# simonmeister/UnFlow

Measured on AMD Instinct MI355X. Metric: image-pairs/s (fwd+bwd) FlowNetC 384x512, higher is better.
Workload: dtype f32; 1 GPU; FlowNetC unsupervised step: bidirectional fwd + census/2nd-order loss pyramid + bwd + L2/Adam, 4 pairs/GPU, 384x512, 441-ch correlation (BASELINE configs[1]); global_batch=4, height=384, width=512, parallelism=dp1, hipgraph=True

## Files before the change

### include/unflow_hip.h

```cpp
#ifndef UNFLOW_HIP_H_
#define UNFLOW_HIP_H_

#include <stddef.h>

#ifdef __cplusplus
extern "C" {
#endif

typedef void* unflow_stream_t;
typedef struct unflow_planes unflow_planes;

#define UNFLOW_OK 0
#define UNFLOW_ERR_NULL (-1)
#define UNFLOW_ERR_EMPTY_OUTPUT (-2)
#define UNFLOW_ERR_EVEN_KERNEL (-3)
#define UNFLOW_ERR_NOT_DIVISIBLE (-4)
#define UNFLOW_ERR_SHAPE (-5)
#define UNFLOW_ERR_UNSUPPORTED (-7)
#define UNFLOW_ERR_LAUNCH (-8)
#define UNFLOW_ERR_WORKSPACE (-9)

const char* unflow_status_string(int status);
int unflow_version(void);

// ... 68 lines not shown
                             size_t workspace_bytes, unflow_stream_t stream);

int unflow_conv2d_transpose_fwd(const float* x, int ldx, const float* w, const float* bias, float* y, int ldy,
                                int B, int H, int W, int Cin, int Cout, int leaky, void* workspace,
                                size_t workspace_bytes, unflow_stream_t stream);
int unflow_conv2d_transpose_bwd_data(const float* dz, int lddz, const float* w, float* dx, int lddx, int B, int H,
                                     int W, int Cin, int Cout, int accumulate, const float* act_src, int ld_act,
                                     int act_lo, int act_hi, void* workspace, size_t workspace_bytes,
                                     unflow_stream_t stream);
int unflow_conv2d_transpose_bwd_filter(const float* x, int ldx, const float* dz, int lddz, float* dw, float* dbias,
                                       int B, int H, int W, int Cin, int Cout, void* workspace,
                                       size_t workspace_bytes, unflow_stream_t stream);

size_t unflow_colsum_batched_workspace_bytes(int n, const int* C);
int unflow_colsum_batched(int n, const float* const* x, const int* ld, const long* npix, const int* C,
                          float* const* out, void* workspace, size_t workspace_bytes, unflow_stream_t stream);

size_t unflow_conv_workspace_bytes(int B, int H, int W, int Cin, int Cout, int k, int stride);

int unflow_leaky_bwd_inplace(float* dy, int lddy, const float* y, int ldy, long npix, int C, unflow_stream_t stream);


int unflow_rgb_to_gray255(const float* im, int ld_im, float* gray, long npix, unflow_stream_t stream);

int unflow_warp_gray_fwd(const float* im, int ld_im, const float* flow, float flow_scale, float* out_gray,
                         int pair_shift, int N, int H, int W, unflow_stream_t stream);
int unflow_warp_gray_bwd(const float* d_gray, const float* im, int ld_im, const float* flow, float flow_scale,
                         float* d_flow, int accumulate, int pair_shift, int N, int H, int W,
                         unflow_stream_t stream);

int unflow_ternary_fwd(const float* gray1, const float* gray2w, const float* mask, int n_mask, float* dist_out,
                       float* loss_acc, float weight, float normalizer, int max_distance, int N, int H, int W,
                       unflow_stream_t stream);
int unflow_ternary_bwd(const float* gray1, const float* gray2w, const float* mask, int n_mask,
                       const float* dist, float* d_gray2w, float weight, float normalizer, int max_distance,
                       int N, int H, int W, unflow_stream_t stream);

int unflow_gray_pair(const float* im, int ld_im, const float* flow, float flow_scale, float* gray1, float* gray2w,
                     int pair_shift, int N, int H, int W, unflow_stream_t stream);
int unflow_ternary_warp_bwd(const float* gray1, const float* gray2w, const float* dist, const float* im, int ld_im,
                            const float* flow, float flow_scale, float* d_flow, int accumulate, int pair_shift,
                            int max_distance, int N, int H, int W, unflow_stream_t stream);

int unflow_second_order_fwd_bwd(const float* flow, float flow_scale, float* loss_acc, float* d_flow,
                                int accumulate, float weight, float normalizer, int N, int H, int W,
                                unflow_stream_t stream);

int unflow_mask_terms(const float* flow, const float* warped_other, const float* fwarp, const float* base_mask,
                      int n_base, float flow_scale, int occlusion_mode, float* mask_out, float* loss_acc, float* d_flow,
                      float* d_warped, int accumulate, float fb_weight, float occ_weight, float sym_weight,
                      int batch_per_direction, int pair_shift, int N, int H, int W, unflow_stream_t stream);

#define UNFLOW_MAX_PYR_LEVELS 7
typedef struct unflow_pyr_level {
  const float* im;
  const float* flow;
  float* gray1;
  float* gray2w;
  const float* mask;
  float* dist;
  float* d_flow;
  int H, W, n_mask, max_distance;
  float flow_scale, ternary_scale, smooth_scale;
} unflow_pyr_level;
int unflow_sizeof_pyr_level(void);
int unflow_loss_pyramid_default(const unflow_pyr_level* levels, int n_levels, int N, int pair_shift, float* loss_acc,
                                int with_grad, unflow_stream_t stream);

int unflow_photometric_fwd_bwd(const float* im, int ld_im, const float* flow, float flow_scale, const float* mask,
                               int n_mask, float* loss_acc, float* d_flow, int accumulate, float weight, float normalizer,
                               int pair_shift, int N, int H, int W, unflow_stream_t stream);

int unflow_charbonnier_loss(const float* x, const float* mask, int mask_channels, float truncate, float alpha, float beta,
                            float epsilon, float* loss_acc, float weight, long npix, int C, unflow_stream_t stream);
int unflow_length_sq(const float* x, float* out, long npix, int C, unflow_stream_t stream);

int unflow_smooth_1st_fwd_bwd(const float* flow, float flow_scale, float* loss_acc, float* d_flow, int accumulate,
                              float weight, float normalizer, int N, int H, int W, unflow_stream_t stream);

int unflow_gradient_loss_fwd(const float* im1, int ld_im1, const float* im2_warped, const float* mask, int n_mask,
                             float* gdiff, float* loss_acc, float weight, float normalizer, int N, int H, int W,
                             unflow_stream_t stream);
int unflow_gradient_loss_bwd(const float* gdiff, float* d_im2_warped, int N, int H, int W, unflow_stream_t stream);


int unflow_prepare_images(const float* im_u8range, float* net_in4, float* out01, const float* mean3, long npix,
                          unflow_stream_t stream);

int unflow_prepare_image_pair(const float* im1, const float* im2, long npix_each, float* net_in4, float* out01,
                              const float* mean3, const unflow_planes* net_pl, unflow_stream_t stream);

int unflow_scale(const float* x, float s, float* y, long n, unflow_stream_t stream);
int unflow_mul_inplace(float* y, const float* x, long n, unflow_stream_t stream);
int unflow_add_inplace(float* y, const float* x, long n, unflow_stream_t stream);
int unflow_zero(void* p, size_t bytes, unflow_stream_t stream);
int unflow_copy(void* dst, const void* src, size_t bytes, unflow_stream_t stream);


int unflow_stn_affine_fwd(const float* U, int n_u, int ld_u, const float* theta, int n_theta, float* out, int ld_out,
                          int B, int H, int W, int C, int out_h, int out_w, unflow_stream_t stream);

int unflow_photometric_augment(const float* im, int ld_in, float* out, int ld_out, const float* contrast,
                               const float* brightness, const float* colour3, const float* gamma, const float* noise,
                               int n_par, const float* mean3, int N, int H, int W, unflow_stream_t stream);

int unflow_supervised_geo_augment(const float* im1, const float* im2, const float* flow_gt, const float* mask_gt,
                                  const float* mats, const float* contrast, const float* brightness, const float* colour3,
                                  const float* gamma, const float* noise, int n_par, const float* mean3, float* im01, float* x0,
                                  int ld_out, float* flow_out, float* mask_out, int mode, int B, int H, int W,
                                  unflow_stream_t stream);

int unflow_stack_input(const float* net_in4, const float* prev_flow2, float* out, int ld_out, int pair_shift, int N,
                       int H, int W, int h, int w, float flow_scale, unflow_stream_t stream);

int unflow_stack_input_bwd(const float* d_out, int ld_out, const float* net_in4, const float* prev_flow2,
                           float* d_prev_flow2, int pair_shift, int N, int H, int W, int h, int w, float flow_scale,
                           unflow_stream_t stream);

typedef struct unflow_planes {
  void* base;
  long plane_stride;
  int ld;
  int n_planes;
  float scale;
} unflow_planes;

int unflow_correlation_nhwc_fwd_pl(const float* in0, const float* in1, int ld_in, const unflow_planes* in0_pl,
                                   const unflow_planes* in1_pl, int pair_shift, float* out, int ld_out, int B, int C,
                                   int H, int W, int kernel_size, int max_displacement, int pad, int stride_1,
                                   int stride_2, unflow_stream_t stream);

int unflow_correlation_nhwc_bwd_pl(const float* dout, int ld_dout, const float* in0, const float* in1, int ld_in,
                                   const unflow_planes* in0_pl, const unflow_planes* in1_pl, int pair_shift, float* grad0,
                                   float* grad1, int ld_grad, int accumulate_g1_into_g0, int B, int C, int H, int W,
                                   int kernel_size, int max_displacement, int pad, int stride_1, int stride_2,
                                   unflow_stream_t stream);

int unflow_planes_from_f32(const float* x, int ldx, long npix, int C, int C_fill, const unflow_planes* out,
                           unflow_stream_t stream);

size_t unflow_weight_planes_elems(int taps, int R, int Cc, int transposed);
int unflow_weight_planes_batched(int n, const float* const* w, const int* taps, const int* R, const int* Cc,
                                 void* const* direct, void* const* transposed, int n_planes, unflow_stream_t stream);

int unflow_adam_planes_batched(int n, float* const* w, const int* taps, const int* R, const int* Cc, void* const* direct,
                               void* const* transposed, const int* regularized, int n_planes, float* P, const float* G, float* M,
                               float* V, float grad_scale, float l2_scale, float lr_t, float beta1, float beta2, float eps,
                               float* loss_acc, unflow_stream_t stream);

size_t unflow_conv_pl_workspace_bytes(int B, int H, int W, int Cin, int Cout, int k, int stride, int n_planes);

size_t unflow_flow_wgrad_batched_workspace_bytes(int n, const int* kind, const int* B, const int* H, const int* W, const int* Cin);
int unflow_flow_wgrad_batched(int n, const int* kind, const float* const* x, const int* ldx, const float* const* dz,
                              const int* lddz, float* const* dw, const int* B, const int* H, const int* W, const int* Cin,
                              void* workspace, size_t workspace_bytes, unflow_stream_t stream);

int unflow_debug_work_order(int mt, int nt, int ncls, int nsplit, int order, int xcd, int* out, int out_blocks);

int unflow_comm_available(void);
int unflow_comm_unique_id(void* id128);
int unflow_comm_init(const void* id128, int nranks, int rank, void** comm);
int unflow_comm_info(void* comm, int* nranks, int* rank);
int unflow_allreduce_sum_f32(float* buf, long n, void* comm, unflow_stream_t stream);
int unflow_comm_destroy(void* comm);

int unflow_debug_streamk_plan(int G, int mtp, int nt, int nchunk, int ncls, const int* ntaps, int ngroups, int* range_pos, int npos,
                              const int* pos, int* decoded);
int unflow_debug_streamk_timeouts(void);

int unflow_conv2d_fwd_pl(const float* x, int ldx, const unflow_planes* x_pl, const float* w, const unflow_planes* w_pl,
                         const float* bias, float* y, int ldy, const unflow_planes* y_pl, int B, int H, int W, int Cin,
                         int Cout, int k, int stride, int leaky, void* workspace, size_t workspace_bytes,
                         unflow_stream_t stream);
int unflow_conv2d_bwd_data_pl(const float* dz, int lddz, const unflow_planes* dz_pl, const float* w,
                              const unflow_planes* w_pl, float* dx, int lddx, const unflow_planes* dx_pl, int pl_lo,
                              int pl_hi, int B, int H, int W, int Cin, int Cout, int k, int stride, int accumulate,
                              const float* act_src, int ld_act, const unflow_planes* act_pl, int act_lo, int act_hi,
                              void* workspace, size_t workspace_bytes, unflow_stream_t stream);
int unflow_conv2d_bwd_filter_pl(const float* x, int ldx, const unflow_planes* x_pl, const float* dz, int lddz,
                                const unflow_planes* dz_pl, float* dw, int B, int H, int W, int Cin, int Cout, int k,
                                int stride, void* workspace, size_t workspace_bytes, unflow_stream_t stream);
int unflow_conv2d_transpose_fwd_pl(const float* x, int ldx, const unflow_planes* x_pl, const float* w,
                                   const unflow_planes* w_pl, const float* bias, float* y, int ldy,
                                   const unflow_planes* y_pl, int B, int H, int W, int Cin, int Cout, int leaky,
                                   void* workspace, size_t workspace_bytes, unflow_stream_t stream);
int unflow_conv2d_transpose_bwd_data_pl(const float* dz, int lddz, const unflow_planes* dz_pl, const float* w,
                                        const unflow_planes* w_pl, float* dx, int lddx, const unflow_planes* dx_pl,
                                        int pl_lo, int pl_hi, int B, int H, int W, int Cin, int Cout, int accumulate,
                                        const float* act_src, int ld_act, const unflow_planes* act_pl, int act_lo,
                                        int act_hi, void* workspace, size_t workspace_bytes, unflow_stream_t stream);
int unflow_conv2d_transpose_bwd_filter_pl(const float* x, int ldx, const unflow_planes* x_pl, const float* dz, int lddz,
                                          const unflow_planes* dz_pl, float* dw, int B, int H, int W, int Cin, int Cout,
                                          void* workspace, size_t workspace_bytes, unflow_stream_t stream);

int unflow_resize_bilinear_tf1(const float* in, float* out, int B, int H, int W, int C, int out_h, int out_w,
                               float scale, unflow_stream_t stream);

int unflow_supervised_flow_loss(const float* flow, int h, int w, const float* flow_gt, const float* mask_gt, float flow_scale,
                                float weight, float* loss_acc, float* d_flow, int accumulate, int B, int H, int W,
                                unflow_stream_t stream);

int unflow_stack_input_pair(const float* first4, const float* second4, const float* prev_flow2, float* out, int ld_out, int N,
                            int H, int W, int h, int w, float flow_scale, unflow_stream_t stream);
int unflow_stack_input_pair_bwd(const float* d_out, int ld_out, const float* first4, const float* second4,
                                const float* prev_flow2, float* d_prev_flow2, int N, int H, int W, int h, int w,
                                float flow_scale, unflow_stream_t stream);

int unflow_adam_step(float* p, const float* grad, float* m, float* v, long n, long n_regularized, float grad_scale,
                     float l2_scale, float lr_t, float beta1, float beta2, float eps, unflow_stream_t stream);

int unflow_adam_step_regloss(float* p, const float* grad, float* m, float* v, long n, long n_regularized,
                             float grad_scale, float l2_scale, float lr_t, float beta1, float beta2, float eps,
                             float* loss_acc, unflow_stream_t stream);

int unflow_l2_loss(const float* p, long n, float scale, float* loss_acc, unflow_stream_t stream);

int unflow_flow_error_sums(const float* f1, const float* f2, const float* mask ,
                           float* out2, long npix, unflow_stream_t stream);



int unflow_inference_input(const void* frames, const int* desc, int B, int Hmax, int Wmax, int H, int W, float* net_in4,
                           const float* mean3, const unflow_planes* net_pl, unflow_stream_t stream);

int unflow_inference_input_frames(const void* frames, const int* desc, int F, int Hmax, int Wmax, int H, int W, float* net_in4,
                                  const float* mean3, const unflow_planes* net_pl, unflow_stream_t stream);

typedef struct {
  void* base;
  long pixels;
  int bytes;
  int stride;
} unflow_carry_buf;
#define UNFLOW_CARRY_MAX 16

int unflow_sequence_carry(const unflow_carry_buf* bufs, int n_bufs, const int* src_row, int max_row, unflow_stream_t stream);

int unflow_sequence_mirror(const unflow_carry_buf* bufs, int n_bufs, int src0, int dst0, int n, int max_row,
                           unflow_stream_t stream);

int unflow_sequence_track(const float* flow_fw, const unsigned char* occ_fw, const int* tab, int B, int Hmax, int Wmax,
                          const int* anchors, int Ncap, float* disp, unsigned char* alive, float* out_disp,
                          unsigned char* out_alive, unflow_stream_t stream);

int unflow_inference_output_blocks(int Hmax, int Wmax);
int unflow_inference_output(const float* flow, int fh, int fw, float flow_scale, int H, int W, const int* desc, int B, int Hmax,
                            int Wmax, float* out_flow, unsigned short* out_u16, const float* gt_flow, const float* gt_mask,
                            double* partial, unsigned* ticket, double* sums, int* counts, unflow_stream_t stream);

int unflow_inference_occlusion(const float* flow_fw, const float* flow_bw, const int* desc, int B, int Hmax, int Wmax,
                               const float* gt_mask, unsigned char* occ_fw, unsigned char* occ_bw, int* counts,
                               unflow_stream_t stream);



int unflow_flow_to_color(const float* flow, const float* mask, const float* max_flow, int B, int H, int W, float* out_f32,
                         unsigned char* out_u8, unsigned* max_bits, unflow_stream_t stream);

int unflow_flow_error_image(const float* flow_1, const float* flow_2, const float* mask_occ, const float* mask_noc, int log_colors,
                            int B, int H, int W, float* out_f32, unsigned char* out_u8, unflow_stream_t stream);

#define UNFLOW_VISUAL_IMAGES 5
int unflow_inference_visual(const void* frames, const int* desc, int B, int Hmax, int Wmax, int H, int W, const float* flow,
                            const float* gt_flow, const float* gt_mask, float* shown, unsigned* max_bits, unsigned char* out_u8,
                            float* out_f32, unflow_stream_t stream);

int unflow_sequence_visual(const void* frames, const int* tab, int B, int Hmax, int Wmax, int H, int W, const float* flow_fw,
                           const float* flow_bw, const unsigned char* occ_fw, float* shown, unsigned* max_bits,
                           unsigned char* out_u8, float* out_f32, unflow_stream_t stream);

size_t unflow_sequence_interpolate_workspace_bytes(int n, int B, int Hmax, int Wmax);
int unflow_sequence_interpolate(const void* frames, const int* tab, int B, int Hmax, int Wmax, int n, const float* flow_fw,
                                const float* flow_bw, const unsigned char* occ_fw, const unsigned char* occ_bw, void* prev,
                                void* workspace, unsigned char* out_mid, int* out_holes, unflow_stream_t stream);



int unflow_png_unfilter_rows(void);

int unflow_png_unfilter(const unsigned char* raw, long raw_bytes, unsigned char* decoded, long decoded_bytes, const long* desc,
                        int n, unflow_stream_t stream);

int unflow_png_to_batch(const unsigned char* decoded, long decoded_bytes, const long* desc, int n, int H, int W,
                        const float* mean3, float stddev, float* out, unflow_stream_t stream);

int unflow_png_to_window(const unsigned char* decoded, long decoded_bytes, const long* desc, int n, int Hs, int Ws,
                         const float* mean3, float stddev, float* out, unflow_stream_t stream);

int unflow_png_to_flow_gt(const unsigned char* decoded, long decoded_bytes, const long* desc, int n, int Hs, int Ws, float* flow,
                          float* mask, unflow_stream_t stream);

int unflow_flo_to_flow_gt(const unsigned char* raw, long raw_bytes, const long* desc, int n, int Hs, int Ws, float* flow,
                          float* mask, unflow_stream_t stream);

int unflow_sintel_gt(const unsigned char* raw, long raw_bytes, const unsigned char* decoded, long decoded_bytes, const long* desc,
                     int n, int Hs, int Ws, float* flow, float* mask, unflow_stream_t stream);


#define UNFLOW_PNG_U8 0
#define UNFLOW_PNG_U8X255 1
#define UNFLOW_PNG_U16BE 2
typedef struct {
  const void* base;
  long image_stride;
  long row_stride;
  int images, H, W;
  int channels;
  int kind;
} unflow_png_surface;
#define UNFLOW_PNG_SURFACES_MAX 16
#define UNFLOW_PNG_FILTER_FIELDS 8
#define UNFLOW_PNG_FILTER_MAX_ROW_BYTES 32512

int unflow_png_filter(const unflow_png_surface* surfaces, int n_surfaces, const long* desc, int n, int max_h, int max_row_bytes,
                      unsigned char* out, long out_bytes, unflow_stream_t stream);

int unflow_stream_create(unflow_stream_t* stream);

#define UNFLOW_DEFLATE_FIELDS 8
#define UNFLOW_DEFLATE_META 4
#define UNFLOW_DEFLATE_CHUNK_MAX 65535
#define UNFLOW_DEFLATE_CHUNK_DEFAULT 16384
int unflow_deflate(const unsigned char* in, long in_bytes, const long* desc, int n, int max_chunks, int chunk_bytes,
                   unsigned char* scratch, long scratch_bytes, int* meta, long meta_chunks, unsigned char* out, long out_bytes,
                   long* sizes, unflow_stream_t stream);
long unflow_deflate_segment_bound(int chunk_bytes);
long unflow_deflate_stream_bound(long bytes, int chunk_bytes);
long unflow_deflate_slot_bytes(int chunk_bytes);

#ifdef __cplusplus
}
#endif
#endif
```

### unflow_amd/core/engine.py

```python
import math
import os
from collections import OrderedDict

import numpy as np
import torch

from .. import _lib
from .._lib import check, ptr, stream, cf, cl
from . import layers as L

FLOW_SCALE = 5.0
CHANNEL_MEAN = [104.920005, 110.1753, 114.785955]
LAYER_WEIGHTS = [12.7, 4.35, 3.9, 3.4, 1.1]
LAYER_PATCH_DISTANCES = [3, 2, 2, 1, 1]
LAYER_WEIGHTS_FULL_RES = [12.7, 5.5, 5.0, 4.35, 3.9, 3.4, 1.1]
LAYER_PATCH_DISTANCES_FULL_RES = [3, 3] + LAYER_PATCH_DISTANCES
L2_SCALE = 0.0004
LOSSES = ['occ', 'sym', 'fb', 'grad', 'ternary', 'photo', 'smooth_1st', 'smooth_2nd']

DEFAULT_PARAMS = dict(flownet='C', pyramid_loss=True, border_mask=True, ternary_weight=1.0, smooth_2nd_weight=3.0)


def pad4(c):
    return (c + 3) // 4 * 4
# ... 302 lines not shown
        assert cuts == sorted(cuts) and (not cuts or cuts[-1] < len(self.bwd))
        self.part_bounds = [0] + cuts + [len(self.bwd)]

    def part_weight_range(self, part):
        ls = [op.l for op, _, _, _ in self.bwd[self.part_bounds[part]:self.part_bounds[part + 1]] if op.kind == 'layer']
        return self.eng.weight_range(ls)

    def alloc(self):
        e = self.eng
        H, W, dev = e.H, e.W, e.dev
        npl = e.n_planes
        self.A, self.Gd = {}, {}
        for name, (div, lay, width) in self.bufs.items():
            is_flow = name.startswith('flow')
            self.A[name] = L.PT.alloc((self.rows[name], H // div, W // div, width), dev, 0 if is_flow else npl)
        self.need_in_grad = (not self.is_c) and self.index > 0 and e.train_all
        if self.need_in_grad and self.full_res:
            raise NotImplementedError("train_all through a full_res refinement stage")
        if self.trainable:
            for name, (div, lay, width) in self.bufs.items():
                if name == 'x0s' and not self.need_in_grad:
                    continue
                is_flow = name.startswith('flow')
                self.Gd[name] = L.PT.alloc((self.rows[name], H // div, W // div, width), dev, 0 if is_flow else npl,
                                           scale=e.grad_plane_scale)
        self.planes_only = set()
        if npl:
            self.planes_only = {n for n in ('c1', 'c4', 'c5', 'c6') + (() if self.is_c else ('c3',)) if n in self.A}
        self.act = ActView(self)
        self.act.update({k: v.t for k, v in self.A.items()})
        self.grad = {k: v.t for k, v in self.Gd.items()}
        if self.full_res:
            self.act['x0s'] = self.act['cat0'][..., :pad4(self.in_ch)]

    def pt(self, spec, grad=False):
        b, lo, hi = spec
        if b == 'x0':
            return self.eng.X0
        src = (self.Gd if grad else self.A)[b]
        return src if (lo == 0 and hi == src.t.shape[-1]) else src.sl(lo, hi)

    def forward(self, prev_flow2=None):
        e = self.eng
        B, N = e.B, e.N
        if not self.is_c:
            x0s = self.act['x0s']
            pf = prev_flow2
            ph, pw = (0, 0) if pf is None else (pf.shape[1], pf.shape[2])
            if self.pairs is None:
                check(_lib.lib().unflow_stack_input(ptr(e.x0), ptr(pf), ptr(x0s), x0s.stride(2), B, N, e.H, e.W, ph, pw,
                                                    cf(4 * FLOW_SCALE), e.stream()), "stack_input")
            else:
                for a, b, o in self.pairs:
                    flow = None if pf is None else pf[o:o + B]
                    check(_lib.lib().unflow_stack_input_pair(ptr(e.x0[a:]), ptr(e.x0[b:]), ptr(flow), ptr(x0s[o:o + B]),
                                                             x0s.stride(2), B, e.H, e.W, ph, pw, cf(4 * FLOW_SCALE), e.stream()),
                          "stack_input_pair")
            inp = self.A[self.bin]
            if inp.pl is not None:
                w_in = pad4(self.in_ch)
                L.planes_from_f32(x0s, inp.pl[..., :round8(w_in)], C=w_in)
        for op in self.ops:
            if op.kind == 'corr':
                c3, out = self.pt(op.src), self.pt(op.dst)
                C = op.src[2] - op.src[1]
                h8, w8 = e.H // 8, e.W // 8
                pl = self._corr_planes(c3, refresh=True)
                if self.pairs is None:
                    c3pl = _lib.planes_of(pl)
                    check(_lib.lib().unflow_correlation_nhwc_fwd_pl(ptr(c3.t), ptr(c3.t), c3.t.stride(2), c3pl, c3pl, B,
                                                                    ptr(out.t), out.t.stride(2), N, C, h8, w8, 1, 20, 20, 1, 2,
                                                                    e.stream()), "correlation")
                else:
                    for a, b, o in self.pairs:
                        p0, p1 = (None, None) if pl is None else (_lib.planes_of(pl[:, a:a + B]), _lib.planes_of(pl[:, b:b + B]))
                        check(_lib.lib().unflow_correlation_nhwc_fwd_pl(ptr(c3.t[a:a + B]), ptr(c3.t[b:b + B]), c3.t.stride(2), p0, p1,
                                                                        0, ptr(out.t[o:o + B]), out.t.stride(2), B, C, h8, w8, 1, 20,
                                                                        20, 1, 2, e.stream()), "correlation")
                if out.pl is not None:
                    L.planes_from_f32(out.t, out.pl)
                continue
            l = op.l
            if self.pairs is not None and l.short == 'conv_redir':
                runs = [(a, o, B) for a, _, o in self.pairs]
            else:
                runs = [(op.r0, op.d0, op.n)]
            for r0, d0, n in runs:
                x, y = _row_range(self.pt(op.src), r0, n), _row_range(self.pt(op.dst), d0, n)
                if l.cout_p != l.cout:
                    y = L.PT(y.t.as_strided(y.t.shape[:3] + (l.cout_p,), y.t.stride(), y.t.storage_offset()),
                             None if y.pl is None else y.pl)
                po = op.dst[0] in self.planes_only
                if l.kind == 'conv':
                    L.conv_fwd(x, l.w, l.wpl_t, l.b, y, l.stride, l.act, planes_only=po)
                else:
                    L.deconv_fwd(x, l.w, l.wpl_d, l.b, y, l.act, planes_only=po)
            if self.seq_bidir and l.short == 'conv2' and self.is_c:
                self.sequence_mirror()

    def mirror_list(self):
        lo, n = self.bufs['cat2'][1]['conv2']
        return _carry_bufs(self.A['cat2'].t, self.A['cat2'].pl, lo, pad4(n))

    def sequence_mirror(self):
        B = self.eng.B
        bufs = self.mirror_list()
        arr = (_lib.CarryBuf * len(bufs))(*bufs)
        check(_lib.lib().unflow_sequence_mirror(arr, len(bufs), self.row0['cat2'] + 1, 0, B, self.rows['cat2'] - 1,
                                                self.eng.stream()), "sequence_mirror")

    def _corr_planes(self, c3, refresh=False):
        e = self.eng
        if e.n_planes == 3:
            return c3.pl
        if e.n_planes != 1:
            return None
        if getattr(self, '_c3_b3', None) is None:
            n, h, w, c = c3.t.shape
            self._c3_b3 = torch.zeros(3, n, h, w, (c + 7) // 8 * 8, dtype=torch.int16, device=c3.t.device)
        if refresh:
            L.planes_from_f32(c3.t, self._c3_b3)
        return self._c3_b3

    def _leaky_bwd_rows(self, g, a, r0, r1, clo, chi):
        gt, at = g.t[r0:r1, ..., clo:chi], a.t[r0:r1, ..., clo:chi]
        L.leaky_bwd_inplace(gt, at)
        if g.pl is not None:
            pl = g.pl[:, r0:r1, ..., clo:min(g.pl.shape[-1], clo + round8(chi - clo))]
            check(_lib.lib().unflow_planes_from_f32(ptr(gt), gt.stride(2), cl(gt.shape[0] * gt.shape[1] * gt.shape[2]),
                                                    chi - clo, min(round8(chi - clo), pl.shape[-1]), _lib.planes_of(pl, g.scale),
                                                    self.eng.stream()), "planes_from_f32")

    def backward(self, part=None, before_join=None):
        e = self.eng
        lo, hi = (0, len(self.bwd)) if part is None else (self.part_bounds[part], self.part_bounds[part + 1])
        B, N = e.B, e.N
        side = e.wgrad_stream
        main = torch.cuda.current_stream(e.dev)
        pending = []
        counter = [100 * (part or 0)]

        def flush():
            if not pending:
                return
            side.wait_stream(main)
            with torch.cuda.stream(side):
                for fn, a in pending:
                    with L.ws_slot(3 + (counter[0] if e.wgrad_unique_ws else 0)):
                        fn(*a)
                    counter[0] += 1
            pending.clear()

        flow_jobs = []
        n_flow = sum(1 for op, _, _, _ in self.bwd[lo:hi] if op.kind == 'layer' and op.l.cout <= 2)

        for k, (op, first, act_lo, act_hi) in enumerate(self.bwd[lo:hi], lo):
            if op.kind == 'corr':
                c3, g3, gout = self.pt(op.src), self.pt(op.src, True), self.pt(op.dst, True)
                C = op.src[2] - op.src[1]
                h8, w8 = e.H // 8, e.W // 8
                assert first
                pl = self._corr_planes(c3)
                if self.pairs is None:
                    c3pl = _lib.planes_of(pl)
                    check(_lib.lib().unflow_correlation_nhwc_bwd_pl(ptr(gout.t), gout.t.stride(2), ptr(c3.t), ptr(c3.t),
                                                                    c3.t.stride(2), c3pl, c3pl, B, ptr(g3.t), ptr(None),
                                                                    g3.t.stride(2), 1, N, C, h8, w8, 1, 20, 20, 1, 2, e.stream()),
                          "correlation_grad")
                else:
                    (a, b, o), = self.pairs
                    p0, p1 = (None, None) if pl is None else (_lib.planes_of(pl[:, a:a + B]), _lib.planes_of(pl[:, b:b + B]))
                    check(_lib.lib().unflow_correlation_nhwc_bwd_pl(ptr(gout.t[o:o + B]), gout.t.stride(2), ptr(c3.t[a:a + B]),
                                                                    ptr(c3.t[b:b + B]), c3.t.stride(2), p0, p1, 0, ptr(g3.t[a:a + B]),
                                                                    ptr(g3.t[b:b + B]), g3.t.stride(2), 0, B, C, h8, w8, 1, 20, 20, 1, 2,
                                                                    e.stream()), "correlation_grad")
                for r0, r1, clo, chi in self.bwd_post_act.get(k, ()):
                    self._leaky_bwd_rows(g3, c3, r0, r1, clo, chi)
                continue
            l = op.l
            x, dz = _rows(self.pt(op.src), op.n), _rows(self.pt(op.dst, True), op.n)
            if l.cout_p != l.cout:
                dz = L.PT(dz.t.as_strided(dz.t.shape[:3] + (l.cout_p,), dz.t.stride(), dz.t.storage_offset()), dz.pl, dz.scale)
            if e._bias_plan is None:
                e._bias_jobs.append((dz.t, l))
            xv = op.src[0] not in self.planes_only
            wg = (L.conv_bwd_filter, (x, dz, l.dw, l.stride, xv)) if l.kind == 'conv' else (L.deconv_bwd_filter, (x, dz, l.dw, xv))
            if l.cout <= 2:
                flow_jobs.append((l.kind, x, dz, l.dw))
                wg = (L.flow_wgrad_batched, (flow_jobs,)) if len(flow_jobs) == n_flow else None
            if wg is None:
                pass
            elif side is None or (e.wgrad_inline_tiny and l.cout <= 2):
                wg[0](*wg[1])
            else:
                pending.append(wg)
                if len(pending) >= e.wgrad_group:
                    flush()
            sb = op.src[0]
            is_input = sb == 'x0' or (sb == self.bin and op.src[1] == 0 and op.src[2] == pad4(self.in_ch)
                                      and op.l.name.endswith('conv1'))
            if sb not in self.Gd or (is_input and not self.need_in_grad):
                continue
            dx = _rows(self.pt(op.src, True), op.n)
            accumulate = (not first) or sb.startswith('flow')
            if k in self.bwd_zero_rows:
                r0, r1 = self.bwd_zero_rows[k]
                gz = self.Gd[sb].t[r0:r1]
                check(_lib.lib().unflow_zero(ptr(gz), _lib.csz(gz.numel() * 4), e.stream()), "zero")
            act_src = _rows(self.pt(op.src), op.n) if act_hi > act_lo else None
            apl = sb in self.planes_only
            if l.kind == 'conv':
                L.conv_bwd_data(dz, l.w, l.wpl_d, dx, l.stride, accumulate, act_src, act_lo, act_hi, act_planes=apl)
            else:
                L.deconv_bwd_data(dz, l.w, l.wpl_t, dx, accumulate, act_src, act_lo, act_hi, act_planes=apl)
        if side is not None:
            flush()
        if before_join is not None:
            before_join()
        if side is not None:
            main.wait_stream(side)


class FlowNetEngine:

    def __init__(self, batch, height, width, params=None, device=None, seed=0, layout_only=False, supervised=False,
                 inference=False, bidirectional=False, sequence=False):
        assert height % 64 == 0 and width % 64 == 0, "FlowNet needs H, W divisible by 64"
        if bidirectional and supervised:
            raise ValueError("FlowNetEngine: bidirectional is for the inference engine; the supervised engine is one-direction")
        if bidirectional and not inference:
            raise ValueError("FlowNetEngine: bidirectional needs inference=True (the training engine is bidirectional already)")
        if supervised and inference:
            raise ValueError("FlowNetEngine: supervised and inference are exclusive")
        if not isinstance(sequence, bool) and sequence != 'bidirectional':
            raise ValueError("FlowNetEngine: sequence is False, True or 'bidirectional', got %r" % (sequence,))
        if sequence and (bidirectional or supervised or not inference):
            raise ValueError("FlowNetEngine: sequence needs inference=True without supervised or bidirectional=True (both "
                             "directions of a clip: sequence='bidirectional')")
        self.supervised = bool(supervised)
        self.inference = bool(inference)
        self.seq_bidir = sequence == 'bidirectional'
        self.bidirectional = bool(bidirectional) or self.seq_bidir
        self.sequence = bool(sequence)
        self.one_dir = self.supervised or (self.inference and not self.bidirectional)
        self.params = dict(DEFAULT_PARAMS) if params is None else dict(params)
        if self.params.get('mask_occlusion', '') not in ('', 'fb', 'disocc'):
            raise ValueError("mask_occlusion must be one of 'fb', 'disocc', ''")
        spec = self.params.get('flownet', 'C')
        if not spec or any(ch not in 'CScs' for ch in spec) or any(ch in 'Cc' for ch in spec[1:]):
            raise ValueError("flownet spec: 'C'/'c' or 'S'/'s' first, then 'S'/'s' refinement nets (flownet.py:20-28)")
        self.train_all = bool(self.params.get('train_all')) and len(spec) > 1
        self.full_res = bool(self.params.get('full_res'))
        if self.supervised and self.full_res and self.train_all:
            raise ValueError("supervised full_res with train_all: the reference subtracts the earlier networks' quarter-size "
                             "flow2 * 20 from the full-size ground truth (supervised.py:50-60), a shape error")
        if sequence and self.full_res:
            raise ValueError("FlowNetEngine: sequence with full_res is not built (DESIGN 7.5)")
        self.spec = spec
        self.B, self.H, self.W = batch, height, width
        self.N = 2 * batch
        self.F = batch + 1
        self.dev = torch.device('cuda:0') if device is None else torch.device(device)
        self.math = conv_math_mode()
        self.wgrad_group = int(os.environ.get('UNFLOW_WGRAD_GROUP', '6'))
        self.wgrad_stream = None
        self.planes_external = False
        self.wgrad_unique_ws = False
        self.wgrad_inline_tiny = False
        self.n_planes = {'bf16x3': 3, 'f16': 1}.get(self.math, 0)
        self.fused_adam = os.environ.get('UNFLOW_FUSED_ADAM', '0') == '1'
        self.grad_plane_scale = 4096.0 if self.math == 'f16' else 0.0
        if layout_only:
            self.n_planes = 0
        self.fused_adam = self.fused_adam and self.n_planes > 0
        import contextlib
        with (torch.cuda.device(self.dev) if self.dev.type == 'cuda' else contextlib.nullcontext()):
            self.stages = [_Stage(self, k, i, self.full_res and i == len(spec) - 1) for i, k in enumerate(spec)]
            for st in self.stages[:-1]:
                st.trainable = self.train_all
            if self.inference:
                for st in self.stages:
                    st.trainable = False
            self.layers = [l for st in self.stages for l in st.layers]
            self.by_name = self.stages[-1].by_name
            self._alloc_params()
            if not layout_only:
                self._alloc_activations()
                if self.wgrad_group > 0 and self.dev.type == 'cuda' and not self.inference:
                    self.wgrad_stream = torch.cuda.Stream(self.dev)
                self._build_masks()
        self.step_count = 0
        self._bias_jobs, self._bias_plan = [], None
        self.defer_l2 = False
        self.fused_pyramid = True
        self._pyr_cache = None
        self._wplanes_version = None
        if seed is not None and not layout_only:
            self.init_params(seed)

    def stream(self):
        return stream(self.dev)

    def _alloc_params(self):
        nw = sum(int(torch.Size(l.wshape()).numel()) for l in self.layers)
        nb = sum(l.cout_p for l in self.layers)
        self.n_weights, self.n_params = nw, nw + nb
        z = lambda: torch.zeros(self.n_params, dtype=torch.float32, device=self.dev)
        self.P = z()
        self.G, self.M, self.V = (None, None, None) if self.inference else (z(), z(), z())
        view = lambda flat, lo, hi, shape=None: None if flat is None else (flat[lo:hi] if shape is None else flat[lo:hi].view(shape))
        off = 0
        for l in self.layers:
            n = int(torch.Size(l.wshape()).numel())
            l.w = self.P[off:off + n].view(l.wshape())
            l.dw = view(self.G, off, off + n, l.wshape())
            l.mw, l.vw = view(self.M, off, off + n, l.wshape()), view(self.V, off, off + n, l.wshape())
            off += n
        for l in self.layers:
            l.b = self.P[off:off + l.cout_p]
            l.db = view(self.G, off, off + l.cout_p)
            l.mb, l.vb = view(self.M, off, off + l.cout_p), view(self.V, off, off + l.cout_p)
            off += l.cout_p
        self._wp_table = None
        if self.n_planes:
            P = self.n_planes
            users = [l for l in self.layers if l.uses_planes()]
            tot = 0
            for l in users:
                d, t = self._wp_layouts(l)
                taps, R, Cc = l.wplane_view()
                tot += P * (d * taps * R * round8(Cc) + t * taps * Cc * round8(R))
            self.WP = torch.zeros(tot, dtype=torch.int16, device=self.dev)
            off = 0
            for l in users:
                d, t = self._wp_layouts(l)
                taps, R, Cc = l.wplane_view()
                if d:
                    n = P * taps * R * round8(Cc)
                    l.wpl_d = self.WP[off:off + n].view(P, taps, R, round8(Cc))
                    off += n
                if t:
                    n = P * taps * Cc * round8(R)
                    l.wpl_t = self.WP[off:off + n].view(P, taps, Cc, round8(R))
                    off += n
            self._wp_users = users
            self._wp_table = self._wp_table_of(users)
            self._wp_range_tables = {}
        self._adam_tables = {}

    def _wp_layouts(self, l):
# ... 828 lines not shown
```

### unflow_amd/core/layers.py

```python
import torch

from .. import _lib
from .._lib import check, ptr, stream, csz
from ..ops import workspace


def nhwc(t):
    assert t.dim() == 4 and t.dtype == torch.float32 and t.is_cuda, "NHWC float32 CUDA tensor expected"
    B, H, W, C = t.shape
    ld = t.stride(2)
    assert t.stride(3) == 1 and t.stride(1) == W * ld and t.stride(0) == H * W * ld, \
        "tensor must be a channel-slice view of a contiguous NHWC buffer"
    return ptr(t), ld, B, H, W, C


def out_hw(H, W, stride):
    return -(-H // stride), -(-W // stride)


_WS_SLOT = [1]


class ws_slot:

# ... 77 lines not shown

def conv2d_transpose_bwd_filter(x, dz, dw, dbias):
    xp, ldx, B, H, W, Cin = nhwc(x)
    dzp, lddz, _, Ho, Wo, Cout = nhwc(dz)
    assert tuple(dw.shape) == (4, 4, Cout, Cin)
    wsp, wsn = _ws(x.device, B, Ho, Wo, Cin, Cout, 4, 2)
    check(_lib.lib().unflow_conv2d_transpose_bwd_filter(xp, ldx, dzp, lddz, ptr(dw), ptr(dbias), B, H, W, Cin, Cout,
                                                        wsp, wsn, stream()), "conv2d_transpose_bwd_filter")
    return dw, dbias


def leaky_bwd_inplace(dy, y):
    dp, ldd, B, H, W, C = nhwc(dy)
    yp, ldy = nhwc(y)[:2]
    check(_lib.lib().unflow_leaky_bwd_inplace(dp, ldd, yp, ldy, _lib.cl(B * H * W), C, stream()), "leaky_bwd")
    return dy


def round8(c):
    return (c + 7) // 8 * 8


class PT:
    __slots__ = ('t', 'pl', 'scale')

    def __init__(self, t, pl=None, scale=0.0):
        self.t, self.pl, self.scale = t, pl, scale

    def sl(self, lo, hi):
        if self.pl is None:
            return PT(self.t[..., lo:hi])
        return PT(self.t[..., lo:hi], self.pl[..., lo:min(self.pl.shape[-1], lo + round8(hi - lo))], self.scale)

    def planes(self):
        return _lib.planes_of(self.pl, self.scale)

    @staticmethod
    def alloc(shape, device, n_planes, scale=0.0):
        import torch as _t
        t = _t.zeros(*shape, dtype=_t.float32, device=device)
        pad = 32
        cp = (shape[-1] + pad - 1) // pad * pad if shape[-1] > 8 else round8(shape[-1])
        pl = _t.zeros(n_planes, *shape[:-1], cp, dtype=_t.int16, device=device) if n_planes else None
        return PT(t, pl, scale if n_planes == 1 else 0.0)


def _pt(x):
    return x if isinstance(x, PT) else PT(x)


def _ws_pl(device, B, H, W, Cin, Cout, k, stride, npl):
    n = _lib.lib().unflow_conv_pl_workspace_bytes(B, H, W, Cin, Cout, k, stride, npl)
    t = workspace(n, device, slot=_WS_SLOT[0])
    return ptr(t), csz(t.numel() * 4)


def _npl(*pts):
    for q in pts:
        if q.pl is not None:
            return q.pl.shape[0]
    return 0


def planes_from_f32(x, out_pl, C=None):
    xp, ldx, B, H, W, Cx = nhwc(x)
    C = Cx if C is None else C
    fill = min(round8(C), out_pl.shape[-1])
    check(_lib.lib().unflow_planes_from_f32(xp, ldx, _lib.cl(B * H * W), C, fill, _lib.planes_of(out_pl), stream()),
          "planes_from_f32")


def conv_fwd(x, w, w_pl, bias, y, stride, leaky, planes_only=False):
    x, y = _pt(x), _pt(y)
    xp, ldx, B, H, W, Cin = nhwc(x.t)
    yp, ldy, _, Ho, Wo, Cout = nhwc(y.t)
    if planes_only:
        assert y.pl is not None
        yp = ptr(None)
    k = w.shape[0]
    assert tuple(w.shape) == (k, k, Cin, Cout) and w.is_contiguous() and (Ho, Wo) == out_hw(H, W, stride)
    wsp, wsn = _ws_pl(x.t.device, B, H, W, Cin, Cout, k, stride, _npl(x, y))
    check(_lib.lib().unflow_conv2d_fwd_pl(xp, ldx, x.planes(), ptr(w), _lib.planes_of(w_pl), ptr(bias), yp, ldy,
                                          y.planes(), B, H, W, Cin, Cout, k, stride, int(bool(leaky)), wsp, wsn,
                                          stream()), "conv2d_fwd_pl")


def _act_args(act_src, act_planes):
    if act_src is None:
        return ptr(None), 0, None
    a = _pt(act_src)
    if act_planes:
        assert a.pl is not None
        return ptr(None), 0, a.planes()
    ap, lda = nhwc(a.t)[:2]
    return ap, lda, None


def conv_bwd_data(dz, w, w_pl, dx, stride, accumulate=False, act_src=None, act_lo=0, act_hi=0, act_planes=False):
    dz, dx = _pt(dz), _pt(dx)
    dzp, lddz, B, Ho, Wo, Cout = nhwc(dz.t)
    dxp, lddx, _, H, W, Cin = nhwc(dx.t)
    k = w.shape[0]
    assert tuple(w.shape) == (k, k, Cin, Cout)
    ap, lda, apl = _act_args(act_src, act_planes)
    wsp, wsn = _ws_pl(dz.t.device, B, H, W, Cin, Cout, k, stride, _npl(dz, dx))
    check(_lib.lib().unflow_conv2d_bwd_data_pl(dzp, lddz, dz.planes(), ptr(w), _lib.planes_of(w_pl), dxp, lddx,
                                               dx.planes(), act_lo, act_hi, B, H, W, Cin, Cout, k, stride,
                                               int(bool(accumulate)), ap, lda, apl, act_lo, act_hi, wsp, wsn, stream()),
          "conv2d_bwd_data_pl")


def conv_bwd_filter(x, dz, dw, stride, x_fp32=True):
    x, dz = _pt(x), _pt(dz)
    xp, ldx, B, H, W, Cin = nhwc(x.t)
    if not x_fp32:
        assert x.pl is not None
        xp = ptr(None)
    dzp, lddz, _, Ho, Wo, Cout = nhwc(dz.t)
    k = dw.shape[0]
    assert tuple(dw.shape) == (k, k, Cin, Cout) and dw.is_contiguous()
    wsp, wsn = _ws_pl(x.t.device, B, H, W, Cin, Cout, k, stride, _npl(x, dz))
    check(_lib.lib().unflow_conv2d_bwd_filter_pl(xp, ldx, x.planes(), dzp, lddz, dz.planes(), ptr(dw), B, H,
                                                 W, Cin, Cout, k, stride, wsp, wsn, stream()), "conv2d_bwd_filter_pl")


def deconv_fwd(x, w, w_pl, bias, y, leaky, planes_only=False):
    x, y = _pt(x), _pt(y)
    xp, ldx, B, H, W, Cin = nhwc(x.t)
    yp, ldy, _, Ho, Wo, Cout = nhwc(y.t)
    if planes_only:
        assert y.pl is not None
        yp = ptr(None)
    assert tuple(w.shape) == (4, 4, Cout, Cin) and (Ho, Wo) == (2 * H, 2 * W)
    wsp, wsn = _ws_pl(x.t.device, B, 2 * H, 2 * W, Cin, Cout, 4, 2, _npl(x, y))
    check(_lib.lib().unflow_conv2d_transpose_fwd_pl(xp, ldx, x.planes(), ptr(w), _lib.planes_of(w_pl), ptr(bias), yp,
                                                    ldy, y.planes(), B, H, W, Cin, Cout, int(bool(leaky)), wsp, wsn,
                                                    stream()), "conv2d_transpose_fwd_pl")


def deconv_bwd_data(dz, w, w_pl, dx, accumulate=False, act_src=None, act_lo=0, act_hi=0, act_planes=False):
    dz, dx = _pt(dz), _pt(dx)
    dzp, lddz, B, Ho, Wo, Cout = nhwc(dz.t)
    dxp, lddx, _, H, W, Cin = nhwc(dx.t)
    assert tuple(w.shape) == (4, 4, Cout, Cin) and (Ho, Wo) == (2 * H, 2 * W)
    ap, lda, apl = _act_args(act_src, act_planes)
    wsp, wsn = _ws_pl(dz.t.device, B, Ho, Wo, Cin, Cout, 4, 2, _npl(dz, dx))
    check(_lib.lib().unflow_conv2d_transpose_bwd_data_pl(dzp, lddz, dz.planes(), ptr(w), _lib.planes_of(w_pl), dxp,
                                                         lddx, dx.planes(), act_lo, act_hi, B, H, W, Cin, Cout,
                                                         int(bool(accumulate)), ap, lda, apl, act_lo, act_hi, wsp, wsn,
                                                         stream()),
          "conv2d_transpose_bwd_data_pl")


def deconv_bwd_filter(x, dz, dw, x_fp32=True):
    x, dz = _pt(x), _pt(dz)
    xp, ldx, B, H, W, Cin = nhwc(x.t)
    if not x_fp32:
        assert x.pl is not None
        xp = ptr(None)
    dzp, lddz, _, Ho, Wo, Cout = nhwc(dz.t)
    assert tuple(dw.shape) == (4, 4, Cout, Cin)
    wsp, wsn = _ws_pl(x.t.device, B, Ho, Wo, Cin, Cout, 4, 2, _npl(x, dz))
    check(_lib.lib().unflow_conv2d_transpose_bwd_filter_pl(xp, ldx, x.planes(), dzp, lddz, dz.planes(),
                                                           ptr(dw), B, H, W, Cin, Cout, wsp, wsn, stream()),
          "conv2d_transpose_bwd_filter_pl")


def flow_wgrad_batched(jobs):
    import ctypes
    n = len(jobs)
    if n == 0:
        return
    xs = [_pt(j[1]).t for j in jobs]
    dzs = [_pt(j[2]).t for j in jobs]
    kinds = (ctypes.c_int * n)(*[0 if j[0] == 'conv' else 1 for j in jobs])
    dims = [nhwc(x) for x in xs]
    Bs = (ctypes.c_int * n)(*[d[2] for d in dims])
    Hs = (ctypes.c_int * n)(*[d[3] for d in dims])
    Ws = (ctypes.c_int * n)(*[d[4] for d in dims])
    Cs = (ctypes.c_int * n)(*[d[5] for d in dims])
    lib = _lib.lib()
    lib.unflow_flow_wgrad_batched_workspace_bytes.restype = ctypes.c_size_t
    need = lib.unflow_flow_wgrad_batched_workspace_bytes(n, kinds, Bs, Hs, Ws, Cs)
    if need == 0 or n > 16:
        for kind, x, dz, dw in jobs:
            if kind == 'conv':
                conv_bwd_filter(x, dz, dw, 1)
            else:
                deconv_bwd_filter(x, dz, dw)
        return
    for (kind, x, dz, dw), xt, dzt in zip(jobs, xs, dzs):
        assert dw.is_contiguous() and dzt.shape[-1] == 2
        assert tuple(dw.shape) == ((3, 3, xt.shape[-1], 2) if kind == 'conv' else (4, 4, 2, 2))
    ws = workspace(need, xs[0].device, slot=_WS_SLOT[0])
    check(lib.unflow_flow_wgrad_batched(n, kinds, (ctypes.c_void_p * n)(*[x.data_ptr() for x in xs]),
                                        (ctypes.c_int * n)(*[x.stride(2) for x in xs]),
                                        (ctypes.c_void_p * n)(*[d.data_ptr() for d in dzs]),
                                        (ctypes.c_int * n)(*[d.stride(2) for d in dzs]),
                                        (ctypes.c_void_p * n)(*[j[3].data_ptr() for j in jobs]), Bs, Hs, Ws, Cs, ptr(ws),
                                        csz(ws.numel() * 4), stream()), "flow_wgrad_batched")
```

### unflow_amd/csrc/conv_igemm.hip

```cpp
#include "igemm_shared.h"
#include "options.h"

namespace {
using namespace igemm;

constexpr int LDK = BK + 4;

struct GatherParams : GatherGeom {
  const float* src;
  const float* w;
  const float* bias;
  float* dst;
  float* partial;
  const float* act_src;
  int lds, ldd, ld_act, act_lo, act_hi;
  int nsplit;
  int leaky, accumulate;
  unsigned cs_magic;
  PlaneOut pl;
};

__device__ __forceinline__ float4 ldg4(const float* p) { return *reinterpret_cast<const float4*>(p); }

typedef __bf16 bf16x8 __attribute__((ext_vector_type(8)));
// ... 1246 lines not shown
    bool ok[2][2];
#pragma unroll
    for (int a = 0; a < 2; a++)
#pragma unroll
      for (int c = 0; c < 2; c++) {
        const int iy = ((oy + 1 - ky0) >> 1) - a, ix = ((ox + 1 - kx0) >> 1) - c;
        ok[a][c] = (unsigned)iy < (unsigned)H && (unsigned)ix < (unsigned)W;
        const float* xp = x + ((size_t)(b * H + min(max(iy, 0), H - 1)) * W + min(max(ix, 0), W - 1)) * ldx;
#pragma unroll
        for (int ci = 0; ci < CI; ci++) xv[a][c][ci] = xp[ci];
      }
    float acc[CO];
#pragma unroll
    for (int c = 0; c < CO; c++) acc[c] = bias ? bias[c] : 0.f;
#pragma unroll
    for (int a = 0; a < 2; a++)
#pragma unroll
      for (int c = 0; c < 2; c++) {
        const float* wp = w + ((ky0 + 2 * a) * 4 + kx0 + 2 * c) * CO * CI;
#pragma unroll
        for (int co = 0; co < CO; co++)
#pragma unroll
          for (int ci = 0; ci < CI; ci++) acc[co] += (ok[a][c] ? xv[a][c][ci] : 0.f) * wp[co * CI + ci];
      }
#pragma unroll
    for (int c = 0; c < CO; c++) {
      y[(size_t)e * ldy + c] = acc[c];
      store_planes(po, (size_t)e, c, acc[c]);
    }
  }
}

template <int CI, int CO>
__global__ void tiny_deconv_dgrad_kernel(const float* __restrict__ dz, int lddz, const float* __restrict__ w,
                                         float* __restrict__ dx, int lddx, int accumulate, int B, int H, int W) {
  const int OH = 2 * H, OW = 2 * W;
  const unsigned n = (unsigned)B * (unsigned)H * (unsigned)W;
  for (unsigned e = blockIdx.x * blockDim.x + threadIdx.x; e < n; e += gridDim.x * blockDim.x) {
    const Pix pp = decode_pix(e, (unsigned)W, (unsigned)H);
    const int ix = pp.x, iy = pp.y, b = pp.n;
    float g[16][CO];
    bool ok[16];
#pragma unroll
    for (int ky = 0; ky < 4; ky++)
#pragma unroll
      for (int kx = 0; kx < 4; kx++) {
        const int oy = 2 * iy + ky - 1, ox = 2 * ix + kx - 1;
        ok[ky * 4 + kx] = (unsigned)oy < (unsigned)OH && (unsigned)ox < (unsigned)OW;
        const float* gp = dz + ((size_t)(b * OH + min(max(oy, 0), OH - 1)) * OW + min(max(ox, 0), OW - 1)) * lddz;
#pragma unroll
        for (int co = 0; co < CO; co++) g[ky * 4 + kx][co] = gp[co];
      }
    float acc[CI];
#pragma unroll
    for (int c = 0; c < CI; c++) acc[c] = 0.f;
#pragma unroll
    for (int t = 0; t < 16; t++) {
      const float* wp = w + t * CO * CI;
#pragma unroll
      for (int co = 0; co < CO; co++)
#pragma unroll
        for (int ci = 0; ci < CI; ci++) acc[ci] += (ok[t] ? g[t][co] : 0.f) * wp[co * CI + ci];
    }
#pragma unroll
    for (int c = 0; c < CI; c++) {
      float* d = dx + (size_t)e * lddx + c;
      *d = accumulate ? *d + acc[c] : acc[c];
    }
  }
}

template <int CI, int CO>
__device__ __forceinline__ void tiny_deconv_wgrad_body(const float* __restrict__ x, int ldx, const float* __restrict__ dz, int lddz,
                                                       float* __restrict__ partial, int B, int H, int W, int bx, int nblocks,
                                                       float (*red)[16 * CO * CI]) {
  constexpr int NV = 16 * CO * CI;
  const int OH = 2 * H, OW = 2 * W;
  const long n = (long)B * H * W;
  float acc[16][CO][CI];
#pragma unroll
  for (int t = 0; t < 16; t++)
#pragma unroll
    for (int a = 0; a < CO; a++)
#pragma unroll
      for (int c = 0; c < CI; c++) acc[t][a][c] = 0.f;
  for (long e = bx * (long)blockDim.x + threadIdx.x; e < n; e += (long)nblocks * blockDim.x) {
    const int ix = (int)(e % W), iy = (int)((e / W) % H);
    const long b = e / ((long)W * H);
    float xv[CI];
#pragma unroll
    for (int c = 0; c < CI; c++) xv[c] = x[e * ldx + c];
#pragma unroll
    for (int ky = 0; ky < 4; ky++) {
      const int oy = 2 * iy + ky - 1;
#pragma unroll
      for (int kx = 0; kx < 4; kx++) {
        const int ox = 2 * ix + kx - 1;
        if ((unsigned)oy < (unsigned)OH && (unsigned)ox < (unsigned)OW) {
          const float* gp = dz + ((b * OH + oy) * OW + ox) * lddz;
#pragma unroll
          for (int co = 0; co < CO; co++)
#pragma unroll
            for (int ci = 0; ci < CI; ci++) acc[ky * 4 + kx][co][ci] += gp[co] * xv[ci];
        }
      }
    }
  }
  const int lane = threadIdx.x & 63, wid = threadIdx.x >> 6;
  static_assert(NV == 64, "the transpose-reduce below maps value index == lane");
  float v32[32], v16[16], v8[8], v4[4], v2[2];
  {
    const float* f = &acc[0][0][0];
    const bool hi = lane & 32;
#pragma unroll
    for (int i = 0; i < 32; i++) v32[i] = (hi ? f[32 + i] : f[i]) + __shfl_xor(hi ? f[i] : f[32 + i], 32);
  }
  {
    const bool hi = lane & 16;
#pragma unroll
    for (int i = 0; i < 16; i++) v16[i] = (hi ? v32[16 + i] : v32[i]) + __shfl_xor(hi ? v32[i] : v32[16 + i], 16);
  }
  {
    const bool hi = lane & 8;
#pragma unroll
    for (int i = 0; i < 8; i++) v8[i] = (hi ? v16[8 + i] : v16[i]) + __shfl_xor(hi ? v16[i] : v16[8 + i], 8);
  }
  {
    const bool hi = lane & 4;
#pragma unroll
    for (int i = 0; i < 4; i++) v4[i] = (hi ? v8[4 + i] : v8[i]) + __shfl_xor(hi ? v8[i] : v8[4 + i], 4);
  }
  {
    const bool hi = lane & 2;
#pragma unroll
    for (int i = 0; i < 2; i++) v2[i] = (hi ? v4[2 + i] : v4[i]) + __shfl_xor(hi ? v4[i] : v4[2 + i], 2);
  }
  {
    const bool hi = lane & 1;
    red[wid][lane] = (hi ? v2[1] : v2[0]) + __shfl_xor(hi ? v2[0] : v2[1], 1);
  }
  __syncthreads();
  if (threadIdx.x < NV)
    partial[(size_t)bx * NV + threadIdx.x] =
        (red[0][threadIdx.x] + red[1][threadIdx.x]) + (red[2][threadIdx.x] + red[3][threadIdx.x]);
}
template <int CI, int CO>
__global__ __launch_bounds__(256) void tiny_deconv_wgrad_kernel(const float* __restrict__ x, int ldx,
                                                                const float* __restrict__ dz, int lddz,
                                                                float* __restrict__ partial, int B, int H, int W) {
  __shared__ float red[4][16 * CO * CI];
  tiny_deconv_wgrad_body<CI, CO>(x, ldx, dz, lddz, partial, B, H, W, blockIdx.x, gridDim.x, red);
}

constexpr int MAX_FLOW_WGRAD = 16;
struct FlowWgradDesc {
  SkinnyWgradParams p;
  float* out;
  int kind;
  int spw, colblocks, chunks, block0, wsz, rblock0;
};
struct FlowWgradBatch {
  FlowWgradDesc d[MAX_FLOW_WGRAD];
  int n;
};
__global__ __launch_bounds__(256) void flow_wgrad_batched_kernel(const FlowWgradBatch b) {
  __shared__ float red[72 * 64];
  int di = 0;
  while (di + 1 < b.n && (int)blockIdx.x >= b.d[di + 1].block0) di++;
  const FlowWgradDesc& d = b.d[di];
  const int lb = blockIdx.x - d.block0;
  if (d.kind == 2) {
    tiny_deconv_wgrad_body<2, 2>(d.p.x, d.p.ldx, d.p.dz, d.p.lddz, d.p.partial, d.p.B, d.p.H, d.p.W, lb, d.chunks,
                                 reinterpret_cast<float(*)[64]>(red));
    return;
  }
  const int bx = lb % d.colblocks, by = lb / d.colblocks;
  if (d.kind == 0) head3_wgrad_strip_body<8>(d.p, d.spw, bx, by, red);
  else head3_wgrad_strip_body<4>(d.p, d.spw, bx, by, red);
}
__global__ __launch_bounds__(256) void flow_wgrad_sum_kernel(const FlowWgradBatch b) {
  int di = 0;
  while (di + 1 < b.n && (int)blockIdx.x >= b.d[di + 1].rblock0) di++;
  const FlowWgradDesc& d = b.d[di];
  const int e = (blockIdx.x - d.rblock0) * 16 + (threadIdx.x >> 4), q = threadIdx.x & 15;
  const bool ok = e < d.wsz;
  float v = 0.f;
  if (ok) {
#pragma unroll 16
    for (int k = q; k < d.chunks; k += 16) v += d.p.partial[(size_t)k * d.wsz + e];
  }
#pragma unroll
  for (int off = 1; off < 16; off <<= 1) v += __shfl_down(v, off, 64);
  if (ok && q == 0) d.out[e] = v;
}

constexpr int MAX_COLSUM = 32;
constexpr int COLSUM_MAX_CHUNKS = 256;
struct ColsumBatch {
  const float* x[MAX_COLSUM];
  float* out[MAX_COLSUM];
  long npix[MAX_COLSUM];
  int ld[MAX_COLSUM], C[MAX_COLSUM], chunks[MAX_COLSUM];
  int block0[MAX_COLSUM + 1];
  long part0[MAX_COLSUM];
  int n;
};

__global__ __launch_bounds__(256) void colsum_batched_kernel(const ColsumBatch d, float* __restrict__ partial) {
  __shared__ float red[16][64];
  int di = 0;
  while (di + 1 < d.n && (int)blockIdx.x >= d.block0[di + 1]) di++;
  const int lb = blockIdx.x - d.block0[di];
  const int C = d.C[di], ld = d.ld[di];
  const int ctiles = (C + 63) / 64;
  const int ct = lb % ctiles, chunk = lb / ctiles;
  const long per = (d.npix[di] + d.chunks[di] - 1) / d.chunks[di];
  const long r0 = chunk * per, r1 = min(d.npix[di], r0 + per);
  const float* x = d.x[di];
  const bool vec = (C % 4 == 0) && (ld % 4 == 0) && ((reinterpret_cast<size_t>(x) & 15) == 0);
  if (vec) {
    const int cq = threadIdx.x & 15, rl = threadIdx.x >> 4;
    const int col = ct * 64 + cq * 4;
    float4 s0 = make_float4(0, 0, 0, 0), s1 = s0;
    if (col < C) {
      long r = r0 + rl;
      for (; r + 16 < r1; r += 32) {
        const float4 a = *reinterpret_cast<const float4*>(x + r * ld + col);
        const float4 b = *reinterpret_cast<const float4*>(x + (r + 16) * ld + col);
        s0.x += a.x; s0.y += a.y; s0.z += a.z; s0.w += a.w;
        s1.x += b.x; s1.y += b.y; s1.z += b.z; s1.w += b.w;
      }
      if (r < r1) {
        const float4 a = *reinterpret_cast<const float4*>(x + r * ld + col);
        s0.x += a.x; s0.y += a.y; s0.z += a.z; s0.w += a.w;
      }
    }
    red[rl][cq * 4] = s0.x + s1.x; red[rl][cq * 4 + 1] = s0.y + s1.y;
    red[rl][cq * 4 + 2] = s0.z + s1.z; red[rl][cq * 4 + 3] = s0.w + s1.w;
  } else {
    const int cl = threadIdx.x & 63, rl = threadIdx.x >> 6;
    const int col = ct * 64 + cl;
    float s0 = 0.f;
    if (col < C)
      for (long r = r0 + rl; r < r1; r += 4) s0 += x[r * ld + col];
    red[rl][cl] = s0;
    for (int k = 4 + rl; k < 16; k += 4) red[k][cl] = 0.f;
  }
  __syncthreads();
  if (threadIdx.x < 64) {
    const int col = ct * 64 + threadIdx.x;
    if (col < C) {
      float v = 0.f;
#pragma unroll
      for (int k = 0; k < 16; k++) v += red[k][threadIdx.x];
      partial[d.part0[di] + (size_t)chunk * C + col] = v;
    }
  }
}

__global__ __launch_bounds__(256) void colsum_batched_final_kernel(const ColsumBatch d, const float* __restrict__ partial) {
  __shared__ float red[4][64];
  const int di = blockIdx.y;
  const int C = d.C[di];
  const int col = blockIdx.x * 64 + (threadIdx.x & 63), rl = threadIdx.x >> 6;
  if (blockIdx.x * 64 >= C) return;
  float v = 0.f;
  if (col < C)
    for (int k = rl; k < d.chunks[di]; k += 4) v += partial[d.part0[di] + (size_t)k * C + col];
  red[rl][threadIdx.x & 63] = v;
  __syncthreads();
  if (rl == 0 && col < C)
    d.out[di][col] = (red[0][threadIdx.x] + red[1][threadIdx.x]) + (red[2][threadIdx.x] + red[3][threadIdx.x]);
}

__global__ void leaky_bwd_inplace_kernel(float* __restrict__ dy, int lddy, const float* __restrict__ y, int ldy,
                                         long npix, int C) {
  const long n = npix * C;
  for (long e = blockIdx.x * (long)blockDim.x + threadIdx.x; e < n; e += (long)gridDim.x * blockDim.x) {
    const long px = e / C;
    const int c = (int)(e - px * C);
    dy[px * lddy + c] *= leaky_grad_from_out(y[px * ldy + c]);
  }
}


struct GatherPlan {
  int cfg;
  int nsplit;
};

inline bool conv_math_bf16x3() { return !unflow::options().conv_math_fp32; }

inline bool wgrad_math_bf16x3() { return conv_math_bf16x3() && !unflow::options().wgrad_math_fp32; }

inline GatherPlan plan_gather(const GatherParams& p) {
  GatherPlan pl;
  const long M = (long)p.B * p.Hg * p.Wg;
  if (p.N <= 32) pl.cfg = 2;
  else if (p.N <= 64) pl.cfg = 1;
  else pl.cfg = 0;
  int maxtaps = 0;
  for (int c = 0; c < p.ncls; c++) maxtaps = max(maxtaps, p.cls[c].nty * p.cls[c].ntx);
  const int KT = (maxtaps * p.Cs + BK - 1) / BK;
  const int min_kt = max(1, unflow::options().gather_min_kt);
  const int max_by_k = min(16, KT / min_kt > 0 ? KT / min_kt : 1);
  if (pl.cfg == 0) {
    const long b128 = ((M + 127) / 128) * ((p.N + 127) / 128) * p.ncls;
    if (b128 * max_by_k < 384) pl.cfg = 2;
  }
  const int bm = pl.cfg == 2 ? 64 : 128, bn = pl.cfg == 0 ? 128 : 64;
  const int slots = 256 * (pl.cfg == 0 ? 3 : pl.cfg == 1 ? 4 : 6);
  const long blocks = ((M + bm - 1) / bm) * ((p.N + bn - 1) / bn) * p.ncls;
  pl.nsplit = fill_one_round(blocks, slots, max_by_k);
  return pl;
}

inline size_t gather_partial_bytes(const GatherParams& p, int nsplit) {
  return nsplit > 1 ? (size_t)nsplit * p.B * p.Hd * p.Wd * p.N * sizeof(float) : 0;
}

inline int wgrad_cfg(const WgradParams& p) { return p.Cb <= 64 ? 1 : 0; }

inline int plan_wgrad(const WgradParams& p) {
  const int Mp = p.KH * p.KW * p.Ca;
  const int cfg = wgrad_cfg(p);
  const int bn = cfg == 1 ? 64 : 128;
  const long blocks = (long)cdiv(Mp, 128) * cdiv(p.Cb, bn);
  const long S = (long)p.B * p.Hg * p.Wg;
  const int KT = (int)((S + BK - 1) / BK);
  const int min_kt = max(1, unflow::options().wgrad_min_kt);
  const int max_by_k = min(256, KT / min_kt > 0 ? KT / min_kt : 1);
  const bool b3 = wgrad_math_bf16x3();
  const int slots = 256 * (b3 ? (cfg == 1 ? 4 : 3) : cfg == 1 ? 5 : 4);
  return fill_one_round(blocks, slots, max_by_k);
}

inline size_t wgrad_partial_bytes(const WgradParams& p, int nsplit) {
  const size_t n = (size_t)p.KH * p.KW * p.Ca * p.Cb;
  return nsplit > 1 ? (size_t)nsplit * n * sizeof(float) + reduce_scratch_bytes(n, nsplit) : 0;
}

inline int skinny_wgrad_chunks(long npix, int Cin) {
  const long colblocks = (Cin / 4 + 63) / 64;
  long c = (4096 + colblocks - 1) / colblocks;
  c = min(c, max((long)1, npix / 8));
  return (int)min(c, (long)1024);
// ... 248 lines not shown
    else if (Cout == 1) skinny_conv_dgrad_kernel<1><<<stream_grid(total), 256, 0, st>>>(p);
    else if (Cout == 4) skinny_conv_dgrad_kernel<4><<<stream_grid(total), 256, 0, st>>>(p);
    else return UNFLOW_ERR_UNSUPPORTED;
    return launch_status();
  }
  if (Cout % 4 != 0 || lddz % 4 != 0) return UNFLOW_ERR_UNSUPPORTED;
  if (k == 1 && stride == 1 && Cout == PW_CO && lddx % 4 == 0 && (!act_src || ld_act % 4 == 0) &&
      (reinterpret_cast<uintptr_t>(dx) & 15) == 0 && (reinterpret_cast<uintptr_t>(act_src) & 15) == 0 &&
      (reinterpret_cast<uintptr_t>(w) & 15) == 0) {
    SkinnyBwdParams sp{dz, lddz, w, dx, lddx, act_src, ld_act, act_lo, act_hi, accumulate, B, H, W, Cin, 1, 0, 0, po};
    const long jobs = (((long)B * H * W + PW_S - 1) / PW_S) * cdiv(Cin / 4, 64);
    pointwise32_dgrad_kernel<<<(int)((jobs + 3) / 4), 256, 0, st>>>(sp);
    return launch_status();
  }
  GatherParams p{};
  const int bc = build_conv_dgrad(p, B, H, W, Cin, Cout, k, stride);
  if (bc != UNFLOW_OK) return bc;
  p.src = dz; p.w = w; p.bias = nullptr; p.dst = dx; p.act_src = act_src;
  p.lds = lddz; p.ldd = lddx; p.ld_act = ld_act; p.act_lo = act_lo; p.act_hi = act_hi;
  p.leaky = 0; p.accumulate = accumulate;
  p.pl = po;
  return run_gather<true>(p, workspace, workspace_bytes, st);
}

UNFLOW_API int unflow_conv2d_bwd_filter(const float* x, int ldx, const float* dz, int lddz, float* dw, float* dbias,
                                        int B, int H, int W, int Cin, int Cout, int k, int stride, void* workspace,
                                        size_t workspace_bytes, unflow_stream_t stream) {
  if (!x || !dz || !dw) return UNFLOW_ERR_NULL;
  if (B <= 0 || H <= 0 || W <= 0 || Cin <= 0 || Cout <= 0 || k <= 0 || stride <= 0) return UNFLOW_ERR_SHAPE;
  if (Cin % 4 != 0 || ldx % 4 != 0 || ldx < Cin || lddz < Cout) return UNFLOW_ERR_UNSUPPORTED;
  int pt, pl, Ho, Wo;
  same_pads(H, k, stride, &pt, &Ho);
  same_pads(W, k, stride, &pl, &Wo);
  hipStream_t st = as_stream(stream);
  size_t used = 0;
  if (Cout <= 4) {
    if (stride != 1 || k != 3 || Cout != 2) return UNFLOW_ERR_UNSUPPORTED;
    const long npix = (long)B * H * W;
    const size_t wsz = (size_t)9 * Cin * Cout;
    const int S = head_strip(B, H, W, k, Cout);
    const bool strip = S != 0;
    int spw = 1;
    const int chunks = strip ? head_wgrad_blocks(B, H, W, Cin, S, &spw) : skinny_wgrad_chunks(npix, Cin);
    used = (size_t)chunks * wsz * sizeof(float) + reduce_scratch_bytes(wsz, chunks);
    if (!workspace || workspace_bytes < used) return UNFLOW_ERR_WORKSPACE;
    SkinnyWgradParams p{x, ldx, dz, lddz, reinterpret_cast<float*>(workspace), B, H, W, Cin, pt, pl};
    dim3 grid(cdiv(Cin / 4, 64), chunks);
    if (S == 8) head3_wgrad_strip_kernel<8><<<grid, 256, 0, st>>>(p, spw);
    else if (S == 4) head3_wgrad_strip_kernel<4><<<grid, 256, 0, st>>>(p, spw);
    else skinny_conv_wgrad3_kernel<2><<<grid, 64, 0, st>>>(p);
    const int rc = reduce_partials(p.partial, p.partial + (size_t)chunks * wsz, dw, wsz, chunks, st);
    if (rc != UNFLOW_OK) return rc;
  } else {
    if (Cout % 4 != 0 || lddz % 4 != 0) return UNFLOW_ERR_UNSUPPORTED;
    WgradParams p{};
    build_conv_wgrad(p, B, H, W, Cin, Cout, k, stride);
    p.src = x; p.dst = dz; p.out = dw; p.lds = ldx; p.ldd = lddz;
    const int code = run_wgrad(p, workspace, workspace_bytes, &used, st);
    if (code != UNFLOW_OK) return code;
  }
  if (dbias) return run_colsum(dz, lddz, (long)B * Ho * Wo, Cout, dbias, workspace, workspace_bytes, used, st);
  return launch_status();
}

UNFLOW_API int unflow_conv2d_transpose_fwd(const float* x, int ldx, const float* w, const float* bias, float* y,
                                           int ldy, int B, int H, int W, int Cin, int Cout, int leaky, void* workspace,
                                           size_t workspace_bytes, unflow_stream_t stream) {
  return unflow_conv2d_transpose_fwd_po(x, ldx, w, bias, y, ldy, B, H, W, Cin, Cout, leaky, igemm::PlaneOut{}, workspace,
                                        workspace_bytes, stream);
}

int unflow_conv2d_transpose_fwd_po(const float* x, int ldx, const float* w, const float* bias, float* y, int ldy, int B, int H,
                                   int W, int Cin, int Cout, int leaky, const igemm::PlaneOut& po, void* workspace,
                                   size_t workspace_bytes, unflow_stream_t stream) {
  if (!x || !w || !y) return UNFLOW_ERR_NULL;
  if (B <= 0 || H <= 0 || W <= 0 || Cin <= 0 || Cout <= 0) return UNFLOW_ERR_SHAPE;
  hipStream_t st = as_stream(stream);
  if (Cin == 2 && Cout == 2) {
    if (leaky) return UNFLOW_ERR_UNSUPPORTED;
    tiny_deconv_fwd_kernel<2, 2><<<stream_grid((long)B * 4 * H * W), 256, 0, st>>>(x, ldx, w, bias, y, ldy, B, H, W, po);
    return launch_status();
  }
  if (Cin % 4 != 0 || ldx % 4 != 0 || ldx < Cin || ldy < Cout) return UNFLOW_ERR_UNSUPPORTED;
  GatherParams p{};
  build_deconv_fwd(p, B, H, W, Cin, Cout);
  p.src = x; p.w = w; p.bias = bias; p.dst = y; p.act_src = nullptr;
  p.lds = ldx; p.ldd = ldy; p.leaky = leaky; p.accumulate = 0;
  p.pl = po;
  return run_gather<true>(p, workspace, workspace_bytes, st);
}

UNFLOW_API int unflow_conv2d_transpose_bwd_data(const float* dz, int lddz, const float* w, float* dx, int lddx, int B,
                                                int H, int W, int Cin, int Cout, int accumulate, const float* act_src,
                                                int ld_act, int act_lo, int act_hi, void* workspace,
                                                size_t workspace_bytes, unflow_stream_t stream) {
  return unflow_conv2d_transpose_bwd_data_po(dz, lddz, w, dx, lddx, B, H, W, Cin, Cout, accumulate, act_src, ld_act, act_lo,
                                             act_hi, igemm::PlaneOut{}, workspace, workspace_bytes, stream);
}

int unflow_conv2d_transpose_bwd_data_po(const float* dz, int lddz, const float* w, float* dx, int lddx, int B, int H, int W,
                                        int Cin, int Cout, int accumulate, const float* act_src, int ld_act, int act_lo,
                                        int act_hi, const igemm::PlaneOut& po, void* workspace, size_t workspace_bytes,
                                        unflow_stream_t stream) {
  if (!dz || !w || !dx) return UNFLOW_ERR_NULL;
  if (B <= 0 || H <= 0 || W <= 0 || Cin <= 0 || Cout <= 0) return UNFLOW_ERR_SHAPE;
  hipStream_t st = as_stream(stream);
  if (Cin == 2 && Cout == 2) {
    if (act_src) return UNFLOW_ERR_UNSUPPORTED;
    tiny_deconv_dgrad_kernel<2, 2><<<stream_grid((long)B * H * W), 256, 0, st>>>(dz, lddz, w, dx, lddx, accumulate, B, H, W);
    return launch_status();
  }
  if (Cout % 4 != 0 || Cin % 4 != 0 || lddz % 4 != 0 || lddz < Cout || lddx < Cin) return UNFLOW_ERR_UNSUPPORTED;
  GatherParams p{};
  build_deconv_dgrad(p, B, H, W, Cin, Cout);
  p.src = dz; p.w = w; p.bias = nullptr; p.dst = dx; p.act_src = act_src;
  p.lds = lddz; p.ldd = lddx; p.ld_act = ld_act; p.act_lo = act_lo; p.act_hi = act_hi;
  p.leaky = 0; p.accumulate = accumulate;
  p.pl = po;
  return run_gather<false>(p, workspace, workspace_bytes, st);
}

UNFLOW_API int unflow_conv2d_transpose_bwd_filter(const float* x, int ldx, const float* dz, int lddz, float* dw,
                                                  float* dbias, int B, int H, int W, int Cin, int Cout, void* workspace,
                                                  size_t workspace_bytes, unflow_stream_t stream) {
  if (!x || !dz || !dw) return UNFLOW_ERR_NULL;
  if (B <= 0 || H <= 0 || W <= 0 || Cin <= 0 || Cout <= 0) return UNFLOW_ERR_SHAPE;
  hipStream_t st = as_stream(stream);
  size_t used = 0;
  if (Cin == 2 && Cout == 2) {
    const int blocks = (int)min((long)32, ((long)B * H * W + 255) / 256);
    if (!workspace || workspace_bytes < (size_t)blocks * 64 * sizeof(float)) return UNFLOW_ERR_WORKSPACE;
    float* part = reinterpret_cast<float*>(workspace);
    tiny_deconv_wgrad_kernel<2, 2><<<blocks, 256, 0, st>>>(x, ldx, dz, lddz, part, B, H, W);
    sum_partials_kernel<<<1, 64, 0, st>>>(part, dw, 64, blocks, 128);
    used = (size_t)blocks * 64 * sizeof(float);
  } else {
    if (Cout % 4 != 0 || Cin % 4 != 0 || lddz % 4 != 0 || ldx % 4 != 0) return UNFLOW_ERR_UNSUPPORTED;
    WgradParams p{};
    build_deconv_wgrad(p, B, H, W, Cin, Cout);
    p.src = dz; p.dst = x; p.out = dw; p.lds = lddz; p.ldd = ldx;
    const int code = run_wgrad(p, workspace, workspace_bytes, &used, st);
    if (code != UNFLOW_OK) return code;
  }
  if (dbias) return run_colsum(dz, lddz, (long)B * 4 * H * W, Cout, dbias, workspace, workspace_bytes, used, st);
  return launch_status();
}

static bool flow_wgrad_plan(FlowWgradDesc& d, int kind_in, int B, int H, int W, int Cin) {
  if (kind_in == 1) {
    d.kind = 2; d.colblocks = 1; d.spw = 0; d.wsz = 64;
    d.chunks = (int)min((long)32, ((long)B * H * W + 255) / 256);
    return true;
  }
  const int S = head_strip(B, H, W, 3, 2);
  if (S != 8 && S != 4) return false;
  d.kind = S == 8 ? 0 : 1;
  d.colblocks = cdiv(Cin / 4, 64);
  d.wsz = 9 * Cin * 2;
  const long nstrips = (long)B * H * (W / S);
  const long blocks = min((long)256, max((long)1, nstrips / 16));
  const long spw = (nstrips + blocks * 4 - 1) / (blocks * 4);
  d.spw = (int)spw;
  d.chunks = (int)((nstrips + spw * 4 - 1) / (spw * 4));
  return true;
}

UNFLOW_API size_t unflow_flow_wgrad_batched_workspace_bytes(int n, const int* kind, const int* B, const int* H, const int* W,
                                                            const int* Cin) {
  size_t need = 0;
  for (int i = 0; i < n; i++) {
    FlowWgradDesc d{};
    if (!flow_wgrad_plan(d, kind[i], B[i], H[i], W[i], Cin[i])) return 0;
    need += ((size_t)d.chunks * d.wsz * sizeof(float) + 255) & ~(size_t)255;
  }
  return need;
}

UNFLOW_API int unflow_flow_wgrad_batched(int n, const int* kind, const float* const* x, const int* ldx, const float* const* dz,
                                         const int* lddz, float* const* dw, const int* B, const int* H, const int* W, const int* Cin,
                                         void* workspace, size_t workspace_bytes, unflow_stream_t stream) {
  if (!kind || !x || !ldx || !dz || !lddz || !dw || !B || !H || !W || !Cin) return UNFLOW_ERR_NULL;
  if (n <= 0) return UNFLOW_OK;
  if (n > MAX_FLOW_WGRAD) return UNFLOW_ERR_UNSUPPORTED;
  FlowWgradBatch b{};
  b.n = n;
  size_t off = 0;
  int blocks = 0, rblocks = 0;
  for (int i = 0; i < n; i++) {
    FlowWgradDesc& d = b.d[i];
    if (!x[i] || !dz[i] || !dw[i]) return UNFLOW_ERR_NULL;
    if (B[i] <= 0 || H[i] <= 0 || W[i] <= 0 || Cin[i] <= 0) return UNFLOW_ERR_SHAPE;
    if (kind[i] == 0 && (Cin[i] % 4 != 0 || ldx[i] % 4 != 0 || ldx[i] < Cin[i] || lddz[i] < 2)) return UNFLOW_ERR_UNSUPPORTED;
    if (kind[i] == 1 && Cin[i] != 2) return UNFLOW_ERR_UNSUPPORTED;
    if (!flow_wgrad_plan(d, kind[i], B[i], H[i], W[i], Cin[i])) return UNFLOW_ERR_UNSUPPORTED;
    int pt, pl, ho, wo;
    same_pads(H[i], 3, 1, &pt, &ho);
    same_pads(W[i], 3, 1, &pl, &wo);
    const size_t bytes = ((size_t)d.chunks * d.wsz * sizeof(float) + 255) & ~(size_t)255;
    if (!workspace || off + bytes > workspace_bytes) return UNFLOW_ERR_WORKSPACE;
    d.p = SkinnyWgradParams{x[i], ldx[i], dz[i], lddz[i], reinterpret_cast<float*>(reinterpret_cast<char*>(workspace) + off),
                            B[i], H[i], W[i], Cin[i], pt, pl};
    off += bytes;
    d.out = dw[i];
    d.block0 = blocks;
    blocks += d.chunks * d.colblocks;
    d.rblock0 = rblocks;
    rblocks += cdiv(d.wsz, 16);
  }
  hipStream_t st = as_stream(stream);
  flow_wgrad_batched_kernel<<<blocks, 256, 0, st>>>(b);
  flow_wgrad_sum_kernel<<<rblocks, 256, 0, st>>>(b);
  return launch_status();
}

UNFLOW_API int unflow_leaky_bwd_inplace(float* dy, int lddy, const float* y, int ldy, long npix, int C,
                                        unflow_stream_t stream) {
  if (!dy || !y) return UNFLOW_ERR_NULL;
  if (npix <= 0 || C <= 0) return UNFLOW_OK;
  leaky_bwd_inplace_kernel<<<stream_grid(npix * C), 256, 0, as_stream(stream)>>>(dy, lddy, y, ldy, npix, C);
  return launch_status();
}

UNFLOW_API size_t unflow_colsum_batched_workspace_bytes(int n, const int* C) {
  size_t t = 0;
  for (int i = 0; i < n; i++) t += (size_t)COLSUM_MAX_CHUNKS * C[i];
  return t * sizeof(float) + 256;
}

UNFLOW_API int unflow_colsum_batched(int n, const float* const* x, const int* ld, const long* npix, const int* C,
                                     float* const* out, void* workspace, size_t workspace_bytes,
                                     unflow_stream_t stream) {
  if (!x || !ld || !npix || !C || !out || !workspace) return UNFLOW_ERR_NULL;
  if (n <= 0) return UNFLOW_OK;
  if (n > MAX_COLSUM) return UNFLOW_ERR_UNSUPPORTED;
  if (workspace_bytes < unflow_colsum_batched_workspace_bytes(n, C)) return UNFLOW_ERR_WORKSPACE;
  ColsumBatch d{};
  d.n = n;
  int blocks = 0;
  long poff = 0;
  for (int i = 0; i < n; i++) {
    if (!x[i] || !out[i] || C[i] <= 0 || npix[i] <= 0 || ld[i] < C[i]) return UNFLOW_ERR_SHAPE;
    d.x[i] = x[i]; d.out[i] = out[i]; d.npix[i] = npix[i]; d.ld[i] = ld[i]; d.C[i] = C[i];
    d.chunks[i] = (int)min((long)COLSUM_MAX_CHUNKS, max((long)1, npix[i] / 512));
    d.block0[i] = blocks;
    blocks += ((C[i] + 63) / 64) * d.chunks[i];
    d.part0[i] = poff;
    poff += (long)d.chunks[i] * C[i];
  }
  d.block0[n] = blocks;
  hipStream_t st = as_stream(stream);
  float* part = reinterpret_cast<float*>(workspace);
  colsum_batched_kernel<<<blocks, 256, 0, st>>>(d, part);
  int maxc = 0;
  for (int i = 0; i < n; i++) maxc = max(maxc, C[i]);
  colsum_batched_final_kernel<<<dim3((maxc + 63) / 64, n), 256, 0, st>>>(d, part);
  return launch_status();
}
```

### unflow_amd/csrc/conv_planes.hip

```cpp
#include "igemm_shared.h"
#include "planes_shared.h"
#include "halo_kernel.h"

namespace {
using namespace igemm;

template <int BM, int BN, int WM, int WN, int NPL, bool F16>
__global__ __launch_bounds__(256, (NPL == 3 && BM == 128 && BN == 128) ? 3 : 1) void igemm_pl_gather_kernel(const PlGatherParams p) {
  constexpr int TM = WM / 32, TN = WN / 32;
  constexpr int WAVES_N = BN / WN;
  static_assert((BM / WM) * WAVES_N == 4, "4 waves");
  static_assert(BM % 64 == 0 && BN % 64 == 0, "row passes of 64");
  constexpr int A_PLANE = BM * LDH, B_PLANE = BN * LDH;
  constexpr int AR = BM / 64, NB = BN / 64;
  constexpr int NT = NPL == 3 ? 6 : 1;

  extern __shared__ __attribute__((aligned(16))) unsigned short smem16[];
  const int tid = threadIdx.x, lane = tid & 63, wid = tid >> 6;
  unsigned short* Ah = smem16;
  unsigned short* Bh = Ah + NPL * A_PLANE;
  int* pix = reinterpret_cast<int*>(reinterpret_cast<char*>(smem16) + pl_gather_main_bytes(BM, BN, WN, NPL));

  const int wm = wid / WAVES_N, wn = wid % WAVES_N;
  int mtile, ntile, cls_id, split;
// ... 295 lines not shown
    for (int i = 0; i < AR; i++) {
      const int y = (a_yx[i] >> 16) + dy, x = (a_yx[i] & 0xffff) + dx;
      const bool inb = (unsigned)y < (unsigned)p.Hs && (unsigned)x < (unsigned)p.Ws;
      const int voff = inb ? a_lin[i] + a_tile : OOB_MARK;
#pragma unroll
      for (int pl = 0; pl < NPL; pl++) ra[i][pl] = buf_ld16(src_rs[pl], voff);
    }
    {
      const int voff = b_row + w_tile;
#pragma unroll
      for (int pl = 0; pl < NPL; pl++) rb[pl] = buf_ld16(w_rs[pl], voff);
    }
    q_cg += adv_c;
    q_tap += adv_t;
    const bool wrap = q_cg >= Cg;
    q_cg -= wrap ? Cg : 0;
    q_tap += wrap ? 1 : 0;
    ld_left--;
  };
  auto swz = [](int row, int g) { return row * LDP + 8 * (g ^ ((row >> 2) & 3)); };
  auto store_tile = [&](int buf) {
    unsigned short* Ah = Abase + buf * A_TILE;
    unsigned short* Bh = Bbase + buf * B_TILE;
#pragma unroll
    for (int i = 0; i < AR; i++)
#pragma unroll
      for (int pl = 0; pl < NPL; pl++)
        *reinterpret_cast<u32x4*>(Ah + pl * A_PLANE + swz((tid >> 2) + 64 * i, kq)) = ra[i][pl];
#pragma unroll
    for (int pl = 0; pl < NPL; pl++) *reinterpret_cast<u32x4*>(Bh + pl * B_PLANE + swz(b_r, kq)) = rb[pl];
  };

  f32x16 acc[TM][TN];
#pragma unroll
  for (int i = 0; i < TM; i++)
#pragma unroll
    for (int j = 0; j < TN; j++)
#pragma unroll
      for (int r = 0; r < 16; r++) acc[i][j][r] = 0.f;

  const int l31 = lane & 31, lh = lane >> 5;
  const int gsw = lh ^ ((l31 >> 2) & 3);
  const int a_rd = (wm * WM + l31) * LDP, b_rd = (wn * WN + l31) * LDP;
  s16x8 av[2][TM][NPL], bv[2][TN][NPL];
  auto read_frags = [&](int buf) {
    const unsigned short* Ah = Abase + buf * A_TILE + a_rd;
    const unsigned short* Bh = Bbase + buf * B_TILE + b_rd;
#pragma unroll
    for (int slab = 0; slab < 2; slab++)
#pragma unroll
      for (int pl = 0; pl < NPL; pl++) {
#pragma unroll
        for (int j = 0; j < TN; j++)
          bv[slab][j][pl] = *reinterpret_cast<const s16x8*>(Bh + pl * B_PLANE + j * 32 * LDP + 8 * (gsw ^ (2 * slab)));
#pragma unroll
        for (int i = 0; i < TM; i++)
          av[slab][i][pl] = *reinterpret_cast<const s16x8*>(Ah + pl * A_PLANE + i * 32 * LDP + 8 * (gsw ^ (2 * slab)));
      }
  };
  auto slot_end = [&]() {
    __builtin_amdgcn_sched_barrier(0);
    __builtin_amdgcn_s_barrier();
    __builtin_amdgcn_sched_barrier(0);
  };

  if (T > 0) {
    load_tile();
    asm volatile("s_waitcnt vmcnt(0)" ::: "memory");
    store_tile(0);
    load_tile();
    asm volatile("s_waitcnt lgkmcnt(0)" ::: "memory");
    slot_end();
    if (inst == 1) slot_end();
#pragma unroll 1
    for (int t = 0; t < T; t++) {
      read_frags(t & 1);
      __builtin_amdgcn_sched_barrier(0);
      asm volatile("s_waitcnt vmcnt(0)" ::: "memory");
      store_tile((t + 1) & 1);
      __builtin_amdgcn_sched_barrier(0);
      load_tile();
      __builtin_amdgcn_sched_barrier(0);
      asm volatile("s_waitcnt lgkmcnt(0)" ::: "memory");
      slot_end();
      __builtin_amdgcn_s_setprio(1);
#pragma unroll
      for (int slab = 0; slab < 2; slab++)
#pragma unroll
        for (int tt = 0; tt < NT; tt++)
#pragma unroll
          for (int i = 0; i < TM; i++)
#pragma unroll
            for (int j = 0; j < TN; j++) mfma_terms<NPL, F16>(av[slab][i], bv[slab][j], acc[i][j], tt);
      __builtin_amdgcn_s_setprio(0);
      slot_end();
    }
    if (inst == 0) slot_end();
    asm volatile("s_waitcnt vmcnt(0)" ::: "memory");
  }
  __syncthreads();
  if (!tile_ok) return;
  pl_gather_epilogue<WM, WN>(p, acc, pix, smem16 + inst * 2 * A_TILE, wm, wn, wid, lane, n0, split);
}


__global__ void pl_splitk_reduce_epilogue_kernel(const PlGatherParams p, int vec) {
  const size_t npix = (size_t)p.B * p.Hd * p.Wd;
  const size_t total = npix * p.N;
  if (vec) {
    const unsigned nq = (unsigned)(p.N >> 2);
    const size_t totq = total >> 2;
    for (size_t q = blockIdx.x * (size_t)blockDim.x + threadIdx.x; q < totq; q += (size_t)gridDim.x * blockDim.x) {
      const size_t px = q / nq;
      const int n = (int)(q - px * nq) * 4;
      const float4* src = reinterpret_cast<const float4*>(p.partial) + q;
      float4 v = make_float4(0.f, 0.f, 0.f, 0.f);
#pragma unroll 4
      for (int s = 0; s < p.nsplit; s++) {
        const f32x4_nt t = __builtin_nontemporal_load(reinterpret_cast<const f32x4_nt*>(src) + (size_t)s * totq);
        v.x += t.x; v.y += t.y; v.z += t.z; v.w += t.w;
      }
      epi_store4(p, px, n, v);
    }
    return;
  }
  for (size_t e = blockIdx.x * (size_t)blockDim.x + threadIdx.x; e < total; e += (size_t)gridDim.x * blockDim.x) {
    const size_t px = e / p.N;
    const int n = (int)(e - px * p.N);
    float v = 0.f;
    for (int s = 0; s < p.nsplit; s++) v += p.partial[(size_t)s * total + e];
    v *= p.src_inv;
    if (p.bias) v += p.bias[n];
    if (p.leaky) v = leaky_relu(v);
    float* d = p.dst + px * p.ldd + n;
    if (p.accumulate) v += *d;
    if (n >= p.act_lo && n < p.act_hi) {
      if (p.act_src) v *= leaky_grad_from_out(p.act_src[px * p.ld_act + n]);
      else if (p.act_pl) v *= leaky_grad_from_bits(p.act_pl[px * p.ld_act + n]);
    }
    if (p.dst) *d = v;
    store_planes(p.pl, px, n, v);
  }
}


struct PlWgradParams : WgradGeom {
  const unsigned short* src;
  long src_ps;
  const unsigned short* dst;
  long dst_ps;
  float* out;
  float* partial;
  int lds, ldd;
  int Ca_out;
  float out_scale;
  int nsplit;
  int gpx;
  unsigned cag_magic;
  int mt, nt, xcd;
};

template <int ROWS>
__device__ __forceinline__ int tr_swz(int k, int granule) {
  const int pair = granule >> 1;
  const int sw = ROWS == 128 ? ((k & 3) << 1) : (((k >> 1) & 1) << 1);
  return k * ROWS + (((pair ^ sw) << 1) | (granule & 1)) * 8;
}

template <int BM, int BN, int WM, int WN, int NPL, bool F16>
__global__ __launch_bounds__(256, (NPL == 3 && BM == 128 && BN == 128) ? 3 : 1) void igemm_pl_wgrad_kernel(const PlWgradParams p) {
  constexpr int TM = WM / 32, TN = WN / 32;
  constexpr int WAVES_N = BN / WN;
  static_assert((BM / WM) * WAVES_N == 4, "4 waves");
  static_assert((BM == 128 || BM == 64) && (BN == 128 || BN == 64), "swizzle forms");
  constexpr int A_PLANE = BK * BM, B_PLANE = BK * BN;
  constexpr int AJ = BM / 8, BJ = BN / 8;
  constexpr int AKS = 256 / AJ, BKS = 256 / BJ;
  constexpr int AR = BK / AKS, BR = BK / BKS;
  constexpr int NT = NPL == 3 ? 6 : 1;

  extern __shared__ __attribute__((aligned(16))) unsigned short smem16[];
  unsigned short* Ah = smem16;
  unsigned short* Bh = Ah + NPL * A_PLANE;

  const int tid = threadIdx.x, lane = tid & 63, wid = tid >> 6;
  const int wm = wid / WAVES_N, wn = wid % WAVES_N;
  const int taps = p.KH * p.KW;
  const int Cag = p.Ca >> 3;
  const int Mg = taps * Cag;
  int v = xcd_remap(blockIdx.x, gridDim.x, p.xcd);
  const int mtile = v % p.mt; v /= p.mt;
  const int ntile = v % p.nt;
  const int split = v / p.nt;
  const int m0 = mtile * BM, n0 = ntile * BN;
  const int S = p.B * p.Hg * p.Wg;
  const int KT = (S + BK - 1) / BK;
  const int kt_per = (KT + p.nsplit - 1) / p.nsplit;
  const int kt0 = split * kt_per, kt1 = min(KT, kt0 + kt_per);

  __amdgpu_buffer_rsrc_t src_rs[NPL], dst_rs[NPL];
#pragma unroll
  for (int pl = 0; pl < NPL; pl++) {
    src_rs[pl] = make_rsrc(p.src + pl * p.src_ps, (((size_t)p.B * p.Hs * p.Ws - 1) * (size_t)p.lds + (size_t)(p.gpx ? p.lds : p.Ca)) * 2);
    dst_rs[pl] = make_rsrc(p.dst + pl * p.dst_ps, (((size_t)S - 1) * (size_t)p.ldd + (size_t)((p.Cb + 7) & ~7)) * 2);
  }

  const int aj = tid % AJ, ak = tid / AJ;
  const int mg = (m0 >> 3) + aj;
  const bool m_ok = mg < Mg;
  const unsigned tap = p.cag_magic ? fast_div((unsigned)mg, p.cag_magic) : (unsigned)mg;
  const int ag = mg - (int)tap * Cag;
  const int ky = (int)tap / p.KW, kx = (int)tap - ky * p.KW;
  const int dy = p.dy0 + ky, dx = p.dx0 + kx + p.gpx * ag;
  const int lds2 = p.lds * 2;
  const int a_lane_off = (dy * p.Ws + (p.dx0 + kx)) * lds2 + ag * 16;
  const int bj = tid % BJ, bk = tid / BJ;
  const int nbq = (n0 >> 3) + bj;
  const bool b_ok = nbq * 8 < p.Cb;
  const int b_lane_off = nbq * 16;
  const int ldd2 = p.ldd * 2;
  const unsigned magW = (unsigned)((0x100000000ull + p.Wg - 1) / p.Wg), magH = (unsigned)((0x100000000ull + p.Hg - 1) / p.Hg);

  u32x4 ra[AR][NPL], rb[BR][NPL];
  auto piece_a = [&](int i, int kt) {
    const unsigned sidx = (unsigned)(kt * BK + ak + AKS * i);
    const unsigned q = fast_div(sidx, magW);
    const int xg = (int)(sidx - q * (unsigned)p.Wg);
    const unsigned bb = fast_div(q, magH);
    const int yg = (int)(q - bb * (unsigned)p.Hg);
    const int yb = yg * p.sm, xb = xg * p.sm;
    const bool ok = m_ok && (int)bb < p.B && (unsigned)(yb + dy) < (unsigned)p.Hs && (unsigned)(xb + dx) < (unsigned)p.Ws;
    const int voff = ok ? (((int)bb * p.Hs + yb) * p.Ws + xb) * lds2 + a_lane_off : OOB_MARK;
#pragma unroll
    for (int pl = 0; pl < NPL; pl++) ra[i][pl] = buf_ld16(src_rs[pl], voff);
  };
  auto piece_b = [&](int i, int kt) {
    const int sidx = kt * BK + bk + BKS * i;
    const int voff = (b_ok && sidx < S) ? sidx * ldd2 + b_lane_off : OOB_MARK;
#pragma unroll
    for (int pl = 0; pl < NPL; pl++) rb[i][pl] = buf_ld16(dst_rs[pl], voff);
  };
  constexpr int NPIECE = AR + BR;
  auto piece = [&](int step, int kt) {
    if (step < AR) piece_a(step, kt);
    else if (step < AR + BR) piece_b(step - AR, kt);
  };
  auto store_tile = [&]() {
#pragma unroll
    for (int i = 0; i < AR; i++)
#pragma unroll
      for (int pl = 0; pl < NPL; pl++)
        *reinterpret_cast<u32x4*>(Ah + pl * A_PLANE + tr_swz<BM>(ak + AKS * i, aj)) = ra[i][pl];
#pragma unroll
    for (int i = 0; i < BR; i++)
#pragma unroll
      for (int pl = 0; pl < NPL; pl++)
        *reinterpret_cast<u32x4*>(Bh + pl * B_PLANE + tr_swz<BN>(bk + BKS * i, bj)) = rb[i][pl];
  };

  f32x16 acc[TM][TN];
#pragma unroll
  for (int i = 0; i < TM; i++)
#pragma unroll
    for (int j = 0; j < TN; j++)
#pragma unroll
      for (int r = 0; r < 16; r++) acc[i][j][r] = 0.f;

  const int i16 = lane & 15, grp = lane >> 4, lh = grp >> 1;
  const int krow = 8 * lh + (i16 >> 2);
  int a_rd[TM], b_rd[TN];
#pragma unroll
  for (int i = 0; i < TM; i++) {
    const int c = wm * WM + i * 32 + 16 * (grp & 1) + 4 * (i16 & 3);
    a_rd[i] = tr_swz<BM>(krow, c >> 3) + (c & 7);
  }
#pragma unroll
  for (int j = 0; j < TN; j++) {
    const int c = wn * WN + j * 32 + 16 * (grp & 1) + 4 * (i16 & 3);
    b_rd[j] = tr_swz<BN>(krow, c >> 3) + (c & 7);
  }
#pragma unroll
  for (int st = 0; st < NPIECE; st++) piece(st, kt0);
  store_tile();
  __syncthreads();
  constexpr int NGROUP = 2 * NT;
  constexpr int PPG = (NPIECE + NGROUP - 1) / NGROUP;
  const int l31 = lane & 31;
  for (int kt = kt0; kt < kt1; kt++) {
    const int ktn = kt + 1 < kt1 ? kt + 1 : KT + 1;
    s16x8 av[TM][NPL], bv[TN][NPL];
    auto read_slab = [&](int slab) {
#pragma unroll
      for (int pl = 0; pl < NPL; pl++) {
#pragma unroll
        for (int i = 0; i < TM; i++) {
          const unsigned short* b0 = Ah + pl * A_PLANE + a_rd[i] + (16 * slab) * BM;
          const s16x4 lo = __builtin_amdgcn_ds_read_tr16_b64_v4i16((s16x4 __attribute__((address_space(3)))*)(b0));
          const s16x4 hi = __builtin_amdgcn_ds_read_tr16_b64_v4i16((s16x4 __attribute__((address_space(3)))*)(b0 + 4 * BM));
          av[i][pl] = __builtin_shufflevector(lo, hi, 0, 1, 2, 3, 4, 5, 6, 7);
        }
#pragma unroll
        for (int j = 0; j < TN; j++) {
          const unsigned short* b0 = Bh + pl * B_PLANE + b_rd[j] + (16 * slab) * BN;
          const s16x4 lo = __builtin_amdgcn_ds_read_tr16_b64_v4i16((s16x4 __attribute__((address_space(3)))*)(b0));
          const s16x4 hi = __builtin_amdgcn_ds_read_tr16_b64_v4i16((s16x4 __attribute__((address_space(3)))*)(b0 + 4 * BN));
          bv[j][pl] = __builtin_shufflevector(lo, hi, 0, 1, 2, 3, 4, 5, 6, 7);
        }
      }
    };
#pragma unroll
    for (int slab = 0; slab < 2; slab++) {
      read_slab(slab);
#pragma unroll
      for (int t = 0; t < NT; t++) {
#pragma unroll
        for (int i = 0; i < TM; i++)
#pragma unroll
          for (int j = 0; j < TN; j++) mfma_terms<NPL, F16>(av[i], bv[j], acc[i][j], t);
#pragma unroll
        for (int q2 = 0; q2 < PPG; q2++) piece((slab * NT + t) * PPG + q2, ktn);
        __builtin_amdgcn_sched_barrier(0);
      }
    }
    __syncthreads();
    store_tile();
    __syncthreads();
  }

  float* o = p.nsplit > 1 ? p.partial + (size_t)split * taps * p.Ca_out * p.Cb : p.out;
  const int lh5 = lane >> 5;
#pragma unroll
  for (int i = 0; i < TM; i++)
#pragma unroll
    for (int r = 0; r < 16; r++) {
      const int m = m0 + wm * WM + i * 32 + (r & 3) + 8 * (r >> 2) + 4 * lh5;
      const int mgr = m >> 3;
      if (mgr >= Mg) continue;
      const unsigned tp = p.cag_magic ? fast_div((unsigned)mgr, p.cag_magic) : (unsigned)mgr;
      const int a = (mgr - (int)tp * Cag) * 8 + (m & 7);
      if (a >= p.Ca_out) continue;
      float* orow = o + ((size_t)tp * p.Ca_out + a) * p.Cb;
#pragma unroll
      for (int j = 0; j < TN; j++) {
        const int n = n0 + wn * WN + j * 32 + l31;
        if (n < p.Cb) orow[n] = acc[i][j][r] * p.out_scale;
      }
    }
}

template <int BN, int WN, bool F16 = false>
__global__ __launch_bounds__(256, 3) void igemm_pl_wgrad_dma_kernel(const PlWgradParams p) {
  constexpr int BM = 128, WM = 64, NPL = 3, KS = 16;
  constexpr int GPS = F16 ? 3 : 1;
  constexpr int TM = WM / 32, TN = WN / 32;
  constexpr int WAVES_N = BN / WN;
  static_assert((BM / WM) * WAVES_N == 4, "4 waves");
  static_assert(BN == 128 || BN == 64, "swizzle forms");
  constexpr int A_PLANE = KS * BM, B_PLANE = KS * BN;
  constexpr int STAGE = NPL * (A_PLANE + B_PLANE);
  constexpr int B_RPI = 512 / BN;
  constexpr int B_NI = KS / B_RPI;
  constexpr int B_SLOTS = BN / 8;

  extern __shared__ __attribute__((aligned(16))) unsigned short smem16[];

  const int lane = threadIdx.x & 63;
  const int wid = __builtin_amdgcn_readfirstlane(threadIdx.x >> 6);
  const int wm = wid / WAVES_N, wn = wid % WAVES_N;
  const int taps = p.KH * p.KW;
  const int Cag = p.Ca >> 3;
  const int Mg = taps * Cag;
  int v = xcd_remap(blockIdx.x, gridDim.x, p.xcd);
  const int mtile = v % p.mt; v /= p.mt;
  const int ntile = v % p.nt;
  const int split = v / p.nt;
  const int m0 = mtile * BM, n0 = ntile * BN;
  const int S = p.B * p.Hg * p.Wg;
  const int KT = ((S + KS - 1) / KS + GPS - 1) / GPS;
  const int kt_per = F16 ? (KT + p.nsplit - 1) / p.nsplit
                         : (((KT + 1) / 2 + p.nsplit - 1) / p.nsplit) * 2;
  const int kt0 = split * kt_per, kt1 = min(KT, kt0 + kt_per);

  u32x4 src_rs[NPL], dst_rs[NPL];
#pragma unroll
  for (int pl = 0; pl < NPL; pl++) {
    src_rs[pl] = raw_rsrc(p.src + (F16 ? 0 : pl * p.src_ps), (((size_t)p.B * p.Hs * p.Ws - 1) * (size_t)p.lds + (size_t)(p.gpx ? p.lds : p.Ca)) * 2);
    dst_rs[pl] = raw_rsrc(p.dst + (F16 ? 0 : pl * p.dst_ps), (((size_t)S - 1) * (size_t)p.ldd + (size_t)((p.Cb + 7) & ~7)) * 2);
  }

  const int a_k = 4 * wid + (lane >> 4);
  const int a_slot = lane & 15;
  const int a_g = ((((a_slot >> 1) ^ ((a_k & 3) << 1)) << 1) | (a_slot & 1));
  const int mg = (m0 >> 3) + a_g;
  const bool m_ok = mg < Mg;
  const unsigned tap = p.cag_magic ? fast_div((unsigned)mg, p.cag_magic) : (unsigned)mg;
  const int ag = mg - (int)tap * Cag;
  const int ky = (int)tap / p.KW, kx = (int)tap - ky * p.KW;
  const int dy = p.dy0 + ky, dx = p.dx0 + kx + p.gpx * ag;
  const int lds2 = p.lds * 2;
  const int a_lane_off = (dy * p.Ws + (p.dx0 + kx)) * lds2 + ag * 16;
  const int b_k = B_RPI * wid + lane / B_SLOTS;
  const int b_slot = lane % B_SLOTS;
  const int b_sw = BN == 128 ? ((b_k & 3) << 1) : (((b_k >> 1) & 1) << 1);
  const int b_g = ((((b_slot >> 1) ^ b_sw) << 1) | (b_slot & 1));
  const int nbq = (n0 >> 3) + b_g;
  const bool b_ok = nbq * 8 < p.Cb;
  const int b_lane_off = nbq * 16;
  const int ldd2 = p.ldd * 2;
  const unsigned magW = (unsigned)((0x100000000ull + p.Wg - 1) / p.Wg), magH = (unsigned)((0x100000000ull + p.Hg - 1) / p.Hg);

  const unsigned lds0 = lds_addr(smem16);
  auto a_voff = [&](int kt) {
    const unsigned sidx = (unsigned)(kt * KS + a_k);
    const unsigned q = fast_div(sidx, magW);
    const int xg = (int)(sidx - q * (unsigned)p.Wg);
    const unsigned bb = fast_div(q, magH);
    const int yg = (int)(q - bb * (unsigned)p.Hg);
    const int yb = yg * p.sm, xb = xg * p.sm;
    const bool ok = m_ok && (int)bb < p.B && (unsigned)(yb + dy) < (unsigned)p.Hs && (unsigned)(xb + dx) < (unsigned)p.Ws;
    return ok ? (((int)bb * p.Hs + yb) * p.Ws + xb) * lds2 + a_lane_off : OOB_MARK;
  };
  auto b_voff = [&](int kt) {
    const int sidx = kt * KS + b_k;
    return (b_ok && sidx < S) ? sidx * ldd2 + b_lane_off : OOB_MARK;
  };
  auto issue = [&](int kt, int buf) {
    const unsigned st = lds0 + (unsigned)(buf * STAGE * 2);
    const unsigned d = st + (unsigned)(4 * wid * BM * 2);
    if constexpr (F16) {
#pragma unroll
      for (int g = 0; g < 3; g++) dma1(a_voff(3 * kt + g), src_rs[0], d + g * A_PLANE * 2);
    } else {
      dma3(a_voff(kt), src_rs[0], src_rs[1], src_rs[2], d, d + A_PLANE * 2, d + 2 * A_PLANE * 2);
    }
    if (wid < B_NI) {
      const unsigned e = st + (unsigned)((NPL * A_PLANE + B_RPI * wid * BN) * 2);
      if constexpr (F16) {
#pragma unroll
        for (int g = 0; g < 3; g++) dma1(b_voff(3 * kt + g), dst_rs[0], e + g * B_PLANE * 2);
      } else {
        dma3(b_voff(kt), dst_rs[0], dst_rs[1], dst_rs[2], e, e + B_PLANE * 2, e + 2 * B_PLANE * 2);
      }
    }
  };

  f32x16 acc[TM][TN];
#pragma unroll
  for (int i = 0; i < TM; i++)
#pragma unroll
    for (int j = 0; j < TN; j++)
#pragma unroll
      for (int r = 0; r < 16; r++) acc[i][j][r] = 0.f;

  const int i16 = lane & 15, grp16 = lane >> 4, lh = grp16 >> 1;
  const int krow = 8 * lh + (i16 >> 2);
  int a_rd[TM], b_rd[TN];
#pragma unroll
  for (int i = 0; i < TM; i++) {
    const int c = wm * WM + i * 32 + 16 * (grp16 & 1) + 4 * (i16 & 3);
    a_rd[i] = tr_swz<BM>(krow, c >> 3) + (c & 7);
  }
#pragma unroll
  for (int j = 0; j < TN; j++) {
    const int c = wn * WN + j * 32 + 16 * (grp16 & 1) + 4 * (i16 & 3);
    b_rd[j] = NPL * A_PLANE + tr_swz<BN>(krow, c >> 3) + (c & 7);
  }
  if (kt0 < kt1) issue(kt0, 0);
  asm volatile("s_waitcnt vmcnt(0)" ::: "memory");
  __builtin_amdgcn_s_barrier();
  __builtin_amdgcn_sched_barrier(0);
  PHASE_DECL;
  for (int kt = kt0; kt < kt1; kt++) {
    PHASE_STAMP(6);
    const int cur = (kt - kt0) & 1;
    const unsigned short* st = smem16 + cur * STAGE;
    s16x8 av[TM][NPL], bv[TN][NPL];
    auto read_a = [&](int pl) {
#pragma unroll
      for (int i = 0; i < TM; i++) {
        const unsigned short* b0 = st + pl * A_PLANE + a_rd[i];
        const s16x4 lo = __builtin_amdgcn_ds_read_tr16_b64_v4i16((s16x4 __attribute__((address_space(3)))*)(b0));
        const s16x4 hi = __builtin_amdgcn_ds_read_tr16_b64_v4i16((s16x4 __attribute__((address_space(3)))*)(b0 + 4 * BM));
        av[i][pl] = __builtin_shufflevector(lo, hi, 0, 1, 2, 3, 4, 5, 6, 7);
      }
    };
    auto read_b = [&](int pl) {
#pragma unroll
      for (int j = 0; j < TN; j++) {
        const unsigned short* b0 = st + pl * B_PLANE + b_rd[j];
        const s16x4 lo = __builtin_amdgcn_ds_read_tr16_b64_v4i16((s16x4 __attribute__((address_space(3)))*)(b0));
        const s16x4 hi = __builtin_amdgcn_ds_read_tr16_b64_v4i16((s16x4 __attribute__((address_space(3)))*)(b0 + 4 * BN));
        bv[j][pl] = __builtin_shufflevector(lo, hi, 0, 1, 2, 3, 4, 5, 6, 7);
      }
    };
    read_a(2); read_b(0); read_a(0); read_b(2); read_a(1); read_b(1);
    __builtin_amdgcn_sched_barrier(0);
    PHASE_STAMP(4);
    const int ktn = kt + 1 < kt1 ? kt + 1 : KT + 1;
    const unsigned stn = lds0 + (unsigned)((cur ^ 1) * STAGE * 2);
    const unsigned da = stn + (unsigned)(4 * wid * BM * 2);
    const unsigned db = stn + (unsigned)((NPL * A_PLANE + B_RPI * wid * BN) * 2);
    auto group = [&](int t) {
#pragma unroll
      for (int i = 0; i < TM; i++)
#pragma unroll
        for (int j = 0; j < TN; j++) mfma_terms<NPL, F16>(av[i], bv[j], acc[i][j], t);
    };
    if constexpr (F16) {
      const int voa0 = a_voff(3 * ktn), voa1 = a_voff(3 * ktn + 1), voa2 = a_voff(3 * ktn + 2);
      const int vob0 = b_voff(3 * ktn), vob1 = b_voff(3 * ktn + 1), vob2 = b_voff(3 * ktn + 2);
      dma1(voa0, src_rs[0], da);
      dma1(voa1, src_rs[0], da + A_PLANE * 2);
      __builtin_amdgcn_sched_barrier(0);
      PHASE_STAMP(0);
      group(0);
      __builtin_amdgcn_sched_barrier(0);
      dma1(voa2, src_rs[0], da + 2 * A_PLANE * 2);
      if (wid < B_NI) dma1(vob0, dst_rs[0], db);
      __builtin_amdgcn_sched_barrier(0);
      group(1);
      __builtin_amdgcn_sched_barrier(0);
      if (wid < B_NI) {
        dma1(vob1, dst_rs[0], db + B_PLANE * 2);
        dma1(vob2, dst_rs[0], db + 2 * B_PLANE * 2);
      }
      __builtin_amdgcn_sched_barrier(0);
      group(2);
    } else {
      const int voa = a_voff(ktn);
      const int vob = b_voff(ktn);
      dma1(voa, src_rs[0], da);
      dma1(voa, src_rs[1], da + A_PLANE * 2);
      __builtin_amdgcn_sched_barrier(0);
      PHASE_STAMP(0);
      group(0);
      __builtin_amdgcn_sched_barrier(0);
      dma1(voa, src_rs[2], da + 2 * A_PLANE * 2);
      if (wid < B_NI) dma1(vob, dst_rs[0], db);
      __builtin_amdgcn_sched_barrier(0);
      group(1);
      __builtin_amdgcn_sched_barrier(0);
      if (wid < B_NI) {
        dma1(vob, dst_rs[1], db + B_PLANE * 2);
        dma1(vob, dst_rs[2], db + 2 * B_PLANE * 2);
      }
      __builtin_amdgcn_sched_barrier(0);
      group(2);
      group(3);
      group(4);
      group(5);
    }
    __builtin_amdgcn_sched_barrier(0);
    PHASE_STAMP(1);
    asm volatile("s_waitcnt vmcnt(0) lgkmcnt(0)" ::: "memory");
    PHASE_STAMP(2);
    __builtin_amdgcn_s_barrier();
    __builtin_amdgcn_sched_barrier(0);
    PHASE_STAMP(3);
  }
  PHASE_FLUSH;

  float* o = p.nsplit > 1 ? p.partial + (size_t)split * taps * p.Ca_out * p.Cb : p.out;
  const int lh5 = lane >> 5, l31 = lane & 31;
#pragma unroll
  for (int i = 0; i < TM; i++)
#pragma unroll
    for (int r = 0; r < 16; r++) {
      const int m = m0 + wm * WM + i * 32 + (r & 3) + 8 * (r >> 2) + 4 * lh5;
      const int mgr = m >> 3;
      if (mgr >= Mg) continue;
      const unsigned tp = p.cag_magic ? fast_div((unsigned)mgr, p.cag_magic) : (unsigned)mgr;
      const int a = (mgr - (int)tp * Cag) * 8 + (m & 7);
      if (a >= p.Ca_out) continue;
      float* orow = o + ((size_t)tp * p.Ca_out + a) * p.Cb;
#pragma unroll
      for (int j = 0; j < TN; j++) {
        const int n = n0 + wn * WN + j * 32 + l31;
        if (n < p.Cb) orow[n] = acc[i][j][r] * p.out_scale;
      }
    }
}

template <int BN, bool F16 = false>
__global__ __launch_bounds__(512, 1) void igemm_pl_wgrad_pp_kernel(const PlWgradParams p, int grp_mode) {
  constexpr int BM = 256, WM = BN == 256 ? 128 : 64, WN = 64, NPL = 3, NT = F16 ? 3 : 6, KS = 16;
  constexpr int GPS = F16 ? 3 : 1;
  constexpr int TM = WM / 32, TN = WN / 32;
  constexpr int A_HALF = KS * 128;
  constexpr int A_PLANE = 2 * A_HALF, B_PLANE = KS * BN;
  constexpr int STAGE = NPL * (A_PLANE + B_PLANE);
  constexpr int NSTAGE = 3;
  extern __shared__ __attribute__((aligned(16))) unsigned short smem16[];

  const int lane = threadIdx.x & 63;
  const int wid = __builtin_amdgcn_readfirstlane((int)(threadIdx.x >> 6));
  const int grp = grp_mode == 0 ? (wid >> 2) : (wid & 1);
  const int idx = grp_mode == 0 ? (wid & 3) : (wid >> 1);
  const int wmq = BN == 256 ? 2 * grp : idx, wn = BN == 256 ? idx : grp;
  const int taps = p.KH * p.KW;
  const int Cag = p.Ca >> 3;
  const int Mg = taps * Cag;
  int v = xcd_remap(blockIdx.x, gridDim.x, p.xcd);
  const int mtile = v % p.mt; v /= p.mt;
  const int ntile = v % p.nt;
  const int split = v / p.nt;
  const int m0 = mtile * BM, n0 = ntile * BN;
  const int S = p.B * p.Hg * p.Wg;
  const int KT = ((S + KS - 1) / KS + GPS - 1) / GPS;
  const int kt_per = F16 ? (KT + p.nsplit - 1) / p.nsplit : (((KT + 1) / 2 + p.nsplit - 1) / p.nsplit) * 2;
  const int kt0 = split * kt_per, kt1 = min(KT, kt0 + kt_per);
  const int n = max(kt1 - kt0, 0);

  u32x4 src_rs[NPL], dst_rs[NPL];
#pragma unroll
  for (int pl = 0; pl < NPL; pl++) {
    src_rs[pl] = raw_rsrc(p.src + (F16 ? 0 : pl * p.src_ps), (((size_t)p.B * p.Hs * p.Ws - 1) * (size_t)p.lds + (size_t)(p.gpx ? p.lds : p.Ca)) * 2);
    dst_rs[pl] = raw_rsrc(p.dst + (F16 ? 0 : pl * p.dst_ps), (((size_t)S - 1) * (size_t)p.ldd + (size_t)((p.Cb + 7) & ~7)) * 2);
  }
  const int dh = wid >> 2, dq = wid & 3;
  const int a_k = 4 * dq + (lane >> 4);
  const int a_slot = lane & 15;
  const int a_g = ((((a_slot >> 1) ^ ((a_k & 3) << 1)) << 1) | (a_slot & 1));
  const int mg = (m0 >> 3) + 16 * dh + a_g;
  const bool m_ok = mg < Mg;
  const unsigned tap = p.cag_magic ? fast_div((unsigned)mg, p.cag_magic) : (unsigned)mg;
  const int ag = mg - (int)tap * Cag;
  const int ky = (int)tap / p.KW, kx = (int)tap - ky * p.KW;
  const int dy = p.dy0 + ky, dx = p.dx0 + kx + p.gpx * ag;
  const int lds2 = p.lds * 2;
  const int a_lane_off = (dy * p.Ws + (p.dx0 + kx)) * lds2 + ag * 16;
  const int b_k = 4 * dq + (lane >> 4);
  const int b_slot = lane & 15;
  const int b_g = ((((b_slot >> 1) ^ ((b_k & 3) << 1)) << 1) | (b_slot & 1));
  const int nbq = (n0 >> 3) + (BN == 256 ? 16 * dh : 0) + b_g;
  const bool b_ok = nbq * 8 < p.Cb;
  const int b_lane_off = nbq * 16;
  const int ldd2 = p.ldd * 2;
  const unsigned magW = (unsigned)((0x100000000ull + p.Wg - 1) / p.Wg), magH = (unsigned)((0x100000000ull + p.Hg - 1) / p.Hg);
  const unsigned lds0 = lds_addr(smem16);
  auto a_voff = [&](int kt) {
    const unsigned sidx = (unsigned)(kt * KS + a_k);
    const unsigned q = fast_div(sidx, magW);
    const int xg = (int)(sidx - q * (unsigned)p.Wg);
    const unsigned bb = fast_div(q, magH);
    const int yg = (int)(q - bb * (unsigned)p.Hg);
    const int yb = yg * p.sm, xb = xg * p.sm;
    const bool ok = m_ok && (int)bb < p.B && (unsigned)(yb + dy) < (unsigned)p.Hs && (unsigned)(xb + dx) < (unsigned)p.Ws;
    return ok ? (((int)bb * p.Hs + yb) * p.Ws + xb) * lds2 + a_lane_off : OOB_MARK;
  };
  auto b_voff = [&](int kt) {
    const int sidx = kt * KS + b_k;
    return (b_ok && sidx < S) ? sidx * ldd2 + b_lane_off : OOB_MARK;
  };
  auto load_a = [&](int kt, unsigned da) {
    if constexpr (F16) {
#pragma unroll
      for (int g = 0; g < 3; g++) dma1(a_voff(3 * kt + g), src_rs[0], da + g * A_PLANE * 2);
    } else {
      dma3(a_voff(kt), src_rs[0], src_rs[1], src_rs[2], da, da + A_PLANE * 2, da + 2 * A_PLANE * 2);
    }
  };
  auto load_b = [&](int kt, unsigned db) {
    if constexpr (F16) {
#pragma unroll
      for (int g = 0; g < 3; g++) dma1(b_voff(3 * kt + g), dst_rs[0], db + g * B_PLANE * 2);
    } else {
      dma3(b_voff(kt), dst_rs[0], dst_rs[1], dst_rs[2], db, db + B_PLANE * 2, db + 2 * B_PLANE * 2);
    }
  };
  auto issue = [&](int x) {
    const int kt = x < n ? kt0 + x : KT + 1;
    const unsigned st = lds0 + (unsigned)((x % NSTAGE) * STAGE * 2);
    const unsigned da = st + (unsigned)((dh * A_HALF + 4 * dq * 128) * 2);
    load_a(kt, da);
    if (BN == 256 || wid < 4) {
      const unsigned db = st + (unsigned)((NPL * A_PLANE + (BN == 256 ? dh * A_HALF : 0) + 4 * dq * 128) * 2);
      load_b(kt, db);
    }
  };
  auto wait_older = [&]() {
    if (BN == 256 || wid < 4) asm volatile("s_waitcnt vmcnt(6)" ::: "memory");
    else asm volatile("s_waitcnt vmcnt(3)" ::: "memory");
  };

  f32x16 acc[TM][TN];
#pragma unroll
  for (int i = 0; i < TM; i++)
#pragma unroll
    for (int j = 0; j < TN; j++)
#pragma unroll
      for (int r = 0; r < 16; r++) acc[i][j][r] = 0.f;

  const int i16 = lane & 15, grp16 = lane >> 4, lh = grp16 >> 1;
  const int krow = 8 * lh + (i16 >> 2);
  int a_rd[TM], b_rd[TN];
#pragma unroll
  for (int i = 0; i < TM; i++) {
    const int c = (BN == 256 ? 0 : (wmq & 1) * 64) + i * 32 + 16 * (grp16 & 1) + 4 * (i16 & 3);
    a_rd[i] = (wmq >> 1) * A_HALF + tr_swz<128>(krow, c >> 3) + (c & 7);
  }
#pragma unroll
  for (int j = 0; j < TN; j++) {
    const int c = (BN == 256 ? (wn & 1) : wn) * WN + j * 32 + 16 * (grp16 & 1) + 4 * (i16 & 3);
    b_rd[j] = NPL * A_PLANE + (BN == 256 ? (wn >> 1) * A_HALF : 0) + tr_swz<128>(krow, c >> 3) + (c & 7);
  }

  constexpr int HALVES = TM / 2;
  s16x8 av[2][NPL], bv[TN][NPL];
  auto read_frags = [&](int x, int half) {
    const unsigned short* st = smem16 + (x % NSTAGE) * STAGE;
    auto read_a = [&](int pl) {
#pragma unroll
      for (int i = 0; i < 2; i++) {
        const unsigned short* b0 = st + pl * A_PLANE + a_rd[2 * half + i];
        const s16x4 lo = __builtin_amdgcn_ds_read_tr16_b64_v4i16((s16x4 __attribute__((address_space(3)))*)(b0));
        const s16x4 hi = __builtin_amdgcn_ds_read_tr16_b64_v4i16((s16x4 __attribute__((address_space(3)))*)(b0 + 4 * 128));
        av[i][pl] = __builtin_shufflevector(lo, hi, 0, 1, 2, 3, 4, 5, 6, 7);
      }
    };
    auto read_b = [&](int pl) {
#pragma unroll
      for (int j = 0; j < TN; j++) {
        const unsigned short* b0 = st + pl * B_PLANE + b_rd[j];
        const s16x4 lo = __builtin_amdgcn_ds_read_tr16_b64_v4i16((s16x4 __attribute__((address_space(3)))*)(b0));
        const s16x4 hi = __builtin_amdgcn_ds_read_tr16_b64_v4i16((s16x4 __attribute__((address_space(3)))*)(b0 + 4 * 128));
        bv[j][pl] = __builtin_shufflevector(lo, hi, 0, 1, 2, 3, 4, 5, 6, 7);
      }
    };
    if (half == 0) { read_a(2); read_b(0); read_a(0); read_b(2); read_a(1); read_b(1); }
    else { read_a(2); read_a(0); read_a(1); }
    __builtin_amdgcn_sched_barrier(0);
  };
  auto issue_part = [&](int x, int part) {
    const int kt = x < n ? kt0 + x : KT + 1;
    const unsigned st = lds0 + (unsigned)((x % NSTAGE) * STAGE * 2);
    if (part == 0 || HALVES == 1) {
      const unsigned da = st + (unsigned)((dh * A_HALF + 4 * dq * 128) * 2);
      load_a(kt, da);
    }
    if ((part == HALVES - 1) && (BN == 256 || wid < 4)) {
      const unsigned db = st + (unsigned)((NPL * A_PLANE + (BN == 256 ? dh * A_HALF : 0) + 4 * dq * 128) * 2);
      load_b(kt, db);
    }
    __builtin_amdgcn_sched_barrier(0);
  };
  auto multiply = [&](int half) {
    __builtin_amdgcn_s_setprio(1);
#pragma unroll
    for (int t = 0; t < NT; t++)
#pragma unroll
      for (int i = 0; i < 2; i++)
#pragma unroll
        for (int j = 0; j < TN; j++) {
          if (half == 0) mfma_terms<NPL, F16>(av[i], bv[j], acc[i][j], t);
          else mfma_terms<NPL, F16>(av[i], bv[j], acc[(TM > 2 ? 2 : 0) + i][j], t);
        }
    __builtin_amdgcn_s_setprio(0);
    __builtin_amdgcn_sched_barrier(0);
  };

  if (n > 0) {
    issue(0);
    issue(1);
    wait_older();
    __builtin_amdgcn_s_barrier();
    __builtin_amdgcn_sched_barrier(0);
    auto slot_end = [&]() {
      __builtin_amdgcn_sched_barrier(0);
      __builtin_amdgcn_s_barrier();
      __builtin_amdgcn_sched_barrier(0);
    };
    if (grp == 1) slot_end();
    PHASE_DECL;
#pragma unroll 1
    for (int x = 0; x < n; x++) {
      PHASE_STAMP(6);
      read_frags(x, 0);
      issue_part(x + 2, 0);
      if (HALVES == 1) {
        asm volatile("s_waitcnt lgkmcnt(0)" ::: "memory");
        wait_older();
      }
      PHASE_STAMP(0);
      slot_end();
      PHASE_STAMP(1);
      multiply(0);
      PHASE_STAMP(2);
      slot_end();
      PHASE_STAMP(3);
      if (HALVES == 2) {
        read_frags(x, 1);
        issue_part(x + 2, 1);
        asm volatile("s_waitcnt lgkmcnt(0)" ::: "memory");
        wait_older();
        slot_end();
        PHASE_STAMP(4);
        multiply(1);
        slot_end();
      }
    }
    PHASE_FLUSH;
    if (grp == 0) slot_end();
    asm volatile("s_waitcnt vmcnt(0)" ::: "memory");
  }

  float* o = p.nsplit > 1 ? p.partial + (size_t)split * taps * p.Ca_out * p.Cb : p.out;
  const int lh5 = lane >> 5, l31 = lane & 31;
#pragma unroll
  for (int i = 0; i < TM; i++)
#pragma unroll
    for (int r = 0; r < 16; r++) {
      const int m = m0 + wmq * 64 + i * 32 + (r & 3) + 8 * (r >> 2) + 4 * lh5;
      const int mgr = m >> 3;
      if (mgr >= Mg) continue;
      const unsigned tp = p.cag_magic ? fast_div((unsigned)mgr, p.cag_magic) : (unsigned)mgr;
      const int a = (mgr - (int)tp * Cag) * 8 + (m & 7);
      if (a >= p.Ca_out) continue;
      float* orow = o + ((size_t)tp * p.Ca_out + a) * p.Cb;
#pragma unroll
      for (int j = 0; j < TN; j++) {
        const int nn = n0 + wn * WN + j * 32 + l31;
        if (nn < p.Cb) orow[nn] = acc[i][j][r] * p.out_scale;
      }
    }
}

__global__ void planes_from_f32_kernel(const float* __restrict__ x, int ldx, long npix, int C, int Cp, PlaneOut o) {
  const int nq = Cp >> 2;
  const long total = npix * nq;
  for (long e = blockIdx.x * (long)blockDim.x + threadIdx.x; e < total; e += (long)gridDim.x * blockDim.x) {
    const long px = e / nq;
    const int n = (int)(e - px * nq) * 4;
    float4 v = make_float4(0.f, 0.f, 0.f, 0.f);
    const float* s = x + px * ldx + n;
    if (n < C) v.x = s[0];
    if (n + 1 < C) v.y = s[1];
    if (n + 2 < C) v.z = s[2];
    if (n + 3 < C) v.w = s[3];
    store_planes4(o, (size_t)px, n, v);
  }
}

struct WPlaneDesc {
  const float* w;
  unsigned short* direct;
  unsigned short* transposed;
  int taps, R, Cc;
  int tiles_r, tiles_c;
  int block0;
};
constexpr int MAX_WDESC = 64;
struct WPlaneBatch {
  WPlaneDesc d[MAX_WDESC];
  int n, n_planes;
};

__device__ __forceinline__ void put_planes8(unsigned short* base, long ps, int n_planes, size_t idx, const float (&v)[8]) {
  if (n_planes == 1) {
    u32x4 o;
#pragma unroll
    for (int i = 0; i < 4; i++) o[i] = (unsigned)to_f16_bits(v[2 * i]) | ((unsigned)to_f16_bits(v[2 * i + 1]) << 16);
    __builtin_nontemporal_store(o, reinterpret_cast<u32x4*>(base + idx));
    return;
  }
  u32x4 h, m, l;
#pragma unroll
  for (int i = 0; i < 4; i++) {
    const float a = v[2 * i], b = v[2 * i + 1];
    const unsigned hh = cvt_pk_bf16(a, b);
    const float ra = a - __uint_as_float(hh << 16), rb = b - __uint_as_float(hh & 0xffff0000u);
    const unsigned mm = cvt_pk_bf16(ra, rb);
    const float sa = ra - __uint_as_float(mm << 16), sb = rb - __uint_as_float(mm & 0xffff0000u);
    h[i] = hh; m[i] = mm; l[i] = cvt_pk_bf16(sa, sb);
  }
  __builtin_nontemporal_store(h, reinterpret_cast<u32x4*>(base + idx));
  __builtin_nontemporal_store(m, reinterpret_cast<u32x4*>(base + idx + ps));
  __builtin_nontemporal_store(l, reinterpret_cast<u32x4*>(base + idx + 2 * ps));
}

__global__ __launch_bounds__(256) void weight_planes_kernel(const WPlaneBatch b) {
  __shared__ float tile[64][65];
  int di = 0;
  while (di + 1 < b.n && (int)blockIdx.x >= b.d[di + 1].block0) di++;
  const WPlaneDesc d = b.d[di];
  int lb = blockIdx.x - d.block0;
  const int tc = lb % d.tiles_c; lb /= d.tiles_c;
  const int tr = lb % d.tiles_r; lb /= d.tiles_r;
  const int tap = lb;
  const int r0 = tr * 64, c0 = tc * 64;
  const int Cc8 = (d.Cc + 7) & ~7, R8 = (d.R + 7) & ~7;
  const float* w = d.w + (size_t)tap * d.R * d.Cc;
  for (int e = threadIdx.x; e < 64 * 64; e += 256) {
    const int r = e >> 6, c = e & 63;
    tile[r][c] = (r0 + r < d.R && c0 + c < d.Cc) ? w[(size_t)(r0 + r) * d.Cc + c0 + c] : 0.f;
  }
  __syncthreads();
  if (d.direct) {
    const long ps = (long)d.taps * d.R * Cc8;
    for (int e = threadIdx.x; e < 64 * 8; e += 256) {
      const int r = e >> 3, c8 = (e & 7) * 8;
      if (r0 + r >= d.R || c0 + c8 >= Cc8) continue;
      float v[8];
#pragma unroll
      for (int i = 0; i < 8; i++) v[i] = tile[r][c8 + i];
      put_planes8(d.direct, ps, b.n_planes, ((size_t)tap * d.R + r0 + r) * Cc8 + c0 + c8, v);
    }
  }
  if (d.transposed) {
    const long ps = (long)d.taps * d.Cc * R8;
    for (int e = threadIdx.x; e < 64 * 8; e += 256) {
      const int r8 = (e & 7) * 8, c = e >> 3;
      if (c0 + c >= d.Cc || r0 + r8 >= R8) continue;
      float v[8];
#pragma unroll
      for (int i = 0; i < 8; i++) v[i] = tile[r8 + i][c];
      put_planes8(d.transposed, ps, b.n_planes, ((size_t)tap * d.Cc + c0 + c) * R8 + r0 + r8, v);
    }
  }
}

struct AdamPlaneArgs {
  float* P; const float* G; float* M; float* V;
  float gscale, l2, lr_t, b1, b2, eps;
  float* loss_acc;
};

__global__ __launch_bounds__(256) void adam_planes_kernel(const WPlaneBatch b, const AdamPlaneArgs a, const unsigned long long reg_mask) {
  __shared__ float tile[64][65];
  __shared__ float red[4];
  int di = 0;
  while (di + 1 < b.n && (int)blockIdx.x >= b.d[di + 1].block0) di++;
  const WPlaneDesc d = b.d[di];
  const bool reg = (reg_mask >> di) & 1ull;
  int lb = blockIdx.x - d.block0;
  const int tc = lb % d.tiles_c; lb /= d.tiles_c;
  const int tr = lb % d.tiles_r; lb /= d.tiles_r;
  const int tap = lb;
  const int r0 = tr * 64, c0 = tc * 64;
  const int Cc8 = (d.Cc + 7) & ~7, R8 = (d.R + 7) & ~7;
  const size_t base = (size_t)(d.w - a.P) + (size_t)tap * d.R * d.Cc;
  float sq = 0.f;
  const bool vec = (d.Cc & 3) == 0 && (base & 3) == 0;
  if (vec) {
    for (int e = threadIdx.x; e < 64 * 16; e += 256) {
      const int r = e >> 4, c = (e & 15) * 4;
      float pv[4] = {0.f, 0.f, 0.f, 0.f};
      if (r0 + r < d.R && c0 + c < d.Cc) {
        const size_t i = base + (size_t)(r0 + r) * d.Cc + c0 + c;
        const f32x4_nt pq = *reinterpret_cast<const f32x4_nt*>(a.P + i);
        const f32x4_nt gq = __builtin_nontemporal_load(reinterpret_cast<const f32x4_nt*>(a.G + i));
        f32x4_nt mq = __builtin_nontemporal_load(reinterpret_cast<const f32x4_nt*>(a.M + i));
        f32x4_nt vq = __builtin_nontemporal_load(reinterpret_cast<const f32x4_nt*>(a.V + i));
        f32x4_nt po;
#pragma unroll
        for (int j = 0; j < 4; j++) {
          float gr = gq[j] * a.gscale;
          if (reg) {
            gr += a.l2 * pq[j];
            sq += pq[j] * pq[j];
          }
          mq[j] = a.b1 * mq[j] + (1.f - a.b1) * gr;
          vq[j] = a.b2 * vq[j] + (1.f - a.b2) * (gr * gr);
          po[j] = pq[j] - a.lr_t * mq[j] / (sqrtf(vq[j]) + a.eps);
          pv[j] = po[j];
        }
        *reinterpret_cast<f32x4_nt*>(a.P + i) = po;
        __builtin_nontemporal_store(mq, reinterpret_cast<f32x4_nt*>(a.M + i));
        __builtin_nontemporal_store(vq, reinterpret_cast<f32x4_nt*>(a.V + i));
      }
#pragma unroll
      for (int j = 0; j < 4; j++) tile[r][c + j] = pv[j];
// ... 139 lines not shown
  const int M = p.B * p.Hg * p.Wg;
  constexpr int smem = 6 * 3 * 128 * 32 * 2 + 2 * 128 * 4;
  static DynLdsBook attr_book{};
  (void)ensure_dyn_lds(reinterpret_cast<const void*>(&igemm_pl_gather_pp_kernel<3, false>), smem, attr_book);
  PlGatherParams q = p;
  q.mt = cdiv(M, 128); q.nt = cdiv(p.N, 128);
  pl_gather_tiles2d<128>(q);
  if (q.tw_log) q.mt = q.B * q.tiles_y * q.tiles_x;
  q.mt = cdiv(q.mt, 2);
  const int grid = pl_grid(q);
  igemm_pl_gather_pp_kernel<3, false><<<grid, 512, smem, st>>>(q);
  return launch_status();
}

template <int NPL, bool F16>
int run_pl_gather_mode(PlGatherParams& p, int cfg, hipStream_t st) {
  switch (cfg) {
    case 0: return launch_pl_gather<128, 128, 64, 64, NPL, F16>(p, st);
    case 1: return launch_pl_gather<128, 64, 64, 32, NPL, F16>(p, st);
    default: return launch_pl_gather<64, 64, 32, 32, NPL, F16>(p, st);
  }
}

inline bool pl_halo_ok(const GatherGeom& p) {
  const bool off = !unflow::options().halo;
  if (off || p.sm != 1 || (p.dstep != 1 && p.dstep != -1) || p.Hg < 2 * TH || p.Wg < TW || p.N <= 32) return false;
  if (p.acc && (p.dstep != 1 || !unflow::options().halo_s2)) return false;
  for (int c = 0; c < p.ncls; c++)
    if (p.cls[c].nty < 1 || p.cls[c].ntx < 1) return false;
  return pl_halo_pixels(p) <= 256;
}
inline bool pl_halo_acc_pays(const GatherGeom& a) {
  if (!a.acc || !pl_halo_ok(a)) return false;
  const int bn = a.N <= 64 ? 64 : 128;
  const long tiles = (long)a.B * cdiv(a.Hg, TH) * cdiv(a.Wg, TW) * cdiv(a.N, bn);
  return tiles >= 384 || unflow::options().halo_s2 >= 2;
}

constexpr int F16_KCH = 2;
inline int f16_kch(const GatherGeom& p, int npl) {
  if (npl != 1) return 1;
  const int o = unflow::options().f16_k64;
  if (o >= 2) return F16_KCH;
  if (o <= 0) return 1;
  int sum = 0;
  bool four = true;
  for (int c = 0; c < p.ncls; c++) {
    sum += p.cls[c].nty * p.cls[c].ntx;
    four = four && p.cls[c].nty * p.cls[c].ntx == 4;
  }
  return (p.acc ? sum <= 9 : (p.ncls == 4 && four)) ? F16_KCH : 1;
}
inline bool f16_tall(const GatherGeom& p, int npl) {
  const int o = unflow::options().f16_tall;
  if (npl != 1 || o <= 0 || f16_kch(p, npl) != 1 || p.N <= 64 || p.Hg < TALL_TH || pl_halo_pixels(p, TALL_TH) > 384) return false;
  if (o >= 2) return true;
  const long tiles = (long)p.B * cdiv(p.Hg, TALL_TH) * cdiv(p.Wg, TW) * cdiv(p.N, 128) * pl_grid_classes(p);
  return tiles >= 512;
}
inline int plan_pl_halo(const GatherGeom& p, int npl, int* bn_out, bool* tall_out = nullptr) {
  const int bn = p.N <= 64 ? 64 : 128;
  const bool tall = f16_tall(p, npl);
  if (tall_out) *tall_out = tall;
  const int th = tall ? TALL_TH : TH;
  *bn_out = bn;
  const int kch = f16_kch(p, npl);
  const int nbuf = (npl == 1 && kch == 1 && unflow::options().f16_db > 0) ? 2 : 1;
  const int smem = pl_halo_main_bytes(bn, bn >= 128 ? 64 : 32, npl == 1 ? kch : npl, pl_halo_pixels(p, th), nbuf) + th * 32 * 4 + 16;
  const int per_cu = min((160 * 1024) / smem, bn >= 128 ? 2 : 3);
  const long blocks = (long)p.B * cdiv(p.Hg, th) * cdiv(p.Wg, TW) * cdiv(p.N, bn) * pl_grid_classes(p);
  const int nchunk = ((((p.Cs >> 3) + 3) >> 2) + kch - 1) / kch;
  int maxtaps = 0, sumtaps = 0;
  for (int c = 0; c < p.ncls; c++) {
    maxtaps = max(maxtaps, p.cls[c].nty * p.cls[c].ntx);
    sumtaps += p.cls[c].nty * p.cls[c].ntx;
  }
  if (p.acc) maxtaps = sumtaps;
  const int max_by_k = max(1, min(min(16, max(1, unflow::options().halo_max_split)), nchunk * maxtaps / 16));
  return min(nchunk, fill_one_round(blocks, 256 * per_cu, max_by_k));
}

template <int BN, int WN, int NPL, bool F16, int WM = 64, bool DB = false>
int launch_pl_halo(const PlGatherParams& p, hipStream_t st) {
  const int hp = pl_halo_pixels(p);
  const int smem = pl_halo_main_bytes(BN, WN, NPL, hp, DB ? 2 : 1) + 128 * 4 + 16;
  static DynLdsBook book{};
  (void)ensure_dyn_lds(reinterpret_cast<const void*>(&igemm_pl_halo_kernel<BN, WM, WN, NPL, F16, DB>), smem, book);
  PlGatherParams q = p;
  if (F16 && NPL > 1) q.src_ps = q.w_ps = 32;
  q.mt = p.B * p.tiles_y * p.tiles_x; q.nt = cdiv(p.N, BN);
  const int grid = pl_grid(q);
  igemm_pl_halo_kernel<BN, WM, WN, NPL, F16, DB><<<grid, 256, smem, st>>>(q, hp);
  return launch_status();
}

int run_pl_gather(PlGatherParams& p, int npl, void* ws, size_t ws_bytes, hipStream_t st) {
  const unflow::Options& opt = unflow::options();
  if (p.src_inv == 0.f) p.src_inv = 1.f;
  p.xcd = opt.xcd_swizzle;
  p.order = 2;
  const bool halo = pl_halo_ok(p);
  int halo_bn = 128;
  bool tall = false;
  PlPlan pl = plan_pl_gather(p, npl);
  if (halo) {
    pl.nsplit = plan_pl_halo(p, npl, &halo_bn, &tall);
    p.tiles_y = cdiv(p.Hg, TH);
    p.tiles_x = cdiv(p.Wg, TW);
  }
  p.nsplit = pl.nsplit;
  p.partial = nullptr;
  if (p.nsplit > 1) {
    if (!ws || ws_bytes < pl_gather_partial_bytes(p, p.nsplit)) p.nsplit = 1;
    else p.partial = reinterpret_cast<float*>(ws);
  }
  {
    const uintptr_t al = reinterpret_cast<uintptr_t>(p.dst) | reinterpret_cast<uintptr_t>(p.partial) |
                         reinterpret_cast<uintptr_t>(p.act_src) | (p.pl.n_planes ? reinterpret_cast<uintptr_t>(p.pl.base) * 2 : 0) |
                         reinterpret_cast<uintptr_t>(p.act_pl) * 2;
    p.vec_epi = p.N % 4 == 0 && (!p.dst || p.ldd % 4 == 0) && ((!p.act_src && !p.act_pl) || p.ld_act % 4 == 0) && (al & 15) == 0 &&
                (!p.pl.n_planes || p.pl.ld % 4 == 0);
    if (!p.dst && (!p.vec_epi || p.accumulate || !p.pl.n_planes)) return UNFLOW_ERR_UNSUPPORTED;
  }
  if (halo && p.vec_epi && pl_halo_sk_ok(p, npl, halo_bn) && ws && ws_bytes >= pl_halo_sk_ws_bytes())
    return launch_pl_halo_sk(p, ws, ws_bytes, st);
  int code;
  if (halo) {
    if (npl == 3) code = halo_bn == 128 ? launch_pl_halo<128, 64, 3, false>(p, st) : launch_pl_halo<64, 32, 3, false>(p, st);
    else if (tall) code = launch_pl_halo_f16_tall(p, st);
    else if (f16_kch(p, npl) == 1 && opt.f16_db > 0)
      code = halo_bn == 128 ? launch_pl_halo<128, 64, 1, true, 64, true>(p, st) : launch_pl_halo<64, 32, 1, true, 64, true>(p, st);
    else if (f16_kch(p, npl) == 1) code = halo_bn == 128 ? launch_pl_halo<128, 64, 1, true>(p, st) : launch_pl_halo<64, 32, 1, true>(p, st);
    else code = halo_bn == 128 ? launch_pl_halo<128, 64, F16_KCH, true>(p, st) : launch_pl_halo<64, 32, F16_KCH, true>(p, st);
  } else {
    code = pl.pp ? launch_pl_gather_pp(p, st) : npl == 3 ? run_pl_gather_mode<3, false>(p, pl.cfg, st) : run_pl_gather_mode<1, true>(p, pl.cfg, st);
  }
  if (code != UNFLOW_OK) return code;
  if (p.nsplit > 1) {
    const size_t total = (size_t)p.B * p.Hd * p.Wd * p.N;
    pl_splitk_reduce_epilogue_kernel<<<stream_grid((long)(p.vec_epi ? total / 4 : total)), 256, 0, st>>>(p, p.vec_epi);
    return launch_status();
  }
  return UNFLOW_OK;
}

inline int pl_wgrad_cfg(const WgradGeom& p) { return p.Cb <= 64 ? 1 : 0; }

inline bool pl_wgrad_pp_ok(const WgradGeom& p, int npl) {
  const int o = unflow::options().wgrad_pp;
  if (o <= 0 || !(npl == 3 || (npl == 1 && unflow::options().f16_wgrad_dma >= 2)) || p.Cb <= 64 || p.KH * p.KW * p.Ca < 256) return false;
  if (o >= 3) return true;
  return p.Cb > 128 && (long)p.B * p.Hg * p.Wg >= 1536;
}
inline int pl_wgrad_pp_bn(const WgradGeom& p) { return p.Cb > 128 ? 256 : 128; }

inline int plan_pl_wgrad(const WgradGeom& p, int npl) {
  const int Mp = p.KH * p.KW * p.Ca;
  if (pl_wgrad_pp_ok(p, npl)) {
    const long blocks = (long)cdiv(Mp, 256) * cdiv(p.Cb, pl_wgrad_pp_bn(p));
    const long S = (long)p.B * p.Hg * p.Wg;
    const int KT = (int)((S + BK - 1) / BK);
    const int min_kt = max(1, unflow::options().wgrad_min_kt);
    return fill_one_round(blocks, 256, min(256, KT / min_kt > 0 ? KT / min_kt : 1));
  }
  const int cfg = pl_wgrad_cfg(p);
  const int bn = cfg == 1 ? 64 : 128;
  const long blocks = (long)cdiv(Mp, 128) * cdiv(p.Cb, bn);
  const long S = (long)p.B * p.Hg * p.Wg;
  const int KT = (int)((S + BK - 1) / BK);
  const int min_kt = max(1, unflow::options().wgrad_min_kt) * (npl == 1 ? 4 : 1);
  const int max_by_k = min(256, KT / min_kt > 0 ? KT / min_kt : 1);
  const int per_cu = min((160 * 1024) / (npl * (128 + bn) * BK * 2), cfg == 1 ? 4 : 3);
  return fill_one_round(blocks, 256 * per_cu, max_by_k);
}

inline size_t pl_wgrad_partial_bytes(const WgradGeom& p, int ca_out, int nsplit) {
  const size_t n = (size_t)p.KH * p.KW * ca_out * p.Cb;
  return nsplit > 1 ? (size_t)nsplit * n * sizeof(float) + reduce_scratch_bytes(n, nsplit) : 0;
}
inline size_t pl_wgrad_plan_bytes(const WgradGeom& p, int ca_out, int npl) {
  return pl_wgrad_partial_bytes(p, ca_out, plan_pl_wgrad(p, npl));
}

template <int BM, int BN, int WM, int WN, int NPL, bool F16>
int launch_pl_wgrad(const PlWgradParams& p, hipStream_t st) {
  const int Mp = p.KH * p.KW * p.Ca;
  const int smem = NPL * (BM + BN) * BK * 2;
  static DynLdsBook attr_book{};
  (void)ensure_dyn_lds(reinterpret_cast<const void*>(&igemm_pl_wgrad_kernel<BM, BN, WM, WN, NPL, F16>), smem, attr_book);
  PlWgradParams q = p;
  q.mt = cdiv(Mp, BM); q.nt = cdiv(p.Cb, BN);
  igemm_pl_wgrad_kernel<BM, BN, WM, WN, NPL, F16><<<q.mt * q.nt * p.nsplit, 256, smem, st>>>(q);
  return launch_status();
}

template <int BN, int WN, bool F16 = false>
int launch_pl_wgrad_dma(const PlWgradParams& p, hipStream_t st) {
  const int Mp = p.KH * p.KW * p.Ca;
  const int smem = 2 * 3 * (128 + BN) * 16 * 2;
  static DynLdsBook attr_book{};
  (void)ensure_dyn_lds(reinterpret_cast<const void*>(&igemm_pl_wgrad_dma_kernel<BN, WN, F16>), smem, attr_book);
  PlWgradParams q = p;
  q.mt = cdiv(Mp, 128); q.nt = cdiv(p.Cb, BN);
  igemm_pl_wgrad_dma_kernel<BN, WN, F16><<<q.mt * q.nt * p.nsplit, 256, smem, st>>>(q);
  return launch_status();
}

template <int BN, bool F16 = false>
int launch_pl_wgrad_pp(const PlWgradParams& p, hipStream_t st) {
  const int Mp = p.KH * p.KW * p.Ca;
  const int smem = 3 * 3 * (256 + BN) * 16 * 2;
  static DynLdsBook attr_book{};
  (void)ensure_dyn_lds(reinterpret_cast<const void*>(&igemm_pl_wgrad_pp_kernel<BN, F16>), smem, attr_book);
  PlWgradParams q = p;
  q.mt = cdiv(Mp, 256); q.nt = cdiv(p.Cb, BN);
  igemm_pl_wgrad_pp_kernel<BN, F16><<<q.mt * q.nt * p.nsplit, 512, smem, st>>>(q, (unflow::options().wgrad_pp & 1) ? 0 : 1);
  return launch_status();
}

int run_pl_wgrad(PlWgradParams& p, int npl, void* ws, size_t ws_bytes, size_t* used, hipStream_t st) {
  const unflow::Options& opt = unflow::options();
  if (p.out_scale == 0.f) p.out_scale = 1.f;
  p.xcd = opt.xcd_swizzle;
  p.cag_magic = p.Ca == 8 ? 0u : magic_u32((unsigned)(p.Ca >> 3));
  const size_t wsize = (size_t)p.KH * p.KW * p.Ca_out * p.Cb;
  int ns = plan_pl_wgrad(p, npl);
  if (ns > 1 && (!ws || ws_bytes < pl_wgrad_partial_bytes(p, p.Ca_out, ns))) {
    ns = ws ? (int)min((size_t)REDUCE_FAN, ws_bytes / (wsize * sizeof(float))) : 1;
    if (ns < 1) ns = 1;
  }
  p.nsplit = ns;
  p.partial = ns > 1 ? reinterpret_cast<float*>(ws) : nullptr;
  *used = pl_wgrad_partial_bytes(p, p.Ca_out, ns);
  const int cfg = pl_wgrad_cfg(p);
  int code;
  if (pl_wgrad_pp_ok(p, npl) && npl == 1) code = pl_wgrad_pp_bn(p) == 256 ? launch_pl_wgrad_pp<256, true>(p, st) : launch_pl_wgrad_pp<128, true>(p, st);
  else if (pl_wgrad_pp_ok(p, npl)) code = pl_wgrad_pp_bn(p) == 256 ? launch_pl_wgrad_pp<256>(p, st) : launch_pl_wgrad_pp<128>(p, st);
  else if (npl == 3 && opt.wgrad_dma) code = cfg == 1 ? launch_pl_wgrad_dma<64, 32>(p, st) : launch_pl_wgrad_dma<128, 64>(p, st);
  else if (npl == 3) code = cfg == 1 ? launch_pl_wgrad<128, 64, 64, 32, 3, false>(p, st) : launch_pl_wgrad<128, 128, 64, 64, 3, false>(p, st);
  else if (opt.wgrad_dma && opt.f16_wgrad_dma) code = cfg == 1 ? launch_pl_wgrad_dma<64, 32, true>(p, st) : launch_pl_wgrad_dma<128, 64, true>(p, st);
  else code = cfg == 1 ? launch_pl_wgrad<128, 64, 64, 32, 1, true>(p, st) : launch_pl_wgrad<128, 128, 64, 64, 1, true>(p, st);
  if (code != UNFLOW_OK) return code;
  if (ns > 1) return reduce_partials(p.partial, p.partial + (size_t)ns * wsize, p.out, wsize, ns, st);
  return UNFLOW_OK;
}

inline bool planes_ok(const unflow_planes* t, int channels) {
  return t && t->base && (t->n_planes == 1 || t->n_planes == 3) && t->ld % 4 == 0 && t->ld >= ((channels + 7) & ~7) &&
         (reinterpret_cast<uintptr_t>(t->base) & 7) == 0;
}

inline PlaneOut plane_out(const unflow_planes* t, int lo, int hi) {
  PlaneOut o{};
  if (t && t->base && t->n_planes) {
    o.base = reinterpret_cast<unsigned short*>(t->base);
    o.plane_stride = t->plane_stride;
    o.ld = t->ld;
    o.lo = lo;
    o.hi = hi;
    o.n_planes = t->n_planes;
    o.scale = t->n_planes == 1 ? t->scale : 0.f;
  }
  return o;
}
inline float plane_scale(const unflow_planes* t) { return (t && t->n_planes == 1 && t->scale != 0.f) ? t->scale : 1.f; }

inline void set_act(PlGatherParams& p, const float* act_src, int ld_act, const unflow_planes* act_pl) {
  p.act_src = act_src; p.ld_act = ld_act; p.act_pl = nullptr;
  if (!act_src && act_pl && act_pl->base) {
    p.act_pl = reinterpret_cast<const unsigned short*>(act_pl->base);
    p.ld_act = act_pl->ld;
  }
}

}

int unflow_conv2d_fwd_po(const float* x, int ldx, const float* w, const float* bias, float* y, int ldy, int B, int H, int W,
                         int Cin, int Cout, int k, int stride, int leaky, const igemm::PlaneOut& po, void* workspace,
                         size_t workspace_bytes, unflow_stream_t stream);
int unflow_conv2d_bwd_data_po(const float* dz, int lddz, const float* w, float* dx, int lddx, int B, int H, int W, int Cin,
                              int Cout, int k, int stride, int accumulate, const float* act_src, int ld_act, int act_lo,
                              int act_hi, const igemm::PlaneOut& po, void* workspace, size_t workspace_bytes,
                              unflow_stream_t stream);
int unflow_conv2d_transpose_fwd_po(const float* x, int ldx, const float* w, const float* bias, float* y, int ldy, int B, int H,
                                   int W, int Cin, int Cout, int leaky, const igemm::PlaneOut& po, void* workspace,
                                   size_t workspace_bytes, unflow_stream_t stream);
int unflow_conv2d_transpose_bwd_data_po(const float* dz, int lddz, const float* w, float* dx, int lddx, int B, int H, int W,
                                        int Cin, int Cout, int accumulate, const float* act_src, int ld_act, int act_lo,
                                        int act_hi, const igemm::PlaneOut& po, void* workspace, size_t workspace_bytes,
                                        unflow_stream_t stream);

UNFLOW_API int unflow_debug_work_order(int mt, int nt, int ncls, int nsplit, int order, int xcd, int* out, int out_blocks) {
  if (mt <= 0 || nt <= 0 || ncls <= 0 || nsplit <= 0 || order < 0 || order > 2) return UNFLOW_ERR_SHAPE;
  PlGatherParams q{};
  q.mt = mt; q.nt = nt; q.ncls = ncls; q.nsplit = nsplit; q.order = order;
  const int grid = pl_grid(q);
  if (!out) return grid;
  if (out_blocks < grid) return UNFLOW_ERR_WORKSPACE;
  for (int b = 0; b < grid; b++) {
    int m, n, c, sp;
    work_decode(xcd_remap(b, grid, xcd), mt, nt, ncls, nsplit, order, q.mgroup, m, n, c, sp);
    out[4 * b] = m; out[4 * b + 1] = n; out[4 * b + 2] = c; out[4 * b + 3] = sp;
  }
  return grid;
}

#ifdef UNFLOW_PHASE_TRACE
UNFLOW_API int unflow_debug_phase_trace(unsigned long long* host_out, int clear) {
  if (clear) {
    static unsigned long long zero[8 * 8];
    return hipMemcpyToSymbol(HIP_SYMBOL(g_phase_trace), zero, sizeof(zero)) == hipSuccess ? UNFLOW_OK : UNFLOW_ERR_LAUNCH;
  }
  return hipMemcpyFromSymbol(host_out, HIP_SYMBOL(g_phase_trace), sizeof(unsigned long long) * 8 * 8) == hipSuccess ? UNFLOW_OK
                                                                                                                       : UNFLOW_ERR_LAUNCH;
}
#endif

UNFLOW_API int unflow_planes_from_f32(const float* x, int ldx, long npix, int C, int C_fill, const unflow_planes* out,
                                      unflow_stream_t stream) {
  if (!x || !out || !out->base) return UNFLOW_ERR_NULL;
  if (npix <= 0 || C <= 0) return UNFLOW_OK;
  const int Cp = (C_fill + 3) & ~3;
  if ((out->n_planes != 1 && out->n_planes != 3) || out->ld % 4 != 0 || (reinterpret_cast<uintptr_t>(out->base) & 7) != 0 ||
      ldx < C || Cp < C || Cp > ((C + 7) & ~7) || out->ld < Cp)
    return UNFLOW_ERR_UNSUPPORTED;
  planes_from_f32_kernel<<<stream_grid(npix * (Cp / 4)), 256, 0, as_stream(stream)>>>(x, ldx, npix, C, Cp, plane_out(out, 0, Cp));
  return launch_status();
}

UNFLOW_API size_t unflow_weight_planes_elems(int taps, int R, int Cc, int transposed) {
  return transposed ? (size_t)taps * Cc * ((R + 7) & ~7) : (size_t)taps * R * ((Cc + 7) & ~7);
}

UNFLOW_API int unflow_weight_planes_batched(int n, const float* const* w, const int* taps, const int* R, const int* Cc,
                                            void* const* direct, void* const* transposed, int n_planes,
                                            unflow_stream_t stream) {
  if (!w || !taps || !R || !Cc || !direct || !transposed) return UNFLOW_ERR_NULL;
  if (n_planes != 1 && n_planes != 3) return UNFLOW_ERR_UNSUPPORTED;
  hipStream_t st = as_stream(stream);
  for (int i0 = 0; i0 < n; i0 += MAX_WDESC) {
    WPlaneBatch b{};
    b.n = min(n - i0, MAX_WDESC);
    b.n_planes = n_planes;
    int blocks = 0;
    for (int i = 0; i < b.n; i++) {
      WPlaneDesc& d = b.d[i];
      if (!w[i0 + i] || taps[i0 + i] <= 0 || R[i0 + i] <= 0 || Cc[i0 + i] <= 0) return UNFLOW_ERR_SHAPE;
      d.w = w[i0 + i];
      d.direct = reinterpret_cast<unsigned short*>(direct[i0 + i]);
      d.transposed = reinterpret_cast<unsigned short*>(transposed[i0 + i]);
      d.taps = taps[i0 + i]; d.R = R[i0 + i]; d.Cc = Cc[i0 + i];
      d.tiles_r = cdiv((d.R + 7) & ~7, 64);
      d.tiles_c = cdiv((d.Cc + 7) & ~7, 64);
      d.block0 = blocks;
      blocks += d.taps * d.tiles_r * d.tiles_c;
    }
    if (blocks > 0) weight_planes_kernel<<<blocks, 256, 0, st>>>(b);
  }
  return launch_status();
}

UNFLOW_API int unflow_adam_planes_batched(int n, float* const* w, const int* taps, const int* R, const int* Cc, void* const* direct,
                                          void* const* transposed, const int* regularized, int n_planes, float* P, const float* G,
                                          float* M, float* V, float grad_scale, float l2_scale, float lr_t, float beta1, float beta2,
                                          float eps, float* loss_acc, unflow_stream_t stream) {
  if (!w || !taps || !R || !Cc || !direct || !transposed || !regularized || !P || !G || !M || !V) return UNFLOW_ERR_NULL;
  if (n_planes != 0 && n_planes != 1 && n_planes != 3) return UNFLOW_ERR_UNSUPPORTED;
  hipStream_t st = as_stream(stream);
  AdamPlaneArgs a{P, G, M, V, grad_scale, l2_scale, lr_t, beta1, beta2, eps, loss_acc};
  for (int i0 = 0; i0 < n; i0 += MAX_WDESC) {
    WPlaneBatch b{};
    b.n = min(n - i0, MAX_WDESC);
    b.n_planes = n_planes ? n_planes : 3;
    unsigned long long reg_mask = 0;
    int blocks = 0;
    for (int i = 0; i < b.n; i++) {
      WPlaneDesc& d = b.d[i];
      if (!w[i0 + i] || taps[i0 + i] <= 0 || R[i0 + i] <= 0 || Cc[i0 + i] <= 0 || w[i0 + i] < P) return UNFLOW_ERR_SHAPE;
      if (!n_planes && (direct[i0 + i] || transposed[i0 + i])) return UNFLOW_ERR_UNSUPPORTED;
      d.w = w[i0 + i];
      d.direct = reinterpret_cast<unsigned short*>(direct[i0 + i]);
      d.transposed = reinterpret_cast<unsigned short*>(transposed[i0 + i]);
      d.taps = taps[i0 + i]; d.R = R[i0 + i]; d.Cc = Cc[i0 + i];
      d.tiles_r = cdiv(d.R, 64);
      d.tiles_c = cdiv(d.Cc, 64);
      d.block0 = blocks;
      blocks += d.taps * d.tiles_r * d.tiles_c;
      if (regularized[i0 + i]) reg_mask |= 1ull << i;
    }
    if (blocks > 0) adam_planes_kernel<<<blocks, 256, 0, st>>>(b, a, reg_mask);
  }
  return launch_status();
}

static int pl_gather_nsplit(const GatherGeom& g, int npl) {
  int bn;
  if (!pl_halo_ok(g)) return plan_pl_gather(g, npl).nsplit;
  return plan_pl_halo(g, npl, &bn);
}

UNFLOW_API size_t unflow_conv_pl_workspace_bytes(int B, int H, int W, int Cin, int Cout, int k, int stride, int n_planes) {
  if (B <= 0 || H <= 0 || W <= 0 || Cin <= 0 || Cout <= 0 || k <= 0 || stride <= 0) return 0;
  size_t need = unflow_conv_workspace_bytes(B, H, W, (Cin + 3) & ~3, Cout, k, stride);
  if (Cout <= 4 || (n_planes != 1 && n_planes != 3)) return need;
  const int Ci8 = (Cin + 7) & ~7, Co8 = (Cout + 7) & ~7;
  GatherGeom g{};
  build_conv_fwd(g, B, H, W, Ci8, Cout, k, stride);
  need = max(need, pl_gather_partial_bytes(g, pl_gather_nsplit(g, n_planes)));
  if (unflow::options().streamk > 0 && n_planes == 3) need = max(need, pl_halo_sk_ws_bytes());
  if (stride == 2 && build_conv_fwd_s2acc(g, B, H, W, Ci8, Cout, k) && pl_halo_acc_pays(g))
    need = max(need, pl_gather_partial_bytes(g, pl_gather_nsplit(g, n_planes)));
  GatherGeom d{};
  if ((stride == 1 || stride == 2) && build_conv_dgrad(d, B, H, W, Cin, Co8, k, stride) == UNFLOW_OK)
    need = max(need, pl_gather_partial_bytes(d, pl_gather_nsplit(d, n_planes)));
  WgradGeom wg{};
  build_conv_wgrad(wg, B, H, W, Ci8, Cout, k, stride);
  need = max(need, pl_wgrad_plan_bytes(wg, Cin, n_planes));
  if (Cin == 4 && k == 7 && stride == 2 && W % 2 == 0) {
    g.Cs = 32; g.KW = 1; g.wtaps = 7; g.cls[0].ntx = 1;
    need = max(need, pl_gather_partial_bytes(g, pl_gather_nsplit(g, n_planes)));
    wg.Ca = 32; wg.KW = 1;
    need = max(need, pl_wgrad_plan_bytes(wg, 28, n_planes));
  }
  if (k == 4 && stride == 2 && H % 2 == 0 && W % 2 == 0) {
    GatherGeom tf{};
    build_deconv_fwd(tf, B, H / 2, W / 2, Ci8, Cout);
    need = max(need, pl_gather_partial_bytes(tf, pl_gather_nsplit(tf, n_planes)));
    GatherGeom td{};
    build_deconv_dgrad(td, B, H / 2, W / 2, Cin, Co8);
    need = max(need, pl_gather_partial_bytes(td, pl_gather_nsplit(td, n_planes)));
    build_deconv_dgrad_acc(td, B, H / 2, W / 2, Cin, Co8);
    if (pl_halo_acc_pays(td)) need = max(need, pl_gather_partial_bytes(td, pl_gather_nsplit(td, n_planes)));
    WgradGeom tw{};
    build_deconv_wgrad(tw, B, H / 2, W / 2, Cin, Co8);
    need = max(need, pl_wgrad_plan_bytes(tw, Cout, n_planes));
  }
  return need + 1024;
}

int conv_first7_fwd(const unflow_planes* x_pl, const unflow_planes* w_pl, const float* bias, const unflow_planes* y_pl, int B, int H,
                    int W, int Cout, int leaky, hipStream_t st);

static bool rgb4_form(const unflow_planes* x_pl, int W, int Cin, int k, int stride) {
  return x_pl && x_pl->base && Cin == 4 && k == 7 && stride == 2 && x_pl->ld == 4 && W % 2 == 0 &&
         (x_pl->n_planes == 1 || x_pl->n_planes == 3) && (reinterpret_cast<uintptr_t>(x_pl->base) & 7) == 0;
}

static bool use_planes(const unflow_planes* a, int ca, const unflow_planes* b, int cb, int Cout_or_n) {
  return Cout_or_n > 4 && planes_ok(a, ca) && planes_ok(b, cb) && a->n_planes == b->n_planes;
}

UNFLOW_API int unflow_conv2d_fwd_pl(const float* x, int ldx, const unflow_planes* x_pl, const float* w,
                                    const unflow_planes* w_pl, const float* bias, float* y, int ldy,
                                    const unflow_planes* y_pl, int B, int H, int W, int Cin, int Cout, int k, int stride,
                                    int leaky, void* workspace, size_t workspace_bytes, unflow_stream_t stream) {
  if ((!y && !(y_pl && y_pl->base)) || (!x && !x_pl)) return UNFLOW_ERR_NULL;
  if (B <= 0 || H <= 0 || W <= 0 || Cin <= 0 || Cout <= 0 || k <= 0 || stride <= 0) return UNFLOW_ERR_SHAPE;
  const int Ci8 = (Cin + 7) & ~7;
  const bool rgb4 = rgb4_form(x_pl, W, Cin, k, stride) && Cout > 4 && planes_ok(w_pl, 28) && w_pl->ld == 32 &&
                    w_pl->n_planes == x_pl->n_planes;
  if (!rgb4 && (!use_planes(x_pl, Cin, w_pl, Cin, Cout) || w_pl->ld != Ci8))
    return !y ? UNFLOW_ERR_UNSUPPORTED : unflow_conv2d_fwd_po(x, ldx, w, bias, y, ldy, B, H, W, Cin, Cout, k, stride, leaky, plane_out(y_pl, 0, Cout), workspace,
                                workspace_bytes, stream);
  if (y && ldy < Cout) return UNFLOW_ERR_UNSUPPORTED;
  if (rgb4 && !y) {
    const int code = conv_first7_fwd(x_pl, w_pl, bias, y_pl, B, H, W, Cout, leaky, as_stream(stream));
    if (code != UNFLOW_ERR_UNSUPPORTED) return code;
  }
  PlGatherParams p{};
  build_conv_fwd(p, B, H, W, Ci8, Cout, k, stride);
  if (stride == 2 && !rgb4) {
    GatherGeom a{};
    if (build_conv_fwd_s2acc(a, B, H, W, Ci8, Cout, k) && pl_halo_acc_pays(a)) static_cast<GatherGeom&>(p) = a;
  }
  if (rgb4) {
    p.Cs = 32; p.KW = 1; p.wtaps = 7; p.gpx = 2;
    p.cls[0].ntx = 1;
  }
  p.src = reinterpret_cast<const unsigned short*>(x_pl->base); p.src_ps = x_pl->plane_stride; p.lds = x_pl->ld;
  p.w = reinterpret_cast<const unsigned short*>(w_pl->base); p.w_ps = w_pl->plane_stride;
  p.src_inv = 1.f / (plane_scale(x_pl) * plane_scale(w_pl));
  p.bias = bias; p.dst = y; p.ldd = ldy; p.act_src = nullptr; p.leaky = leaky; p.accumulate = 0;
  p.pl = plane_out(y_pl, 0, Cout);
  return run_pl_gather(p, x_pl->n_planes, workspace, workspace_bytes, as_stream(stream));
}

UNFLOW_API int unflow_conv2d_bwd_data_pl(const float* dz, int lddz, const unflow_planes* dz_pl, const float* w,
                                         const unflow_planes* w_pl, float* dx, int lddx, const unflow_planes* dx_pl,
                                         int pl_lo, int pl_hi, int B, int H, int W, int Cin, int Cout, int k, int stride,
                                         int accumulate, const float* act_src, int ld_act, const unflow_planes* act_pl,
                                         int act_lo, int act_hi, void* workspace, size_t workspace_bytes,
                                         unflow_stream_t stream) {
  if ((!dx && !(dx_pl && dx_pl->base)) || (!dz && !dz_pl)) return UNFLOW_ERR_NULL;
  if (B <= 0 || H <= 0 || W <= 0 || Cin <= 0 || Cout <= 0 || k <= 0 || (stride != 1 && stride != 2)) return UNFLOW_ERR_SHAPE;
  const int Co8 = (Cout + 7) & ~7;
  const bool pointwise32 = k == 1 && stride == 1 && Cout == 32;
  if (pointwise32 || !use_planes(dz_pl, Cout, w_pl, Cout, Cout) || w_pl->ld != Co8)
    return (!dx || (!act_src && act_pl && act_hi > act_lo)) ? UNFLOW_ERR_UNSUPPORTED : unflow_conv2d_bwd_data_po(dz, lddz, w, dx, lddx, B, H, W, Cin, Cout, k, stride, accumulate, act_src, ld_act, act_lo,
                                     act_hi, plane_out(dx_pl, pl_lo, pl_hi), workspace, workspace_bytes, stream);
  if (dx && lddx < Cin) return UNFLOW_ERR_UNSUPPORTED;
  PlGatherParams p{};
  const int bc = build_conv_dgrad(p, B, H, W, Cin, Co8, k, stride);
  if (bc != UNFLOW_OK) return bc;
  p.src = reinterpret_cast<const unsigned short*>(dz_pl->base); p.src_ps = dz_pl->plane_stride; p.lds = dz_pl->ld;
  p.w = reinterpret_cast<const unsigned short*>(w_pl->base); p.w_ps = w_pl->plane_stride;
  p.src_inv = 1.f / (plane_scale(dz_pl) * plane_scale(w_pl));
  p.bias = nullptr; p.dst = dx; p.ldd = lddx; p.act_lo = act_lo; p.act_hi = act_hi;
  set_act(p, act_src, ld_act, act_pl);
  p.leaky = 0; p.accumulate = accumulate;
  p.pl = plane_out(dx_pl, pl_lo, pl_hi);
  return run_pl_gather(p, dz_pl->n_planes, workspace, workspace_bytes, as_stream(stream));
}

UNFLOW_API int unflow_conv2d_bwd_filter_pl(const float* x, int ldx, const unflow_planes* x_pl, const float* dz, int lddz,
                                           const unflow_planes* dz_pl, float* dw, int B, int H, int W, int Cin, int Cout,
                                           int k, int stride, void* workspace, size_t workspace_bytes,
                                           unflow_stream_t stream) {
  if (!dw || (!x && !x_pl) || (!dz && !dz_pl)) return UNFLOW_ERR_NULL;
  if (B <= 0 || H <= 0 || W <= 0 || Cin <= 0 || Cout <= 0 || k <= 0 || stride <= 0) return UNFLOW_ERR_SHAPE;
  const bool rgb4 = rgb4_form(x_pl, W, Cin, k, stride) && planes_ok(dz_pl, Cout) && dz_pl->n_planes == x_pl->n_planes &&
                    Cout > 4 && Cout % 4 == 0;
  if (!rgb4 && (!use_planes(x_pl, Cin, dz_pl, Cout, Cout) || Cout % 4 != 0))
    return (!x || !dz) ? UNFLOW_ERR_UNSUPPORTED :
           unflow_conv2d_bwd_filter(x, ldx, dz, lddz, dw, nullptr, B, H, W, Cin, Cout, k, stride, workspace, workspace_bytes, stream);
  PlWgradParams p{};
  build_conv_wgrad(p, B, H, W, (Cin + 7) & ~7, Cout, k, stride);
  if (rgb4) { p.Ca = 32; p.KW = 1; p.gpx = 2; }
  p.src = reinterpret_cast<const unsigned short*>(x_pl->base); p.src_ps = x_pl->plane_stride; p.lds = x_pl->ld;
  p.dst = reinterpret_cast<const unsigned short*>(dz_pl->base); p.dst_ps = dz_pl->plane_stride; p.ldd = dz_pl->ld;
  p.out_scale = 1.f / (plane_scale(x_pl) * plane_scale(dz_pl));
  p.out = dw; p.Ca_out = rgb4 ? 28 : Cin;
  size_t used = 0;
  return run_pl_wgrad(p, x_pl->n_planes, workspace, workspace_bytes, &used, as_stream(stream));
}

UNFLOW_API int unflow_conv2d_transpose_fwd_pl(const float* x, int ldx, const unflow_planes* x_pl, const float* w,
                                              const unflow_planes* w_pl, const float* bias, float* y, int ldy,
                                              const unflow_planes* y_pl, int B, int H, int W, int Cin, int Cout, int leaky,
                                              void* workspace, size_t workspace_bytes, unflow_stream_t stream) {
  if ((!y && !(y_pl && y_pl->base)) || (!x && !x_pl)) return UNFLOW_ERR_NULL;
  if (B <= 0 || H <= 0 || W <= 0 || Cin <= 0 || Cout <= 0) return UNFLOW_ERR_SHAPE;
  const int Ci8 = (Cin + 7) & ~7;
  if (!use_planes(x_pl, Cin, w_pl, Cin, Cout) || w_pl->ld != Ci8)
    return !y ? UNFLOW_ERR_UNSUPPORTED : unflow_conv2d_transpose_fwd_po(x, ldx, w, bias, y, ldy, B, H, W, Cin, Cout, leaky, plane_out(y_pl, 0, Cout), workspace,
                                          workspace_bytes, stream);
  if (y && ldy < Cout) return UNFLOW_ERR_UNSUPPORTED;
  PlGatherParams p{};
  build_deconv_fwd(p, B, H, W, Ci8, Cout);
  p.src = reinterpret_cast<const unsigned short*>(x_pl->base); p.src_ps = x_pl->plane_stride; p.lds = x_pl->ld;
  p.w = reinterpret_cast<const unsigned short*>(w_pl->base); p.w_ps = w_pl->plane_stride;
  p.src_inv = 1.f / (plane_scale(x_pl) * plane_scale(w_pl));
  p.bias = bias; p.dst = y; p.ldd = ldy; p.act_src = nullptr; p.leaky = leaky; p.accumulate = 0;
  p.pl = plane_out(y_pl, 0, Cout);
  return run_pl_gather(p, x_pl->n_planes, workspace, workspace_bytes, as_stream(stream));
}

UNFLOW_API int unflow_conv2d_transpose_bwd_data_pl(const float* dz, int lddz, const unflow_planes* dz_pl, const float* w,
                                                   const unflow_planes* w_pl, float* dx, int lddx,
                                                   const unflow_planes* dx_pl, int pl_lo, int pl_hi, int B, int H, int W,
                                                   int Cin, int Cout, int accumulate, const float* act_src, int ld_act,
                                                   const unflow_planes* act_pl, int act_lo, int act_hi, void* workspace,
                                                   size_t workspace_bytes, unflow_stream_t stream) {
  if ((!dx && !(dx_pl && dx_pl->base)) || (!dz && !dz_pl)) return UNFLOW_ERR_NULL;
  if (B <= 0 || H <= 0 || W <= 0 || Cin <= 0 || Cout <= 0) return UNFLOW_ERR_SHAPE;
  const int Co8 = (Cout + 7) & ~7;
  if (!use_planes(dz_pl, Cout, w_pl, Cout, Cout) || w_pl->ld != Co8 || Cin <= 4)
    return (!dx || (!act_src && act_pl && act_hi > act_lo)) ? UNFLOW_ERR_UNSUPPORTED : unflow_conv2d_transpose_bwd_data_po(dz, lddz, w, dx, lddx, B, H, W, Cin, Cout, accumulate, act_src, ld_act, act_lo,
                                               act_hi, plane_out(dx_pl, pl_lo, pl_hi), workspace, workspace_bytes, stream);
  if (dx && lddx < Cin) return UNFLOW_ERR_UNSUPPORTED;
  PlGatherParams p{};
  build_deconv_dgrad(p, B, H, W, Cin, Co8);
  {
    GatherGeom a{};
    build_deconv_dgrad_acc(a, B, H, W, Cin, Co8);
    if (pl_halo_acc_pays(a)) static_cast<GatherGeom&>(p) = a;
  }
  p.src = reinterpret_cast<const unsigned short*>(dz_pl->base); p.src_ps = dz_pl->plane_stride; p.lds = dz_pl->ld;
  p.w = reinterpret_cast<const unsigned short*>(w_pl->base); p.w_ps = w_pl->plane_stride;
  p.src_inv = 1.f / (plane_scale(dz_pl) * plane_scale(w_pl));
  p.bias = nullptr; p.dst = dx; p.ldd = lddx; p.act_lo = act_lo; p.act_hi = act_hi;
  set_act(p, act_src, ld_act, act_pl);
  p.leaky = 0; p.accumulate = accumulate;
  p.pl = plane_out(dx_pl, pl_lo, pl_hi);
  return run_pl_gather(p, dz_pl->n_planes, workspace, workspace_bytes, as_stream(stream));
}

UNFLOW_API int unflow_conv2d_transpose_bwd_filter_pl(const float* x, int ldx, const unflow_planes* x_pl, const float* dz,
                                                     int lddz, const unflow_planes* dz_pl, float* dw, int B, int H, int W,
                                                     int Cin, int Cout, void* workspace, size_t workspace_bytes,
                                                     unflow_stream_t stream) {
  if (!dw || (!x && !x_pl) || (!dz && !dz_pl)) return UNFLOW_ERR_NULL;
  if (B <= 0 || H <= 0 || W <= 0 || Cin <= 0 || Cout <= 0) return UNFLOW_ERR_SHAPE;
  if (!use_planes(x_pl, Cin, dz_pl, Cout, Cout) || Cin % 4 != 0 || Cin <= 4)
    return (!x || !dz) ? UNFLOW_ERR_UNSUPPORTED :
           unflow_conv2d_transpose_bwd_filter(x, ldx, dz, lddz, dw, nullptr, B, H, W, Cin, Cout, workspace, workspace_bytes, stream);
  PlWgradParams p{};
  build_deconv_wgrad(p, B, H, W, Cin, (Cout + 7) & ~7);
  p.src = reinterpret_cast<const unsigned short*>(dz_pl->base); p.src_ps = dz_pl->plane_stride; p.lds = dz_pl->ld;
  p.dst = reinterpret_cast<const unsigned short*>(x_pl->base); p.dst_ps = x_pl->plane_stride; p.ldd = x_pl->ld;
  p.out_scale = 1.f / (plane_scale(x_pl) * plane_scale(dz_pl));
  p.out = dw; p.Ca_out = Cout;
  size_t used = 0;
  return run_pl_wgrad(p, x_pl->n_planes, workspace, workspace_bytes, &used, as_stream(stream));
}
```

### unflow_amd/csrc/igemm_shared.h

```cpp
#pragma once
#include <stdlib.h>
#include <cstdint>
#include <cstring>
#include "common.h"

typedef float f32x16 __attribute__((ext_vector_type(16)));
typedef unsigned int u32x4 __attribute__((ext_vector_type(4)));

namespace igemm {

constexpr int BK = 32;

struct TapClass {
  int nty, ntx;
  int dy0, dx0;
  int ky0, kx0;
  int py, px;
};

struct GatherGeom {
  int B, Hg, Wg, Hs, Ws, sm;
  int dstep, kstep, KW;
  int Cs, N;
  int Hd, Wd, so;
// ... 185 lines not shown
inline void build_conv_fwd(GatherGeom& p, int B, int H, int W, int Cin, int Cout, int k, int stride) {
  int pt, pl, Ho, Wo;
  same_pads(H, k, stride, &pt, &Ho);
  same_pads(W, k, stride, &pl, &Wo);
  p.B = B; p.Hg = Ho; p.Wg = Wo; p.Hs = H; p.Ws = W; p.sm = stride;
  p.dstep = 1; p.kstep = 1; p.KW = k; p.Cs = Cin; p.N = Cout; p.wtaps = k * k;
  p.Hd = Ho; p.Wd = Wo; p.so = 1; p.ncls = 1; p.sp = 1; p.acc = 0;
  p.cls[0] = TapClass{k, k, -pt, -pl, 0, 0, 0, 0};
}

inline bool build_conv_fwd_s2acc(GatherGeom& p, int B, int H, int W, int Cin, int Cout, int k) {
  if (k < 2) return false;
  build_conv_fwd(p, B, H, W, Cin, Cout, k, 2);
  const int pt = -p.cls[0].dy0, pl = -p.cls[0].dx0;
  p.sm = 1; p.sp = 2; p.acc = 1; p.ncls = 4; p.kstep = 2; p.dstep = 1;
  for (int c = 0; c < 4; c++) {
    const int py = c >> 1, px = c & 1;
    const int nty = (k - py + 1) / 2, ntx = (k - px + 1) / 2;
    if (nty < 1 || ntx < 1) return false;
    p.cls[c] = TapClass{nty, ntx, py - pt, px - pl, py, px, 0, 0};
  }
  return true;
}

inline int build_conv_dgrad(GatherGeom& p, int B, int H, int W, int Cin, int Cout, int k, int stride) {
  int pt, pl, Ho, Wo;
  same_pads(H, k, stride, &pt, &Ho);
  same_pads(W, k, stride, &pl, &Wo);
  p.B = B; p.Hs = Ho; p.Ws = Wo; p.sm = 1;
  p.dstep = -1; p.KW = k; p.Cs = Cout; p.N = Cin; p.wtaps = k * k;
  p.Hd = H; p.Wd = W; p.sp = 1; p.acc = 0;
  if (stride == 1) {
    p.Hg = H; p.Wg = W; p.so = 1; p.ncls = 1; p.kstep = 1;
    p.cls[0] = TapClass{k, k, pt, pl, 0, 0, 0, 0};
    return UNFLOW_OK;
  }
  if (H % 2 != 0 || W % 2 != 0) return UNFLOW_ERR_UNSUPPORTED;
  p.Hg = H / 2; p.Wg = W / 2; p.so = 2; p.ncls = 4; p.kstep = 2;
  for (int c = 0; c < 4; c++) {
    const int py = c >> 1, px = c & 1;
    const int ky0 = (py + pt) & 1, kx0 = (px + pl) & 1;
    const int nty = ky0 < k ? (k - ky0 + 1) / 2 : 0, ntx = kx0 < k ? (k - kx0 + 1) / 2 : 0;
    if (nty == 0 || ntx == 0) return UNFLOW_ERR_UNSUPPORTED;
    p.cls[c] = TapClass{nty, ntx, (py + pt - ky0) / 2, (px + pl - kx0) / 2, ky0, kx0, py, px};
  }
  return UNFLOW_OK;
}

inline void build_deconv_fwd(GatherGeom& p, int B, int H, int W, int Cin, int Cout) {
  p.B = B; p.Hg = H; p.Wg = W; p.Hs = H; p.Ws = W; p.sm = 1;
  p.dstep = -1; p.kstep = 2; p.KW = 4; p.Cs = Cin; p.N = Cout; p.wtaps = 16;
  p.Hd = 2 * H; p.Wd = 2 * W; p.so = 2; p.ncls = 4; p.sp = 1; p.acc = 0;
  for (int c = 0; c < 4; c++) {
    const int py = c >> 1, px = c & 1;
    const int ky0 = (py + 1) & 1, kx0 = (px + 1) & 1;
    p.cls[c] = TapClass{2, 2, (py + 1 - ky0) / 2, (px + 1 - kx0) / 2, ky0, kx0, py, px};
  }
}

inline void build_deconv_dgrad(GatherGeom& p, int B, int H, int W, int Cin, int Cout) {
  p.B = B; p.Hg = H; p.Wg = W; p.Hs = 2 * H; p.Ws = 2 * W; p.sm = 2;
  p.dstep = 1; p.kstep = 1; p.KW = 4; p.Cs = Cout; p.N = Cin; p.wtaps = 16;
  p.Hd = H; p.Wd = W; p.so = 1; p.ncls = 1; p.sp = 1; p.acc = 0;
  p.cls[0] = TapClass{4, 4, -1, -1, 0, 0, 0, 0};
}

inline void build_deconv_dgrad_acc(GatherGeom& p, int B, int H, int W, int Cin, int Cout) {
  build_deconv_dgrad(p, B, H, W, Cin, Cout);
  p.sm = 1; p.sp = 2; p.acc = 1; p.ncls = 4; p.kstep = 2; p.dstep = 1;
  for (int c = 0; c < 4; c++) {
    const int py = c >> 1, px = c & 1;
    p.cls[c] = TapClass{2, 2, py - 1, px - 1, py, px, 0, 0};
  }
}

inline void build_conv_wgrad(WgradGeom& p, int B, int H, int W, int Cin, int Cout, int k, int stride) {
  int pt, pl, Ho, Wo;
  same_pads(H, k, stride, &pt, &Ho);
  same_pads(W, k, stride, &pl, &Wo);
  p.B = B; p.Hg = Ho; p.Wg = Wo; p.Hs = H; p.Ws = W; p.sm = stride;
  p.KH = k; p.KW = k; p.dy0 = -pt; p.dx0 = -pl; p.Ca = Cin; p.Cb = Cout;
}

inline void build_deconv_wgrad(WgradGeom& p, int B, int H, int W, int Cin, int Cout) {
  p.B = B; p.Hg = H; p.Wg = W; p.Hs = 2 * H; p.Ws = 2 * W; p.sm = 2;
  p.KH = 4; p.KW = 4; p.dy0 = -1; p.dx0 = -1; p.Ca = Cout; p.Cb = Cin;
}

inline int fill_one_round(long blocks, int slots, int max_split) {
  if (blocks >= slots) return 1;
  int ns = (int)(slots / blocks);
  if (ns > max_split) ns = max_split;
  if (ns < 1) ns = 1;
  auto eff = [&](int n) { const long b = blocks * n; return (double)b / (double)(((b + slots - 1) / slots) * slots); };
  const double e1 = eff(ns);
  if (e1 < 0.8) {
    int best = ns;
    double be = e1;
    for (int n = ns + 1; n <= max_split && blocks * n <= 3L * slots; n++)
      if (eff(n) > be + 0.02) { best = n; be = eff(n); }
    if (be >= e1 + 0.15) ns = best;
  }
  return ns;
}

constexpr int REDUCE_FAN = 32;

static __global__ void sum_partials_kernel(const float* __restrict__ partial, float* __restrict__ out, size_t n, int S,
                                           int fan) {
  const int G = (S + fan - 1) / fan;
  const size_t total = n * (size_t)G;
  for (size_t t = blockIdx.x * (size_t)blockDim.x + threadIdx.x; t < total; t += (size_t)gridDim.x * blockDim.x) {
    const size_t g = t / n, e = t - g * n;
    const int k1 = min(S, (int)(g + 1) * fan);
    float v = 0.f;
#pragma unroll 8
    for (int k = (int)g * fan; k < k1; k++) v += partial[(size_t)k * n + e];
    out[g * n + e] = v;
  }
}

typedef float f32x4_nt __attribute__((ext_vector_type(4)));
static __global__ void sum_partials4_kernel(const float4* __restrict__ partial, float4* __restrict__ out, size_t nq, int S,
                                            int fan) {
  const int G = (S + fan - 1) / fan;
  const size_t total = nq * (size_t)G;
  for (size_t t = blockIdx.x * (size_t)blockDim.x + threadIdx.x; t < total; t += (size_t)gridDim.x * blockDim.x) {
    const size_t g = t / nq, e = t - g * nq;
    const int k1 = min(S, (int)(g + 1) * fan);
    float4 v = make_float4(0.f, 0.f, 0.f, 0.f);
#pragma unroll 8
    for (int k = (int)g * fan; k < k1; k++) {
      const f32x4_nt a = __builtin_nontemporal_load(reinterpret_cast<const f32x4_nt*>(partial) + (size_t)k * nq + e);
      v.x += a.x; v.y += a.y; v.z += a.z; v.w += a.w;
    }
    f32x4_nt o; o.x = v.x; o.y = v.y; o.z = v.z; o.w = v.w;
    __builtin_nontemporal_store(o, reinterpret_cast<f32x4_nt*>(out) + g * nq + e);
  }
}

inline size_t reduce_scratch_bytes(size_t n, int S) {
  return S > REDUCE_FAN ? 2 * (size_t)((S + REDUCE_FAN - 1) / REDUCE_FAN) * n * sizeof(float) : 0;
}

inline void launch_sum_partials(const float* partial, float* out, size_t n, int S, int G, hipStream_t st) {
  const bool vec = n % 4 == 0 && ((reinterpret_cast<uintptr_t>(partial) | reinterpret_cast<uintptr_t>(out)) & 15) == 0;
  if (vec)
    sum_partials4_kernel<<<stream_grid((long)(n / 4 * G)), 256, 0, st>>>(reinterpret_cast<const float4*>(partial),
                                                                        reinterpret_cast<float4*>(out), n / 4, S, REDUCE_FAN);
  else
    sum_partials_kernel<<<stream_grid((long)(n * G)), 256, 0, st>>>(partial, out, n, S, REDUCE_FAN);
}

inline int reduce_partials(const float* partial, float* scratch, float* out, size_t n, int S, hipStream_t st) {
  while (S > REDUCE_FAN) {
    const int G = (S + REDUCE_FAN - 1) / REDUCE_FAN;
    launch_sum_partials(partial, scratch, n, S, G, st);
    partial = scratch;
    scratch = scratch + (size_t)G * n;
    S = G;
  }
  launch_sum_partials(partial, out, n, S, 1, st);
  return launch_status();
}

}
```

### unflow_amd/csrc/options.h

```cpp
#pragma once

#define UNFLOW_OPTION_LIST(X)                                                                                              \
  X(conv_math_fp32, 0)           \
  X(wgrad_math_fp32, 0)                             \
  X(corr_math_fp32, 0)                                                               \
  X(gather_min_kt, 8)                          \
  X(gather_max_split, 16)                                                           \
  X(wgrad_min_kt, 8)                     \
  X(gather_pp, 1)          \
  X(gather_pp_fill, 60)    \
  X(f16_k64, 1)            \
  X(f16_wgrad_dma, 1)      \
  X(f16_tall, 0)           \
  X(f16_db, 0)             \
  X(gather_tile2d, 1)                                                     \
  X(conv1_direct, 1)       \
  X(halo, 1)                                     \
  X(streamk, 1)                \
  X(streamk_groups, 8)             \
  X(halo_max_split, 16)                                         \
  X(halo_s2, 1)                       \
  X(xcd_swizzle, 1)                                                                        \
  X(wgrad_dma, 1)                                                \
  X(wgrad_pp, 1)                                                     \
  X(corr_nb, 1)                                                               \
  X(corr_rs, 2)            \
  X(corr_wb, 1)                                                                 \
  X(corr_rw, 1)                                                       \
  X(corr_bwd_b128, 1)                                                 \
  X(corr_bwd_rot, -1)              \
  X(corr_bwd_planes, 1)                                                 \
  X(corr_bwd_share, 1)                                          \
  X(fw_bwd_rows, 1)

namespace unflow {
struct Options {
#define X(name, def) int name = def;
  UNFLOW_OPTION_LIST(X)
#undef X
};
Options& options();
}
```

Measured before the change: 681.6 image-pairs/s.

## Split deconv weight-grad flow-channel tail into batched skinny kernel

For deconv layers whose input channels are 128k+4 (features plus upsampled flow), the weight gradient is split. The 128k feature columns go through the planes GEMM wgrad with a strided output. The 2 flow columns go into a new skinny kernel batched with the existing flow wgrad jobs, and the 2 pad columns are zeroed. This avoids padding the GEMM N dimension to the next 256 tile for a handful of columns. A separate option picks BN=128 when that wastes less padding. It adds a strided reduction kernel and more launch-plan complexity.

```diff
diff --git a/include/unflow_hip.h b/include/unflow_hip.h
--- a/include/unflow_hip.h
+++ b/include/unflow_hip.h
@@ -244,8 +244,8 @@
 
 size_t unflow_flow_wgrad_batched_workspace_bytes(int n, const int* kind, const int* B, const int* H, const int* W, const int* Cin);
 int unflow_flow_wgrad_batched(int n, const int* kind, const float* const* x, const int* ldx, const float* const* dz,
-                              const int* lddz, float* const* dw, const int* B, const int* H, const int* W, const int* Cin,
-                              void* workspace, size_t workspace_bytes, unflow_stream_t stream);
+                              const int* lddz, float* const* dw, const int* ldw, const int* B, const int* H, const int* W,
+                              const int* Cin, void* workspace, size_t workspace_bytes, unflow_stream_t stream);
 
 int unflow_debug_work_order(int mt, int nt, int ncls, int nsplit, int order, int xcd, int* out, int out_blocks);
 
@@ -284,6 +284,9 @@
 int unflow_conv2d_transpose_bwd_filter_pl(const float* x, int ldx, const unflow_planes* x_pl, const float* dz, int lddz,
                                           const unflow_planes* dz_pl, float* dw, int B, int H, int W, int Cin, int Cout,
                                           void* workspace, size_t workspace_bytes, unflow_stream_t stream);
+int unflow_conv2d_transpose_bwd_filter_pl_cols(const unflow_planes* x_pl, const unflow_planes* dz_pl, float* dw, int B, int H,
+                                               int W, int Cin, int Cout, int col_lo, int col_hi, void* workspace,
+                                               size_t workspace_bytes, unflow_stream_t stream);
 
 int unflow_resize_bilinear_tf1(const float* in, float* out, int B, int H, int W, int C, int out_h, int out_w,
                                float scale, unflow_stream_t stream);
diff --git a/unflow_amd/core/engine.py b/unflow_amd/core/engine.py
--- a/unflow_amd/core/engine.py
+++ b/unflow_amd/core/engine.py
@@ -478,7 +478,17 @@
             pending.clear()
 
         flow_jobs = []
-        n_flow = sum(1 for op, _, _, _ in self.bwd[lo:hi] if op.kind == 'layer' and op.l.cout <= 2)
+
+        def has_tail(op):
+            l = op.l
+            if l.kind != 'deconv' or l.cout <= 2 or op.src[0] == 'x0':
+                return False
+            up = self.bufs[op.src[0]][1].get('up')
+            return up is not None and up[1] == 2 and up[0] - op.src[1] == l.cin_p - 4 and op.src[2] - op.src[1] == l.cin_p
+
+        tail_ops = {id(op) for op, _, _, _ in self.bwd[lo:hi] if op.kind == 'layer' and has_tail(op)
+                    and L.deconv_flow_tail(_rows(self.pt(op.src), op.n), _rows(self.pt(op.dst, True), op.n))}
+        n_flow = sum(1 for op, _, _, _ in self.bwd[lo:hi] if op.kind == 'layer' and op.l.cout <= 2) + len(tail_ops)
 
         for k, (op, first, act_lo, act_hi) in enumerate(self.bwd[lo:hi], lo):
             if op.kind == 'corr':
@@ -511,17 +521,24 @@
                 e._bias_jobs.append((dz.t, l))
             xv = op.src[0] not in self.planes_only
             wg = (L.conv_bwd_filter, (x, dz, l.dw, l.stride, xv)) if l.kind == 'conv' else (L.deconv_bwd_filter, (x, dz, l.dw, xv))
+            batch = None
+            if id(op) in tail_ops:
+                wg = (L.deconv_bwd_filter, (x, dz, l.dw, xv, (0, l.cin_p - 4)))
+                flow_jobs.append(('deconv_tail', x.t[..., l.cin_p - 4:l.cin_p - 2], dz, l.dw))
             if l.cout <= 2:
                 flow_jobs.append((l.kind, x, dz, l.dw))
-                wg = (L.flow_wgrad_batched, (flow_jobs,)) if len(flow_jobs) == n_flow else None
-            if wg is None:
-                pass
-            elif side is None or (e.wgrad_inline_tiny and l.cout <= 2):
-                wg[0](*wg[1])
-            else:
-                pending.append(wg)
-                if len(pending) >= e.wgrad_group:
-                    flush()
+                wg = None
+            if len(flow_jobs) == n_flow and (l.cout <= 2 or id(op) in tail_ops):
+                batch = (L.flow_wgrad_batched, (flow_jobs,))
+            for job, tiny in ((wg, False), (batch, True)):
+                if job is None:
+                    pass
+                elif side is None or (e.wgrad_inline_tiny and tiny):
+                    job[0](*job[1])
+                else:
+                    pending.append(job)
+                    if len(pending) >= e.wgrad_group:
+                        flush()
             sb = op.src[0]
             is_input = sb == 'x0' or (sb == self.bin and op.src[1] == 0 and op.src[2] == pad4(self.in_ch)
                                       and op.l.name.endswith('conv1'))
diff --git a/unflow_amd/core/layers.py b/unflow_amd/core/layers.py
--- a/unflow_amd/core/layers.py
+++ b/unflow_amd/core/layers.py
@@ -253,7 +253,14 @@
           "conv2d_transpose_bwd_data_pl")
 
 
-def deconv_bwd_filter(x, dz, dw, x_fp32=True):
+def deconv_flow_tail(x, dz):
+    x, dz = _pt(x), _pt(dz)
+    Cin = x.t.shape[-1]
+    return (Cin > 4 and Cin % 128 == 4 and dz.t.shape[-1] > 4 and x.pl is not None and dz.pl is not None
+            and _lib.get_option("wgrad_flow_tail") > 0)
+
+
+def deconv_bwd_filter(x, dz, dw, x_fp32=True, cols=None):
     x, dz = _pt(x), _pt(dz)
     xp, ldx, B, H, W, Cin = nhwc(x.t)
     if not x_fp32:
@@ -262,6 +269,12 @@
     dzp, lddz, _, Ho, Wo, Cout = nhwc(dz.t)
     assert tuple(dw.shape) == (4, 4, Cout, Cin)
     wsp, wsn = _ws_pl(x.t.device, B, Ho, Wo, Cin, Cout, 4, 2, _npl(x, dz))
+    if cols is not None:
+        assert dw.is_contiguous() and x.pl is not None and dz.pl is not None
+        check(_lib.lib().unflow_conv2d_transpose_bwd_filter_pl_cols(x.planes(), dz.planes(), ptr(dw), B, H, W, Cin, Cout,
+                                                                    int(cols[0]), int(cols[1]), wsp, wsn, stream()),
+              "conv2d_transpose_bwd_filter_pl_cols")
+        return
     check(_lib.lib().unflow_conv2d_transpose_bwd_filter_pl(xp, ldx, x.planes(), dzp, lddz, dz.planes(),
                                                            ptr(dw), B, H, W, Cin, Cout, wsp, wsn, stream()),
           "conv2d_transpose_bwd_filter_pl")
@@ -274,29 +287,40 @@
         return
     xs = [_pt(j[1]).t for j in jobs]
     dzs = [_pt(j[2]).t for j in jobs]
-    kinds = (ctypes.c_int * n)(*[0 if j[0] == 'conv' else 1 for j in jobs])
+    code = {'conv': 0, 'deconv': 1, 'deconv_tail': 2}
+    kinds = (ctypes.c_int * n)(*[code[j[0]] for j in jobs])
     dims = [nhwc(x) for x in xs]
     Bs = (ctypes.c_int * n)(*[d[2] for d in dims])
     Hs = (ctypes.c_int * n)(*[d[3] for d in dims])
     Ws = (ctypes.c_int * n)(*[d[4] for d in dims])
-    Cs = (ctypes.c_int * n)(*[d[5] for d in dims])
+    Cs = (ctypes.c_int * n)(*[dz.shape[-1] if j[0] == 'deconv_tail' else d[5] for j, d, dz in zip(jobs, dims, dzs)])
     lib = _lib.lib()
     lib.unflow_flow_wgrad_batched_workspace_bytes.restype = ctypes.c_size_t
     need = lib.unflow_flow_wgrad_batched_workspace_bytes(n, kinds, Bs, Hs, Ws, Cs)
     if need == 0 or n > 16:
+        tails = [j for j in jobs if j[0] == 'deconv_tail']
         for kind, x, dz, dw in jobs:
             if kind == 'conv':
                 conv_bwd_filter(x, dz, dw, 1)
-            else:
+            elif kind == 'deconv':
                 deconv_bwd_filter(x, dz, dw)
+        for i in range(0, len(tails), 16):
+            flow_wgrad_batched(tails[i:i + 16])
         return
     for (kind, x, dz, dw), xt, dzt in zip(jobs, xs, dzs):
-        assert dw.is_contiguous() and dzt.shape[-1] == 2
+        assert dw.is_contiguous()
+        if kind == 'deconv_tail':
+            assert xt.shape[-1] == 2 and tuple(dw.shape[:3]) == (4, 4, dzt.shape[-1]) and dw.shape[3] >= 8
+            assert tuple(dzt.shape[:3]) == (xt.shape[0], 2 * xt.shape[1], 2 * xt.shape[2])
+            continue
+        assert dzt.shape[-1] == 2
         assert tuple(dw.shape) == ((3, 3, xt.shape[-1], 2) if kind == 'conv' else (4, 4, 2, 2))
     ws = workspace(need, xs[0].device, slot=_WS_SLOT[0])
+    dwp = [j[3].data_ptr() + (4 * (j[3].shape[3] - 4) if j[0] == 'deconv_tail' else 0) for j in jobs]
+    ldw = (ctypes.c_int * n)(*[j[3].shape[3] if j[0] == 'deconv_tail' else 0 for j in jobs])
     check(lib.unflow_flow_wgrad_batched(n, kinds, (ctypes.c_void_p * n)(*[x.data_ptr() for x in xs]),
                                         (ctypes.c_int * n)(*[x.stride(2) for x in xs]),
                                         (ctypes.c_void_p * n)(*[d.data_ptr() for d in dzs]),
                                         (ctypes.c_int * n)(*[d.stride(2) for d in dzs]),
-                                        (ctypes.c_void_p * n)(*[j[3].data_ptr() for j in jobs]), Bs, Hs, Ws, Cs, ptr(ws),
+                                        (ctypes.c_void_p * n)(*dwp), ldw, Bs, Hs, Ws, Cs, ptr(ws),
                                         csz(ws.numel() * 4), stream()), "flow_wgrad_batched")
diff --git a/unflow_amd/csrc/conv_igemm.hip b/unflow_amd/csrc/conv_igemm.hip
--- a/unflow_amd/csrc/conv_igemm.hip
+++ b/unflow_amd/csrc/conv_igemm.hip
@@ -1422,12 +1422,94 @@
   tiny_deconv_wgrad_body<CI, CO>(x, ldx, dz, lddz, partial, B, H, W, blockIdx.x, gridDim.x, red);
 }
 
+__device__ __forceinline__ void deconv_flow_tail_wgrad_body(const SkinnyWgradParams& p, int bx, int chunk, int nchunks,
+                                                            float* __restrict__ red) {
+  const int lane = threadIdx.x & 63;
+  const int wid = __builtin_amdgcn_readfirstlane((int)(threadIdx.x >> 6));
+  const int CO = p.Cin;
+  const int co = bx * 64 + lane;
+  const bool co_ok = co < CO;
+  const int H = p.H, W = p.W, OW = 2 * W;
+  const int n = p.B * H * W;
+  const int per = (n + nchunks - 1) / nchunks;
+  const int q0 = chunk * per, q1 = min(n, q0 + per);
+  float acc[16][2];
+#pragma unroll
+  for (int t = 0; t < 16; t++) acc[t][0] = acc[t][1] = 0.f;
+  constexpr int U = 4;
+  for (int qb = q0 + wid; qb < q1; qb += 4 * U) {
+    float g[U][2][2];
+    float xv[U][3][3][2];
+#pragma unroll
+    for (int j = 0; j < U; j++) {
+      const bool live = qb + 4 * j < q1;
+      const int q = live ? qb + 4 * j : qb;
+      const int ix0 = q % W, r = q / W;
+      const int iy0 = r % H;
+      const long b = r / H;
+#pragma unroll
+      for (int py = 0; py < 2; py++)
+#pragma unroll
+        for (int px = 0; px < 2; px++)
+          g[j][py][px] = (live && co_ok) ? p.dz[((b * 2 * H + 2 * iy0 + py) * OW + 2 * ix0 + px) * p.lddz + co] : 0.f;
+#pragma unroll
+      for (int u = 0; u < 3; u++)
+#pragma unroll
+        for (int v = 0; v < 3; v++) {
+          const int iy = iy0 - 1 + u, ix = ix0 - 1 + v;
+          const bool ok = live && (unsigned)iy < (unsigned)H && (unsigned)ix < (unsigned)W;
+          const float* xp = p.x + ((b * H + iy) * W + ix) * p.ldx;
+          xv[j][u][v][0] = ok ? xp[0] : 0.f;
+          xv[j][u][v][1] = ok ? xp[1] : 0.f;
+        }
+    }
+#pragma unroll
+    for (int j = 0; j < U; j++)
+#pragma unroll
+      for (int py = 0; py < 2; py++)
+#pragma unroll
+        for (int px = 0; px < 2; px++)
+#pragma unroll
+          for (int a = 0; a < 2; a++)
+#pragma unroll
+            for (int c = 0; c < 2; c++) {
+              const int ky = 1 - py + 2 * a, kx = 1 - px + 2 * c;
+              const int u = 1 + py - a, v = 1 + px - c;
+              acc[ky * 4 + kx][0] += g[j][py][px] * xv[j][u][v][0];
+              acc[ky * 4 + kx][1] += g[j][py][px] * xv[j][u][v][1];
+            }
+  }
+  float* out = p.partial + (size_t)chunk * 16 * CO * 2;
+#pragma unroll
+  for (int h = 0; h < 2; h++) {
+    if (h) __syncthreads();
+    if (wid > 0) {
+#pragma unroll
+      for (int t = 0; t < 8; t++) {
+        red[((wid - 1) * 16 + 2 * t) * 64 + lane] = acc[8 * h + t][0];
+        red[((wid - 1) * 16 + 2 * t + 1) * 64 + lane] = acc[8 * h + t][1];
+      }
+    }
+    __syncthreads();
+    if (wid == 0 && co_ok) {
+#pragma unroll
+      for (int t = 0; t < 8; t++) {
+        float2 s;
+        s.x = ((acc[8 * h + t][0] + red[(2 * t) * 64 + lane]) + red[(16 + 2 * t) * 64 + lane]) + red[(32 + 2 * t) * 64 + lane];
+        s.y = ((acc[8 * h + t][1] + red[(2 * t + 1) * 64 + lane]) + red[(16 + 2 * t + 1) * 64 + lane]) + red[(32 + 2 * t + 1) * 64 + lane];
+        *reinterpret_cast<float2*>(out + ((size_t)(8 * h + t) * CO + co) * 2) = s;
+      }
+    }
+  }
+}
+
 constexpr int MAX_FLOW_WGRAD = 16;
 struct FlowWgradDesc {
   SkinnyWgradParams p;
   float* out;
   int kind;
   int spw, colblocks, chunks, block0, wsz, rblock0;
+  int ldw;
 };
 struct FlowWgradBatch {
   FlowWgradDesc d[MAX_FLOW_WGRAD];
@@ -1445,6 +1527,10 @@
     return;
   }
   const int bx = lb % d.colblocks, by = lb / d.colblocks;
+  if (d.kind == 3) {
+    deconv_flow_tail_wgrad_body(d.p, bx, by, d.chunks, red);
+    return;
+  }
   if (d.kind == 0) head3_wgrad_strip_body<8>(d.p, d.spw, bx, by, red);
   else head3_wgrad_strip_body<4>(d.p, d.spw, bx, by, red);
 }
@@ -1461,7 +1547,15 @@
   }
 #pragma unroll
   for (int off = 1; off < 16; off <<= 1) v += __shfl_down(v, off, 64);
-  if (ok && q == 0) d.out[e] = v;
+  if (ok && q == 0) {
+    if (d.kind == 3) {
+      float* o = d.out + (size_t)(e >> 1) * d.ldw + (e & 1);
+      o[0] = v;
+      o[2] = 0.f;
+    } else {
+      d.out[e] = v;
+    }
+  }
 }
 
 constexpr int MAX_COLSUM = 32;
@@ -2016,6 +2110,11 @@
     d.chunks = (int)min((long)32, ((long)B * H * W + 255) / 256);
     return true;
   }
+  if (kind_in == 2) {
+    d.kind = 3; d.colblocks = cdiv(Cin, 64); d.spw = 0; d.wsz = 16 * Cin * 2;
+    d.chunks = (int)min((long)512, max((long)1, (long)B * H * W / 64));
+    return true;
+  }
   const int S = head_strip(B, H, W, 3, 2);
   if (S != 8 && S != 4) return false;
   d.kind = S == 8 ? 0 : 1;
@@ -2041,8 +2140,8 @@
 }
 
 UNFLOW_API int unflow_flow_wgrad_batched(int n, const int* kind, const float* const* x, const int* ldx, const float* const* dz,
-                                         const int* lddz, float* const* dw, const int* B, const int* H, const int* W, const int* Cin,
-                                         void* workspace, size_t workspace_bytes, unflow_stream_t stream) {
+                                         const int* lddz, float* const* dw, const int* ldw, const int* B, const int* H, const int* W,
+                                         const int* Cin, void* workspace, size_t workspace_bytes, unflow_stream_t stream) {
   if (!kind || !x || !ldx || !dz || !lddz || !dw || !B || !H || !W || !Cin) return UNFLOW_ERR_NULL;
   if (n <= 0) return UNFLOW_OK;
   if (n > MAX_FLOW_WGRAD) return UNFLOW_ERR_UNSUPPORTED;
@@ -2056,6 +2155,9 @@
     if (B[i] <= 0 || H[i] <= 0 || W[i] <= 0 || Cin[i] <= 0) return UNFLOW_ERR_SHAPE;
     if (kind[i] == 0 && (Cin[i] % 4 != 0 || ldx[i] % 4 != 0 || ldx[i] < Cin[i] || lddz[i] < 2)) return UNFLOW_ERR_UNSUPPORTED;
     if (kind[i] == 1 && Cin[i] != 2) return UNFLOW_ERR_UNSUPPORTED;
+    if (kind[i] == 2 && (!ldw || ldw[i] < 8 || ldx[i] < 2 || lddz[i] < Cin[i] || (long)B[i] * H[i] * W[i] > 0x3fffffffL))
+      return UNFLOW_ERR_UNSUPPORTED;
+    if (kind[i] < 0 || kind[i] > 2) return UNFLOW_ERR_UNSUPPORTED;
     if (!flow_wgrad_plan(d, kind[i], B[i], H[i], W[i], Cin[i])) return UNFLOW_ERR_UNSUPPORTED;
     int pt, pl, ho, wo;
     same_pads(H[i], 3, 1, &pt, &ho);
@@ -2066,6 +2168,7 @@
                             B[i], H[i], W[i], Cin[i], pt, pl};
     off += bytes;
     d.out = dw[i];
+    d.ldw = kind[i] == 2 ? ldw[i] : 0;
     d.block0 = blocks;
     blocks += d.chunks * d.colblocks;
     d.rblock0 = rblocks;
diff --git a/unflow_amd/csrc/conv_planes.hip b/unflow_amd/csrc/conv_planes.hip
--- a/unflow_amd/csrc/conv_planes.hip
+++ b/unflow_amd/csrc/conv_planes.hip
@@ -471,6 +471,7 @@
   float* out;
   float* partial;
   int lds, ldd;
+  int ldo;
   int Ca_out;
   float out_scale;
   int nsplit;
@@ -647,6 +648,7 @@
   }
 
   float* o = p.nsplit > 1 ? p.partial + (size_t)split * taps * p.Ca_out * p.Cb : p.out;
+  const int ldo = p.nsplit > 1 ? p.Cb : p.ldo;
   const int lh5 = lane >> 5;
 #pragma unroll
   for (int i = 0; i < TM; i++)
@@ -658,7 +660,7 @@
       const unsigned tp = p.cag_magic ? fast_div((unsigned)mgr, p.cag_magic) : (unsigned)mgr;
       const int a = (mgr - (int)tp * Cag) * 8 + (m & 7);
       if (a >= p.Ca_out) continue;
-      float* orow = o + ((size_t)tp * p.Ca_out + a) * p.Cb;
+      float* orow = o + ((size_t)tp * p.Ca_out + a) * ldo;
 #pragma unroll
       for (int j = 0; j < TN; j++) {
         const int n = n0 + wn * WN + j * 32 + l31;
@@ -880,6 +882,7 @@
   PHASE_FLUSH;
 
   float* o = p.nsplit > 1 ? p.partial + (size_t)split * taps * p.Ca_out * p.Cb : p.out;
+  const int ldo = p.nsplit > 1 ? p.Cb : p.ldo;
   const int lh5 = lane >> 5, l31 = lane & 31;
 #pragma unroll
   for (int i = 0; i < TM; i++)
@@ -891,7 +894,7 @@
       const unsigned tp = p.cag_magic ? fast_div((unsigned)mgr, p.cag_magic) : (unsigned)mgr;
       const int a = (mgr - (int)tp * Cag) * 8 + (m & 7);
       if (a >= p.Ca_out) continue;
-      float* orow = o + ((size_t)tp * p.Ca_out + a) * p.Cb;
+      float* orow = o + ((size_t)tp * p.Ca_out + a) * ldo;
 #pragma unroll
       for (int j = 0; j < TN; j++) {
         const int n = n0 + wn * WN + j * 32 + l31;
@@ -1124,6 +1127,7 @@
   }
 
   float* o = p.nsplit > 1 ? p.partial + (size_t)split * taps * p.Ca_out * p.Cb : p.out;
+  const int ldo = p.nsplit > 1 ? p.Cb : p.ldo;
   const int lh5 = lane >> 5, l31 = lane & 31;
 #pragma unroll
   for (int i = 0; i < TM; i++)
@@ -1135,7 +1139,7 @@
       const unsigned tp = p.cag_magic ? fast_div((unsigned)mgr, p.cag_magic) : (unsigned)mgr;
       const int a = (mgr - (int)tp * Cag) * 8 + (m & 7);
       if (a >= p.Ca_out) continue;
-      float* orow = o + ((size_t)tp * p.Ca_out + a) * p.Cb;
+      float* orow = o + ((size_t)tp * p.Ca_out + a) * ldo;
 #pragma unroll
       for (int j = 0; j < TN; j++) {
         const int nn = n0 + wn * WN + j * 32 + l31;
@@ -1581,7 +1585,11 @@
   if (o >= 3) return true;
   return p.Cb > 128 && (long)p.B * p.Hg * p.Wg >= 1536;
 }
-inline int pl_wgrad_pp_bn(const WgradGeom& p) { return p.Cb > 128 ? 256 : 128; }
+inline int pl_wgrad_pp_bn(const WgradGeom& p) {
+  if (p.Cb <= 128) return 128;
+  if (unflow::options().wgrad_pp_bn128 > 0 && cdiv(p.Cb, 128) * 128 < cdiv(p.Cb, 256) * 256) return 128;
+  return 256;
+}
 
 inline int plan_pl_wgrad(const WgradGeom& p, int npl) {
   const int Mp = p.KH * p.KW * p.Ca;
@@ -1647,8 +1655,15 @@
   return launch_status();
 }
 
-int run_pl_wgrad(PlWgradParams& p, int npl, void* ws, size_t ws_bytes, size_t* used, hipStream_t st) {
+int run_pl_wgrad(PlWgradParams& p, int npl, void* ws, size_t ws_bytes, size_t* used, hipStream_t st, int col_lo = 0, int col_hi = 0) {
   const unflow::Options& opt = unflow::options();
+  p.ldo = p.Cb;
+  if (col_hi > 0) {
+    if (col_lo < 0 || col_lo % 8 != 0 || col_hi <= col_lo || col_hi > p.Cb || (col_hi - col_lo) % 4 != 0) return UNFLOW_ERR_UNSUPPORTED;
+    p.dst += col_lo;
+    p.out += col_lo;
+    p.Cb = col_hi - col_lo;
+  }
   if (p.out_scale == 0.f) p.out_scale = 1.f;
   p.xcd = opt.xcd_swizzle;
   p.cag_magic = p.Ca == 8 ? 0u : magic_u32((unsigned)(p.Ca >> 3));
@@ -1670,7 +1685,7 @@
   else if (opt.wgrad_dma && opt.f16_wgrad_dma) code = cfg == 1 ? launch_pl_wgrad_dma<64, 32, true>(p, st) : launch_pl_wgrad_dma<128, 64, true>(p, st);
   else code = cfg == 1 ? launch_pl_wgrad<128, 64, 64, 32, 1, true>(p, st) : launch_pl_wgrad<128, 128, 64, 64, 1, true>(p, st);
   if (code != UNFLOW_OK) return code;
-  if (ns > 1) return reduce_partials(p.partial, p.partial + (size_t)ns * wsize, p.out, wsize, ns, st);
+  if (ns > 1) return reduce_partials(p.partial, p.partial + (size_t)ns * wsize, p.out, wsize, ns, st, p.Cb, p.ldo);
   return UNFLOW_OK;
 }
 
@@ -1863,6 +1878,10 @@
     WgradGeom tw{};
     build_deconv_wgrad(tw, B, H / 2, W / 2, Cin, Co8);
     need = max(need, pl_wgrad_plan_bytes(tw, Cout, n_planes));
+    if (Cin > 4 && Cin % 128 == 4) {
+      tw.Cb = Cin - 4;
+      need = max(need, pl_wgrad_plan_bytes(tw, Cout, n_planes));
+    }
   }
   return need + 1024;
 }
@@ -2014,6 +2033,22 @@
   return run_pl_gather(p, dz_pl->n_planes, workspace, workspace_bytes, as_stream(stream));
 }
 
+UNFLOW_API int unflow_conv2d_transpose_bwd_filter_pl_cols(const unflow_planes* x_pl, const unflow_planes* dz_pl, float* dw, int B,
+                                                          int H, int W, int Cin, int Cout, int col_lo, int col_hi,
+                                                          void* workspace, size_t workspace_bytes, unflow_stream_t stream) {
+  if (!dw || !x_pl || !dz_pl) return UNFLOW_ERR_NULL;
+  if (B <= 0 || H <= 0 || W <= 0 || Cin <= 0 || Cout <= 0) return UNFLOW_ERR_SHAPE;
+  if (!use_planes(x_pl, Cin, dz_pl, Cout, Cout) || Cin % 4 != 0 || Cin <= 4 || col_hi <= 0) return UNFLOW_ERR_UNSUPPORTED;
+  PlWgradParams p{};
+  build_deconv_wgrad(p, B, H, W, Cin, (Cout + 7) & ~7);
+  p.src = reinterpret_cast<const unsigned short*>(dz_pl->base); p.src_ps = dz_pl->plane_stride; p.lds = dz_pl->ld;
+  p.dst = reinterpret_cast<const unsigned short*>(x_pl->base); p.dst_ps = x_pl->plane_stride; p.ldd = x_pl->ld;
+  p.out_scale = 1.f / (plane_scale(x_pl) * plane_scale(dz_pl));
+  p.out = dw; p.Ca_out = Cout;
+  size_t used = 0;
+  return run_pl_wgrad(p, x_pl->n_planes, workspace, workspace_bytes, &used, as_stream(stream), col_lo, col_hi);
+}
+
 UNFLOW_API int unflow_conv2d_transpose_bwd_filter_pl(const float* x, int ldx, const unflow_planes* x_pl, const float* dz,
                                                      int lddz, const unflow_planes* dz_pl, float* dw, int B, int H, int W,
                                                      int Cin, int Cout, void* workspace, size_t workspace_bytes,
@@ -2023,12 +2058,5 @@
   if (!use_planes(x_pl, Cin, dz_pl, Cout, Cout) || Cin % 4 != 0 || Cin <= 4)
     return (!x || !dz) ? UNFLOW_ERR_UNSUPPORTED :
            unflow_conv2d_transpose_bwd_filter(x, ldx, dz, lddz, dw, nullptr, B, H, W, Cin, Cout, workspace, workspace_bytes, stream);
-  PlWgradParams p{};
-  build_deconv_wgrad(p, B, H, W, Cin, (Cout + 7) & ~7);
-  p.src = reinterpret_cast<const unsigned short*>(dz_pl->base); p.src_ps = dz_pl->plane_stride; p.lds = dz_pl->ld;
-  p.dst = reinterpret_cast<const unsigned short*>(x_pl->base); p.dst_ps = x_pl->plane_stride; p.ldd = x_pl->ld;
-  p.out_scale = 1.f / (plane_scale(x_pl) * plane_scale(dz_pl));
-  p.out = dw; p.Ca_out = Cout;
-  size_t used = 0;
-  return run_pl_wgrad(p, x_pl->n_planes, workspace, workspace_bytes, &used, as_stream(stream));
-}
+  return unflow_conv2d_transpose_bwd_filter_pl_cols(x_pl, dz_pl, dw, B, H, W, Cin, Cout, 0, Cin, workspace, workspace_bytes, stream);
+}
diff --git a/unflow_amd/csrc/igemm_shared.h b/unflow_amd/csrc/igemm_shared.h
--- a/unflow_amd/csrc/igemm_shared.h
+++ b/unflow_amd/csrc/igemm_shared.h
@@ -361,7 +361,38 @@
     sum_partials_kernel<<<stream_grid((long)(n * G)), 256, 0, st>>>(partial, out, n, S, REDUCE_FAN);
 }
 
-inline int reduce_partials(const float* partial, float* scratch, float* out, size_t n, int S, hipStream_t st) {
+template <int V>
+static __global__ void sum_partials_rows_kernel(const float* __restrict__ partial, float* __restrict__ out, size_t n, int cols,
+                                                int ldo, int S) {
+  const size_t nv = n / V;
+  const int cv = cols / V;
+  for (size_t t = blockIdx.x * (size_t)blockDim.x + threadIdx.x; t < nv; t += (size_t)gridDim.x * blockDim.x) {
+    const size_t r = t / cv;
+    const int c = (int)(t - r * cv) * V;
+    float v[V];
+#pragma unroll
+    for (int i = 0; i < V; i++) v[i] = 0.f;
+#pragma unroll 8
+    for (int k = 0; k < S; k++) {
+      if constexpr (V == 4) {
+        const f32x4_nt a = __builtin_nontemporal_load(reinterpret_cast<const f32x4_nt*>(partial + (size_t)k * n) + t);
+        v[0] += a.x; v[1] += a.y; v[2] += a.z; v[3] += a.w;
+      } else {
+        v[0] += partial[(size_t)k * n + t];
+      }
+    }
+    float* o = out + r * (size_t)ldo + c;
+    if constexpr (V == 4) {
+      f32x4_nt q; q.x = v[0]; q.y = v[1]; q.z = v[2]; q.w = v[3];
+      __builtin_nontemporal_store(q, reinterpret_cast<f32x4_nt*>(o));
+    } else {
+      *o = v[0];
+    }
+  }
+}
+
+inline int reduce_partials(const float* partial, float* scratch, float* out, size_t n, int S, hipStream_t st, int cols = 0,
+                           int ldo = 0) {
   while (S > REDUCE_FAN) {
     const int G = (S + REDUCE_FAN - 1) / REDUCE_FAN;
     launch_sum_partials(partial, scratch, n, S, G, st);
@@ -369,6 +400,12 @@
     scratch = scratch + (size_t)G * n;
     S = G;
   }
+  if (cols > 0 && ldo != cols) {
+    const bool vec = cols % 4 == 0 && ldo % 4 == 0 && ((reinterpret_cast<uintptr_t>(partial) | reinterpret_cast<uintptr_t>(out)) & 15) == 0;
+    if (vec) sum_partials_rows_kernel<4><<<stream_grid((long)(n / 4)), 256, 0, st>>>(partial, out, n, cols, ldo, S);
+    else sum_partials_rows_kernel<1><<<stream_grid((long)n), 256, 0, st>>>(partial, out, n, cols, ldo, S);
+    return launch_status();
+  }
   launch_sum_partials(partial, out, n, S, 1, st);
   return launch_status();
 }
diff --git a/unflow_amd/csrc/options.h b/unflow_amd/csrc/options.h
--- a/unflow_amd/csrc/options.h
+++ b/unflow_amd/csrc/options.h
@@ -23,7 +23,9 @@
   X(xcd_swizzle, 1)                                                                        \
   X(wgrad_dma, 1)                                                \
   X(wgrad_pp, 1)                                                     \
-  X(corr_nb, 1)                                                               \
+  X(wgrad_pp_bn128, 1)     \
+  X(wgrad_flow_tail, 1)    \
+  X(corr_nb, 1)                                                             \
   X(corr_rs, 2)            \
   X(corr_wb, 1)                                                                 \
   X(corr_rw, 1)                                                       \
```

Result: no change. 687.8 image-pairs/s, median of 6 (+0.9%).
